# yanglei18/SGV3D

Measured on AMD Instinct MI355X. Metric: camera frames/sec at 864x1536->BEV, higher is better.
Workload: dtype f32

## Files before the change

include/sgv3d_hip.h:

```cpp
#ifndef SGV3D_HIP_H
#define SGV3D_HIP_H

#include <stddef.h>
#include <stdint.h>

#ifdef __cplusplus
extern "C" {
#endif

#define SGV3D_OK 0
#define SGV3D_EINVAL (-1)
#define SGV3D_ELAUNCH (-2)
#define SGV3D_ENOSPACE (-3)

const char *sgv3d_last_error(void);
int sgv3d_abi_version(void);


int sgv3d_voxel_pooling_forward(int batch_size, int num_points, int num_channels,
                                int num_voxel_x, int num_voxel_y, int num_voxel_z,
                                const int32_t *geom_xyz, const float *input_features,
                                float *output_features, int32_t *pos_memo, void *stream);
int sgv3d_voxel_pooling_forward_fresh(int batch_size, int num_points, int num_channels,
                                      int num_voxel_x, int num_voxel_y, int num_voxel_z,
                                      const int32_t *geom_xyz, const float *input_features,
                                      float *output_features, int32_t *pos_memo, void *stream);
int sgv3d_voxel_pooling_select_kernel(int which);
int sgv3d_voxel_pooling_kernel_for(int batch_size, int num_points, int num_channels, int num_voxel_x, int num_voxel_y, int fused);
int sgv3d_voxel_pooling_cache_clear(void);
int sgv3d_voxel_pooling_cache_stats(unsigned long long *out4);

int sgv3d_voxel_pooling_forward_atomic(int batch_size, int num_points, int num_channels,
                                       int num_voxel_x, int num_voxel_y, int num_voxel_z,
                                       const int32_t *geom_xyz, const float *input_features,
                                       float *output_features, int32_t *pos_memo, void *stream);

size_t sgv3d_voxel_plan_bytes(int batch_size, int num_points, int num_voxel_x, int num_voxel_y);

int sgv3d_voxel_plan_build(int batch_size, int num_points,
                           int num_voxel_x, int num_voxel_y, int num_voxel_z,
                           const int32_t *geom_xyz, int32_t *pos_memo,
                           void *plan, size_t plan_bytes, int sort_segments, void *stream);

int sgv3d_voxel_plan_init(int batch_size, int num_points, int num_voxel_x, int num_voxel_y,
                          void *plan, size_t plan_bytes, void *stream);
int sgv3d_voxel_plan_build_cached(int batch_size, int num_points,
                                  int num_voxel_x, int num_voxel_y, int num_voxel_z,
                                  const int32_t *geom_xyz, void *plan, size_t plan_bytes,
                                  int sort_segments, void *stream);
size_t sgv3d_voxel_plan_stats_offset(int batch_size, int num_points, int num_voxel_x, int num_voxel_y);

size_t sgv3d_voxel_pooling_workspace_bytes(int batch_size, int num_points, int num_channels);
int sgv3d_voxel_pooling_forward_planned(int batch_size, int num_points, int num_channels,
                                        int num_voxel_x, int num_voxel_y,
                                        const void *plan, const float *input_features,
                                        float *output_features, void *workspace, size_t workspace_bytes,
                                        void *stream);
int sgv3d_voxel_pooling_forward_planned_bf16(int batch_size, int num_points, int num_channels,
                                             int num_voxel_x, int num_voxel_y, const void *plan,
                                             const void *input_features_bf16, void *output_features, int out_bf16_ld,
                                             void *workspace, size_t workspace_bytes, void *stream);

int sgv3d_lift_splat_planned(int batch_size, int num_depth, int num_pixels, int num_channels,
                             int num_voxel_x, int num_voxel_y, const void *plan,
                             const float *prob, const float *context,
                             float *output_features, void *workspace, size_t workspace_bytes,
                             void *stream);

int sgv3d_lift_splat_planned_bf16out(int batch_size, int num_depth, int num_pixels, int num_channels, int num_voxel_x,
                                     int num_voxel_y, const void *plan, const float *prob, const void *context, int context_bf16,
                                     void *output_bf16, int out_bf16_ld, void *workspace, size_t workspace_bytes, void *stream);

int sgv3d_voxel_pooling_backward(int batch_size, int num_points, int num_channels,
                                 const int32_t *pos_memo, const float *grad_output,
                                 long long sb, long long sc, long long sy, long long sx,
                                 float *grad_input, void *stream);

size_t sgv3d_lift_splat_backward_workspace_bytes(int batch_size, int num_depth, int num_pixels, int num_channels);
int sgv3d_lift_splat_backward(int batch_size, int num_depth, int num_pixels, int num_channels,
                              int num_voxel_x, int num_voxel_y, int num_voxel_z,
                              const int32_t *geom_xyz,
                              const float *prob,
                              const float *context,
                              const float *grad_output,
                              long long sb, long long sy, long long sx,
                              float *grad_prob,
                              float *grad_context,
                              void *workspace, size_t workspace_bytes, void *stream);


int sgv3d_calib_prep(int num_cams, const float *sensor2ego, const float *sensor2virtual,
                     const float *intrin, const float *ida, float *prep, void *stream);

int sgv3d_geometry_voxel_index(int num_cams, int cams_per_batch, int num_depth, int feat_h, int feat_w,
                               const float *frustum, const float *prep, const float *ref_h,
                               const float *bda, const float *voxel_coord ,
                               const float *voxel_size , int32_t *geom_xyz, float *geom_f,
                               void *stream);

int sgv3d_calib_changed(int n, const void *const *tensors , const int32_t *nbytes ,
                        void *copy, int force, int32_t *changed, void *stream);
int sgv3d_calib_prep_gated(int num_cams, const float *sensor2ego, const float *sensor2virtual, const float *intrin,
                           const float *ida, float *prep, const int32_t *run, void *stream);
// ... 3 lines not shown
                                     float *geom_f, const int32_t *run, void *stream);


int sgv3d_lift(int batch_size, int num_pixels, int num_depth, int num_channels,
               const float *height_context, float *prob, float *lifted, void *stream);
int sgv3d_lift_bf16(int batch_size, int num_pixels, int num_depth, int num_channels, const float *height_context,
                    float *prob, void *lifted_bf16, void *stream);


typedef struct sgv3d_conv_desc {
    int batch, in_h, in_w, cin;
    int out_h, out_w, cout;
    int kh, kw, stride, pad, dil;
    int x_ld, x_coff;
    int y_ld, y_coff;
    int res_ld;
    int relu;
    int mode;
    int deconv_ks;
    int k_pad, cout_pad;
    int tile;
    int x_nchw;
    int k_order;
    int split_k;
} sgv3d_conv_desc;

#define SGV3D_CONV_NORMAL 0
#define SGV3D_CONV_DECONV 1
#define SGV3D_CONV_NCHW_OUT 2
#define SGV3D_CONV_GROUP_PLANES 3

#define SGV3D_TILE_128x128 1
#define SGV3D_TILE_128x64 2
#define SGV3D_TILE_64x128 3
#define SGV3D_TILE_64x64 4
#define SGV3D_TILE_32x128 9
#define SGV3D_TILE_48x64 10
#define SGV3D_TILE_X3 64
#define SGV3D_TILE_MFIRST 16
#define SGV3D_TILE_OCC5 32
#define SGV3D_WINOGRAD_RESIDENT 6
#define SGV3D_WINOGRAD_HALF 8

int sgv3d_conv_winograd4_pack_weight(const float *w_src , int cout, int cin, int k_pad, int cout_pad,
                                     float *u_packed , void *stream);
int sgv3d_conv_winograd4_pack_weight_x3(const float *w_src, int cout, int cin, int cin_pad, int cout_pad, void *u3_packed,
                                        void *stream);

int sgv3d_conv_pack_weight_x3(const float *w_src, int cout, int cin, int kh, int kw, int cin_pad, int cout_pad, void *u3_packed,
                              void *stream);
int sgv3d_conv2d_x3_forward(const sgv3d_conv_desc *desc, const float *x, const void *u3_packed, const float *scale,
                            const float *bias, const float *residual, float *y, void *workspace, size_t workspace_bytes,
                            void *stream);
int sgv3d_conv2d_x3_shortcut_forward(const sgv3d_conv_desc *desc_a, const float *xa, const void *u3a, const float *scale_a,
                                     const float *bias_a, const sgv3d_conv_desc *desc_b, const float *xb, const void *u3b,
                                     const float *scale_b, const float *bias_b, float *y, void *stream);
int sgv3d_stem_pool_x3_forward(int batch, int h, int w, const float *x_nchw, const void *w_x3, size_t w_bytes, const float *scale,
                               const float *shift, float *y_nhwc, int y_ld, int variant, void *stream);
int sgv3d_wino4_lattice_axis(int n, int dil, int tile, int k0, int count, int *tiles, int *stacked, int *pixels);
size_t sgv3d_conv2d_winograd4_workspace_bytes(const sgv3d_conv_desc *desc );
int sgv3d_conv2d_winograd4_forward(const sgv3d_conv_desc *desc , const float *x, const float *u_packed,
                                   const float *scale, const float *bias, const float *residual, float *y,
                                   void *workspace, size_t workspace_bytes, void *stream);

size_t sgv3d_conv2d_winograd4_multi_workspace_bytes(int n, const sgv3d_conv_desc *descs );
int sgv3d_conv2d_winograd4_forward_multi(int n, const sgv3d_conv_desc *descs , const float *x, const void *const *u_packed,
                                         const float *const *scale, const float *const *bias, float *const *y, void *workspace,
                                         size_t workspace_bytes, void *stream);

void sgv3d_conv_pack_geometry(int k, int n, int *k_pad, int *n_pad);

int sgv3d_conv_pack_weight(const float *w_src, int cout, int cin, int kh, int kw, int cin_pad,
                           int transposed, int k_order, float *w_packed, int k_pad, int cout_pad,
                           void *stream);

size_t sgv3d_conv2d_workspace_bytes(const sgv3d_conv_desc *desc );
int sgv3d_conv2d_forward(const sgv3d_conv_desc *desc , const float *x, const float *w_packed,
                         const float *scale, const float *bias, const float *residual,
                         const float *gate, float *y, void *workspace, size_t workspace_bytes,
                         void *stream);

int sgv3d_conv2d_forward_bf16(const sgv3d_conv_desc *desc , const float *x, const float *w_packed,
                              const float *scale, const float *bias, const float *residual,
                              const float *gate, float *y, void *workspace, size_t workspace_bytes,
                              void *stream);

int sgv3d_conv_weight_to_bf16(const float *w_packed, int k_pad, int cout_pad, void *w_packed_bf16, void *stream);
int sgv3d_conv2d_forward_bf16io(const sgv3d_conv_desc *desc , const void *x, const void *w_packed,
                                const float *scale, const float *bias, const void *residual, const float *gate,
                                void *y, void *workspace, size_t workspace_bytes, void *stream, int io_flags);

int sgv3d_conv2d_forward_f32x3(const sgv3d_conv_desc *desc , const float *x, const float *w_packed,
                               const float *scale, const float *bias, const float *residual,
                               const float *gate, float *y, void *workspace, size_t workspace_bytes,
                               void *stream);

size_t sgv3d_conv_winograd_weight_floats(int cout, int cin_pad);
int sgv3d_conv_winograd_pack_weight(const float *w_src, int cout, int cin, int cin_pad, float *w_packed,
                                    void *stream);
int sgv3d_conv2d_winograd_forward(const sgv3d_conv_desc *desc , const float *x, const float *w_wino,
                                  const float *scale, const float *bias, const float *residual,
                                  const float *gate, float *y, void *workspace, size_t workspace_bytes,
                                  void *stream);


int sgv3d_maxpool3x3s2(int batch, int in_h, int in_w, int channels, const float *x, float *y,
// ... 630 lines not shown
```

sgv3d_amd/_lib.py:

```python
import ctypes
import os

_HERE = os.path.dirname(os.path.abspath(__file__))
LIB_PATH = os.path.join(_HERE, "csrc", "libsgv3d_hip.so")

c_int, c_void_p, c_size_t, c_ll = ctypes.c_int, ctypes.c_void_p, ctypes.c_size_t, ctypes.c_longlong


class ConvDesc(ctypes.Structure):
    _fields_ = [(n, c_int) for n in (
        "batch", "in_h", "in_w", "cin", "out_h", "out_w", "cout", "kh", "kw", "stride", "pad", "dil",
        "x_ld", "x_coff", "y_ld", "y_coff", "res_ld", "relu", "mode", "deconv_ks", "k_pad", "cout_pad",
        "tile", "x_nchw", "k_order", "split_k")]


class VitAttnDesc(ctypes.Structure):
    _fields_ = [(n, c_int) for n in ("batch", "height", "width", "heads", "head_dim", "win_h", "win_w")]


class SamAttnDesc(ctypes.Structure):
    _fields_ = [(n, c_int) for n in ("batch", "nq", "nk", "heads", "head_dim", "q_ld", "k_ld", "v_ld", "o_ld")] + [("scale", ctypes.c_float)]


CONV_NORMAL, CONV_DECONV, CONV_NCHW_OUT, CONV_GROUP_PLANES = 0, 1, 2, 3
TILE_AUTO, TILE_128x128, TILE_128x64, TILE_64x128, TILE_64x64 = 0, 1, 2, 3, 4

_PROTOS = {
    "sgv3d_last_error": (ctypes.c_char_p, []),
    "sgv3d_abi_version": (c_int, []),
    "sgv3d_voxel_pooling_select_kernel": (c_int, [c_int]),
    "sgv3d_voxel_pooling_kernel_for": (c_int, [c_int] * 6),
    "sgv3d_voxel_pooling_forward": (c_int, [c_int] * 6 + [c_void_p] * 5),
    "sgv3d_voxel_pooling_forward_fresh": (c_int, [c_int] * 6 + [c_void_p] * 5),
    "sgv3d_voxel_pooling_forward_atomic": (c_int, [c_int] * 6 + [c_void_p] * 5),
    "sgv3d_voxel_pooling_cache_clear": (c_int, []),
    "sgv3d_voxel_pooling_cache_stats": (c_int, [ctypes.POINTER(ctypes.c_ulonglong)]),
    "sgv3d_voxel_plan_bytes": (c_size_t, [c_int] * 4),
    "sgv3d_voxel_plan_build": (c_int, [c_int] * 5 + [c_void_p, c_void_p, c_void_p, c_size_t, c_int, c_void_p]),
    "sgv3d_voxel_plan_init": (c_int, [c_int] * 4 + [c_void_p, c_size_t, c_void_p]),
    "sgv3d_voxel_plan_build_cached": (c_int, [c_int] * 5 + [c_void_p, c_void_p, c_size_t, c_int, c_void_p]),
    "sgv3d_voxel_plan_stats_offset": (c_size_t, [c_int] * 4),
    "sgv3d_voxel_pooling_workspace_bytes": (c_size_t, [c_int] * 3),
    "sgv3d_voxel_pooling_forward_planned": (c_int, [c_int] * 5 + [c_void_p] * 4 + [c_size_t, c_void_p]),
    "sgv3d_voxel_pooling_forward_planned_bf16": (c_int, [c_int] * 5 + [c_void_p] * 3 + [c_int, c_void_p, c_size_t, c_void_p]),
    "sgv3d_lift_splat_planned_bf16out": (c_int, [c_int] * 6 + [c_void_p] * 3 + [c_int, c_void_p, c_int, c_void_p, c_size_t, c_void_p]),
    "sgv3d_lift_splat_planned": (c_int, [c_int] * 6 + [c_void_p] * 5 + [c_size_t, c_void_p]),
    "sgv3d_voxel_pooling_backward": (c_int, [c_int] * 3 + [c_void_p, c_void_p, c_ll, c_ll, c_ll, c_ll, c_void_p, c_void_p]),
    "sgv3d_lift_splat_backward_workspace_bytes": (c_size_t, [c_int] * 4),
    "sgv3d_lift_splat_backward": (c_int, [c_int] * 7 + [c_void_p] * 4 + [c_ll] * 3 + [c_void_p] * 3 + [c_size_t, c_void_p]),
    "sgv3d_calib_prep": (c_int, [c_int] + [c_void_p] * 6),
    "sgv3d_calib_prep_gated": (c_int, [c_int] + [c_void_p] * 7),
    "sgv3d_calib_changed": (c_int, [c_int, ctypes.POINTER(c_void_p), ctypes.POINTER(c_int), c_void_p, c_int, c_void_p, c_void_p]),
    "sgv3d_geometry_voxel_index_gated": (c_int, [c_int] * 5 + [c_void_p] * 4 + [ctypes.POINTER(ctypes.c_float)] * 2 + [c_void_p] * 4),
    "sgv3d_dense_gated": (c_int, [c_int] * 3 + [c_void_p] * 4 + [c_int, c_void_p, c_void_p, c_void_p]),
    "sgv3d_geometry_voxel_index": (c_int, [c_int] * 5 + [c_void_p] * 4 + [ctypes.POINTER(ctypes.c_float)] * 2 + [c_void_p] * 3),
    "sgv3d_lift": (c_int, [c_int] * 4 + [c_void_p] * 4),
    "sgv3d_lift_bf16": (c_int, [c_int] * 4 + [c_void_p] * 4),
    "sgv3d_conv_pack_geometry": (None, [c_int, c_int, ctypes.POINTER(c_int), ctypes.POINTER(c_int)]),
    "sgv3d_conv_pack_weight": (c_int, [c_void_p] + [c_int] * 7 + [c_void_p, c_int, c_int, c_void_p]),
    "sgv3d_conv2d_workspace_bytes": (c_size_t, [ctypes.POINTER(ConvDesc)]),
    "sgv3d_conv2d_forward": (c_int, [ctypes.POINTER(ConvDesc)] + [c_void_p] * 8 + [c_size_t, c_void_p]),
    "sgv3d_conv2d_forward_bf16": (c_int, [ctypes.POINTER(ConvDesc)] + [c_void_p] * 8 + [c_size_t, c_void_p]),
    "sgv3d_conv2d_forward_bf16io": (c_int, [ctypes.POINTER(ConvDesc)] + [c_void_p] * 8 + [c_size_t, c_void_p, c_int]),
    "sgv3d_conv_weight_to_bf16": (c_int, [c_void_p, c_int, c_int, c_void_p, c_void_p]),
    "sgv3d_conv2d_forward_f32x3": (c_int, [ctypes.POINTER(ConvDesc)] + [c_void_p] * 8 + [c_size_t, c_void_p]),
    "sgv3d_centerhead_branches_workspace_bytes": (c_size_t, [c_int] * 4),
    "sgv3d_centerhead_branches_forward": (c_int, [c_int] * 6 + [c_void_p, c_int] + [c_void_p] * 3 + [c_int] + [c_void_p] * 5
                                          + [c_size_t, c_void_p]),
    "sgv3d_centerhead_bf16_weight_bytes": (c_size_t, [c_int]),
    "sgv3d_centerhead_bf16_pack_weight": (c_int, [c_void_p, c_int, c_int, c_void_p, c_void_p]),
    "sgv3d_centerhead_bf16_weight2_bytes": (c_size_t, [c_int]),
    "sgv3d_centerhead_bf16_pack_weight2": (c_int, [c_void_p, c_void_p, c_int, c_void_p, c_void_p]),
    "sgv3d_centerhead_f4_weight_floats": (c_size_t, [c_int]),
    "sgv3d_centerhead_f4_pack_weight": (c_int, [c_void_p, c_int, c_void_p, c_void_p]),
    "sgv3d_centerhead_branches_forward_f4": (c_int, [c_int] * 6 + [c_void_p, c_int] + [c_void_p] * 3 + [c_int] + [c_void_p] * 5
                                             + [c_size_t, c_void_p]),
    "sgv3d_conv3x3_f4res_weight_floats": (c_size_t, [c_int, c_int]),
    "sgv3d_conv3x3_f4res_pack_weight": (c_int, [c_void_p, c_int, c_int, c_int, c_void_p, c_void_p]),
    "sgv3d_conv3x3_f4res_forward": (c_int, [ctypes.POINTER(ConvDesc)] + [c_void_p] * 7),
    "sgv3d_centerhead_branches_forward_bf16": (c_int, [c_int] * 6 + [c_void_p, c_int] + [c_void_p] * 3 + [c_int] + [c_void_p] * 5),
    "sgv3d_centerhead_branches_forward_bf16x": (c_int, [c_int] * 6 + [c_void_p, c_int] + [c_void_p] * 3 + [c_int] + [c_void_p] * 5),
    "sgv3d_centerhead_bf16_select_plain": (None, [c_int]),
    "sgv3d_centerhead_bf16_debug_stamps": (None, [c_void_p]),
    "sgv3d_scale_channels_bf16": (c_int, [c_int] * 3 + [c_void_p] * 4),
    "sgv3d_global_avgpool_bf16": (c_int, [c_int] * 4 + [c_void_p] * 3 + [c_size_t, c_void_p]),
    "sgv3d_broadcast_channels_bf16": (c_int, [c_int] * 5 + [c_void_p] * 3),
    "sgv3d_upsample_bilinear2x_bf16": (c_int, [c_int] * 4 + [c_void_p] * 3),
    "sgv3d_add_mul_sigmoid_bf16": (c_int, [c_ll] + [c_void_p] * 5),
    "sgv3d_deform_im2col3x3_bf16": (c_int, [c_int] * 5 + [c_void_p] * 2 + [c_int, c_void_p, c_void_p]),
    "sgv3d_conv3x3_patch_bf16_weight_bytes": (c_size_t, [c_int, c_int]),
    "sgv3d_conv3x3_patch_bf16_debug_stamps": (None, [c_void_p]),
    "sgv3d_conv3x3_patch_bf16_pack_weight": (c_int, [c_void_p, c_int, c_int, c_void_p, c_void_p]),
    "sgv3d_conv3x3_patch_bf16_forward": (c_int, [c_int] * 11 + [c_void_p] * 6 + [c_int, c_int, c_void_p, c_size_t, c_void_p]),
    "sgv3d_conv_dw_bf16_weight_bytes": (c_size_t, [c_int] * 4),
    "sgv3d_conv_dw_bf16_pack_weight": (c_int, [c_void_p] + [c_int] * 5 + [c_void_p, c_void_p]),
    "sgv3d_conv_dw_bf16_forward": (c_int, [ctypes.POINTER(ConvDesc)] + [c_void_p] * 7),
    "sgv3d_conv_dw_bf16_workspace_bytes": (c_size_t, [ctypes.POINTER(ConvDesc)]),
    "sgv3d_conv_dw_bf16_forward_splitk": (c_int, [ctypes.POINTER(ConvDesc)] + [c_void_p] * 7 + [c_size_t, c_void_p]),
    "sgv3d_conv_dw_bf16_pair_forward": (c_int, [ctypes.POINTER(ConvDesc)] + [c_void_p] * 4 + [c_int] + [c_void_p] * 4 + [c_int, c_void_p, c_int, c_int, c_int, c_void_p]),
    "sgv3d_conv_winograd_weight_floats": (c_size_t, [c_int, c_int]),
    "sgv3d_conv_winograd_pack_weight": (c_int, [c_void_p, c_int, c_int, c_int, c_void_p, c_void_p]),
    "sgv3d_conv2d_winograd_forward": (c_int, [ctypes.POINTER(ConvDesc)] + [c_void_p] * 8 + [c_size_t, c_void_p]),
    "sgv3d_conv_winograd4_pack_weight": (c_int, [c_void_p, c_int, c_int, c_int, c_int, c_void_p, c_void_p]),
    "sgv3d_conv_winograd4_pack_weight_x3": (c_int, [c_void_p, c_int, c_int, c_int, c_int, c_void_p, c_void_p]),
    "sgv3d_conv_pack_weight_x3": (c_int, [c_void_p, c_int, c_int, c_int, c_int, c_int, c_int, c_void_p, c_void_p]),
    "sgv3d_conv2d_x3_forward": (c_int, [c_void_p] * 8 + [c_size_t, c_void_p]),
    "sgv3d_conv2d_x3_shortcut_forward": (c_int, [c_void_p] * 12),
    "sgv3d_stem_pool_x3_forward": (c_int, [c_int] * 3 + [c_void_p, c_void_p, c_size_t] + [c_void_p] * 3 + [c_int, c_int, c_void_p]),
    "sgv3d_wino4_lattice_axis": (c_int, [c_int] * 5 + [c_void_p] * 3),
    "sgv3d_conv2d_winograd4_workspace_bytes": (c_size_t, [ctypes.POINTER(ConvDesc)]),
    "sgv3d_conv2d_winograd4_forward": (c_int, [ctypes.POINTER(ConvDesc)] + [c_void_p] * 7 + [c_size_t, c_void_p]),
    "sgv3d_conv2d_winograd4_multi_workspace_bytes": (c_size_t, [c_int, c_void_p]),
    "sgv3d_conv2d_winograd4_forward_multi": (c_int, [c_int] + [c_void_p] * 7 + [c_size_t, c_void_p]),
    "sgv3d_maxpool3x3s2": (c_int, [c_int] * 4 + [c_void_p] * 3),
    "sgv3d_maxpool3x3s2_bf16": (c_int, [c_int] * 4 + [c_void_p] * 3),
    "sgv3d_nchw_to_nhwc": (c_int, [c_int] * 5 + [c_void_p] * 3),
    "sgv3d_nhwc_to_nchw": (c_int, [c_int] * 6 + [c_void_p] * 3),
    "sgv3d_global_avgpool_workspace_bytes": (c_size_t, [c_int] * 2),
    "sgv3d_global_avgpool": (c_int, [c_int] * 4 + [c_void_p] * 3 + [c_size_t, c_void_p]),
    "sgv3d_dense": (c_int, [c_int] * 3 + [c_void_p] * 4 + [c_int, c_void_p, c_void_p]),
    "sgv3d_broadcast_channels": (c_int, [c_int] * 5 + [c_void_p] * 3),
    "sgv3d_scale_channels": (c_int, [c_int] * 3 + [c_void_p] * 4),
    "sgv3d_copy_channels": (c_int, [c_int] * 5 + [c_void_p] * 3),
    "sgv3d_upsample_bilinear2x": (c_int, [c_int] * 4 + [c_void_p] * 3),
    "sgv3d_add_mul_sigmoid": (c_int, [c_ll] + [c_void_p] * 5),
    "sgv3d_bsm_compose": (c_int, [c_int] * 6 + [c_void_p, c_int, ctypes.c_float, c_void_p, c_void_p]),
    "sgv3d_deform_im2col3x3": (c_int, [c_int] * 5 + [c_void_p, c_void_p, c_int, c_void_p, c_void_p]),
    "sgv3d_deform_conv3x3_forward": (c_int, [c_int] * 6 + [c_void_p, c_void_p, c_int, c_void_p, c_int, c_int, c_void_p, c_int, c_int,
                                                          c_void_p]),
    "sgv3d_deform_conv3x3_bf16_weight_bytes": (c_size_t, [c_int] * 3),
    "sgv3d_deform_conv3x3_bf16_pack_weight": (c_int, [c_void_p, c_int, c_int, c_int, c_void_p, c_void_p]),
    "sgv3d_deform_conv3x3_forward_bf16": (c_int, [c_int] * 6 + [c_void_p, c_int, c_void_p, c_int, c_void_p, c_void_p, c_int, c_int, c_int,
                                                               c_void_p]),
    "sgv3d_head_final_conv": (c_int, [c_int] * 6 + [c_void_p] * 6),
    "sgv3d_centerpoint_decode_workspace_bytes": (c_size_t, [c_int] * 3),
    "sgv3d_centerpoint_decode": (c_int, [c_int] * 5 + [c_void_p] * 6 + [c_ll] + [ctypes.c_float] * 6 +
                                 [ctypes.POINTER(ctypes.c_float), c_int, ctypes.c_float, c_int, c_void_p, c_size_t] +
                                 [c_void_p] * 6),
    "sgv3d_centerpoint_decode_tasks_workspace_bytes": (c_size_t, [c_int] * 4),
    "sgv3d_centerpoint_decode_tasks": (c_int, [c_int, c_int, ctypes.POINTER(ctypes.c_int32), c_int, c_int, c_int] +
                                       [ctypes.POINTER(c_void_p)] * 6 + [c_ll] + [ctypes.c_float] * 6 +
                                       [ctypes.POINTER(ctypes.c_float), c_int, ctypes.POINTER(ctypes.c_float), c_int, c_void_p,
                                        c_size_t] + [c_void_p] * 6),
    "sgv3d_centerpoint_merge_tasks": (c_int, [c_int] * 3 + [c_void_p] * 4 + [ctypes.POINTER(ctypes.c_int32)] + [c_void_p] * 5),
    "sgv3d_rotated_bev_iou_host": (c_int, [c_int] + [ctypes.POINTER(ctypes.c_float)] * 3),
    "sgv3d_rotate_nms_workspace_bytes": (c_size_t, [c_int] * 3),
    "sgv3d_rotate_nms": (c_int, [c_int] * 3 + [c_void_p] * 3 + [ctypes.c_float, ctypes.POINTER(ctypes.c_float), c_int, c_int,
                                                                ctypes.POINTER(ctypes.c_float), c_void_p, c_size_t, c_void_p, c_void_p]),
    "sgv3d_centerpoint_decode_tasks_rotate_workspace_bytes": (c_size_t, [c_int] * 4),
    "sgv3d_centerpoint_decode_tasks_rotate": (c_int, [c_int, c_int, ctypes.POINTER(ctypes.c_int32), c_int, c_int, c_int] +
                                              [ctypes.POINTER(c_void_p)] * 6 + [c_ll] + [ctypes.c_float] * 6 +
                                              [ctypes.POINTER(ctypes.c_float), c_int, ctypes.c_float, ctypes.POINTER(ctypes.c_float),
                                               c_int, c_int, ctypes.POINTER(ctypes.c_float), c_void_p, c_size_t] + [c_void_p] * 6),
    "sgv3d_centerhead_targets": (c_int, [c_int, c_int, c_void_p, c_void_p, c_int, ctypes.POINTER(ctypes.c_int32)] +
                                 [c_int] * 3 + [ctypes.c_float] * 5 + [ctypes.c_double, c_int, c_int] + [c_void_p] * 5),
    "sgv3d_conv2d_backward_weight_workspace_bytes": (c_size_t, [ctypes.POINTER(ConvDesc), c_int]),
    "sgv3d_conv2d_backward_weight": (c_int, [ctypes.POINTER(ConvDesc)] + [c_void_p] * 3 + [c_int, c_void_p, c_size_t, c_void_p]),
    "sgv3d_conv2d_backward_weight_bf16_workspace_bytes": (c_size_t, [ctypes.POINTER(ConvDesc), c_int]),
    "sgv3d_conv2d_backward_weight_bf16": (c_int, [ctypes.POINTER(ConvDesc)] + [c_void_p] * 3 + [c_int, c_void_p, c_size_t, c_void_p]),
# ... 196 lines not shown
```

sgv3d_amd/csrc/conv_pw_x3.hip:

```cpp
#include "conv_common.hpp"
#include "f32x3.hpp"

using namespace sgv3d;

namespace {

struct PwX3Args {
    const float *x, *scale, *bias, *res;
    const void *w;
    float *y;
    int M, K, N;
    int x_ld, x_coff, y_ld, y_coff, res_ld, relu;
    int cout_pad, tiles_m, tiles_n, mfirst;
    unsigned x_bytes, w_bytes;
    int in_h, in_w, out_h, out_w, kh, kw, stride, pad, dil;
    int cin4;
    int split_k;
    float *ws;
    const float *x2, *scale2, *bias2;
    const void *w2;
    int K2, x2_ld, x2_coff;
    unsigned x2_bytes, w2_bytes;
};

template <int MA, int WN, int MODE>
__global__ __launch_bounds__(64 * WN, 2) void conv_pw_x3_kernel(const PwX3Args a) {
    constexpr bool TAPS = MODE == 1, TM = MODE == 2, DUAL = MODE == 3, DECONV = MODE == 4;
    constexpr int NT = 64 * WN, BM = 16 * MA, BN = 32 * WN;
    constexpr int PLANE = x3_plane_bytes(BM), BUF = x3_buf_bytes(BM);
    __shared__ __attribute__((aligned(16))) unsigned char smem[2 * BUF];

    const int logical = xcd_tile(blockIdx.x, a.tiles_m * a.tiles_n);
    int tn, tm;
    if (a.mfirst) {
        tm = (int)((unsigned)logical / (unsigned)a.tiles_n);
        tn = logical - tm * a.tiles_n;
    } else {
        tn = (int)((unsigned)logical / (unsigned)a.tiles_m);
        tm = logical - tn * a.tiles_m;
    }
    const int m0 = tm * BM, n0 = tn * BN;
    const int kb = a.K >> 5;

    const int tid = threadIdx.x;
    __amdgpu_buffer_rsrc_t x_rsrc = __builtin_amdgcn_make_buffer_rsrc(const_cast<float *>(a.x), 0, (int)a.x_bytes, 0x00020000);
    __amdgpu_buffer_rsrc_t w_rsrc = __builtin_amdgcn_make_buffer_rsrc(const_cast<void *>(a.w), 0, (int)a.w_bytes, 0x00020000);

    constexpr int RPA = NT / 8, PA = (BM + RPA - 1) / RPA;
    static_assert(RPA % 16 == 0, "a pass is a multiple of 16 rows");
    const int arow = tid >> 3, ach = tid & 7;
    unsigned xg[PA];
    [[maybe_unused]] unsigned xmask[PA];
    [[maybe_unused]] unsigned long long xmask64[PA];
    bool a_on[PA];
    const int taps = (TAPS || TM) ? a.kh * a.kw : 1;
#pragma unroll
    for (int i = 0; i < PA; ++i) {
        const int r = arow + RPA * i;
        a_on[i] = (arow & ~7) + RPA * i < BM;
        const bool live = a_on[i] && m0 + r < a.M;
        if constexpr (!TAPS && !TM) {
            xg[i] = live ? (unsigned)((((long long)(m0 + r)) * a.x_ld + a.x_coff + ach * 4) * 4) : 0xffffffffu;
        } else if constexpr (TM) {
            const int m = live ? m0 + r : 0;
            const int t = (int)((unsigned)m / (unsigned)a.out_w);
            const int ow = m - t * a.out_w;
            const int n = (int)((unsigned)t / (unsigned)a.out_h);
            const int oh = t - n * a.out_h;
            const int ih0 = oh * a.stride - a.pad, iw0 = ow * a.stride - a.pad;
            xg[i] = (unsigned)((((long long)(n * a.in_h + ih0) * a.in_w + iw0) * a.x_ld + a.x_coff) * 4);
            unsigned long long mk = 0;
            int tt = 0;
            for (int th = 0; th < a.kh; ++th) {
                const bool row_in = live && (unsigned)(ih0 + th * a.dil) < (unsigned)a.in_h;
                for (int tw = 0; tw < a.kw; ++tw, ++tt) mk |= (row_in && (unsigned)(iw0 + tw * a.dil) < (unsigned)a.in_w) ? (1ull << tt) : 0ull;
            }
            xmask64[i] = mk;
        } else {
            const int m = live ? m0 + r : 0;
            const int t = (int)((unsigned)m / (unsigned)a.out_w);
            const int ow = m - t * a.out_w;
            const int n = (int)((unsigned)t / (unsigned)a.out_h);
            const int oh = t - n * a.out_h;
            const int ih0 = oh * a.stride - a.pad, iw0 = ow * a.stride - a.pad;
            xg[i] = (unsigned)((((long long)(n * a.in_h + ih0) * a.in_w + iw0) * a.x_ld + a.x_coff + ach * 4) * 4);
            unsigned mk = 0;
            int tt = 0;
            for (int th = 0; th < a.kh; ++th) {
                const bool row_in = live && (unsigned)(ih0 + th * a.dil) < (unsigned)a.in_h;
                for (int tw = 0; tw < a.kw; ++tw, ++tt) mk |= (row_in && (unsigned)(iw0 + tw * a.dil) < (unsigned)a.in_w) ? (1u << tt) : 0u;
            }
            xmask[i] = mk;
        }
    }
    [[maybe_unused]] int ld_tap = 0, ld_kh = 0, ld_kw = 0, ld_c0 = 0;
    [[maybe_unused]] const int cq = a.cin4;
    [[maybe_unused]] int tm_tap = 0, tm_kh = 0, tm_kw = 0, tm_c4 = 0;
    const unsigned xl = (unsigned)(arow * 64 + ((((ach >> 1) ^ x3_swizzle(arow)) << 4) | ((ach & 1) << 3)));

    const int wave = tid >> 6, lane = tid & 63;
    const int l16 = lane & 15, g = lane >> 4;
    unsigned wgo[2];
#pragma unroll
    for (int nb = 0; nb < 2; ++nb) wgo[nb] = u3_lane_offset((n0 >> 4) + 2 * wave + nb, kb, lane, a.cout_pad);
    const unsigned x_frag = X3_FRAG_OFFSET(l16, g);

    f32x4 acc[MA][2];
#pragma unroll
    for (int ma = 0; ma < MA; ++ma)
#pragma unroll
        for (int nb = 0; nb < 2; ++nb) acc[ma][nb] = f32x4{0.f, 0.f, 0.f, 0.f};

    f32x4 rx[PA];
    bf16x8 fw[2][2][3];
    int kt0 = 0, nkt = kb;
    if (a.split_k > 1) {
        kt0 = (int)((unsigned)kb * blockIdx.y / (unsigned)a.split_k);
        nkt = (int)((unsigned)kb * (blockIdx.y + 1) / (unsigned)a.split_k) - kt0;
        if constexpr (TAPS) {
            const int chunk = kt0 / taps;
            ld_tap = kt0 - chunk * taps;
            ld_c0 = chunk * 32;
            ld_kh = ld_tap / a.kw;
            ld_kw = ld_tap - ld_kh * a.kw;
        }
    }
    if constexpr (TM) {
        const int q = kt0 * 8 + ach;
        tm_tap = q / cq;
        tm_c4 = q - tm_tap * cq;
        tm_kh = tm_tap / a.kw;
        tm_kw = tm_tap - tm_kh * a.kw;
    }

#define PWX3_REQUEST(KT)                                                                                  \
    do {                                                                                                  \
        if constexpr (!TAPS && !TM) {                                                                     \
            _Pragma("unroll") for (int i = 0; i < PA; ++i)                                                \
                rx[i] = __builtin_bit_cast(f32x4, __builtin_amdgcn_raw_buffer_load_b128(x_rsrc, xg[i], (kt0 + (KT)) * 128, 0)); \
        } else if constexpr (TM) {                                                                        \
            const unsigned koff_ = (unsigned)((((tm_kh * a.in_w + tm_kw) * a.dil) * a.x_ld + tm_c4 * 4) * 4); \
            const unsigned long long bit_ = tm_tap < taps ? 1ull << tm_tap : 0ull;      \
            _Pragma("unroll") for (int i = 0; i < PA; ++i)                                                \
                rx[i] = __builtin_bit_cast(f32x4, __builtin_amdgcn_raw_buffer_load_b128(                   \
                    x_rsrc, (xmask64[i] & bit_) ? xg[i] + koff_ : 0xffffffffu, 0, 0));                    \
            tm_c4 += 8;                                                                                   \
            while (tm_c4 >= cq) {                                                                         \
                tm_c4 -= cq;                                                                              \
                ++tm_tap;                                                                                 \
                if (++tm_kw == a.kw) { tm_kw = 0; ++tm_kh; }                                              \
            }                                                                                             \
        } else {                                                                                          \
            const unsigned koff_ = (unsigned)((((ld_kh * a.in_w + ld_kw) * a.dil) * a.x_ld + ld_c0) * 4);  \
            const unsigned bit_ = 1u << ld_tap;                                                           \
            _Pragma("unroll") for (int i = 0; i < PA; ++i)                                                \
                rx[i] = __builtin_bit_cast(f32x4, __builtin_amdgcn_raw_buffer_load_b128(                   \
                    x_rsrc, (xmask[i] & bit_) ? xg[i] + koff_ : 0xffffffffu, 0, 0));                      \
            ++ld_tap;                                                                                     \
            if (++ld_kw == a.kw) {                                                                        \
                ld_kw = 0;                                                                                \
                if (++ld_kh == a.kh) { ld_kh = 0; ld_tap = 0; ld_c0 += 32; }                              \
            }                                                                                             \
        }                                                                                                 \
    } while (0)
#define PWX3_STORE(B)                                                                                     \
    do {                                                                                                  \
        _Pragma("unroll") for (int i = 0; i < PA; ++i)                                                    \
            if (a_on[i]) {                                                                                \
                bf16x4 hi, mid, lo;                                                                       \
                split3(rx[i], hi, mid, lo);                                                               \
                unsigned char *d = smem + (B) * BUF + xl + i * RPA * 64;                                  \
                *reinterpret_cast<bf16x4 *>(d) = hi;                                                      \
                *reinterpret_cast<bf16x4 *>(d + PLANE) = mid;                                             \
                *reinterpret_cast<bf16x4 *>(d + 2 * PLANE) = lo;                                          \
            }                                                                                             \
    } while (0)
#define PWX3_KLOOP() X3_KLOOP(MA, smem, w_rsrc, wgo, kt0, nkt, x_frag, fw, acc, PWX3_REQUEST, PWX3_STORE)

    PWX3_KLOOP();
    [[maybe_unused]] f32x4 tkeep[MA][2];
    if constexpr (DUAL) {
#pragma unroll
        for (int nb = 0; nb < 2; ++nb) {
            const int col = n0 + 32 * wave + 16 * nb + 4 * g;
            const bool on = col < a.N;
            const f32x4 sc = (on && a.scale) ? *reinterpret_cast<const f32x4 *>(a.scale + col) : f32x4{1.f, 1.f, 1.f, 1.f};
            const f32x4 sh = (on && a.bias) ? *reinterpret_cast<const f32x4 *>(a.bias + col) : f32x4{0.f, 0.f, 0.f, 0.f};
#pragma unroll
            for (int ma = 0; ma < MA; ++ma) {
                tkeep[ma][nb] = acc[ma][nb] * sc + sh;
                acc[ma][nb] = f32x4{0.f, 0.f, 0.f, 0.f};
            }
        }
        x_rsrc = __builtin_amdgcn_make_buffer_rsrc(const_cast<float *>(a.x2), 0, (int)a.x2_bytes, 0x00020000);
        w_rsrc = __builtin_amdgcn_make_buffer_rsrc(const_cast<void *>(a.w2), 0, (int)a.w2_bytes, 0x00020000);
        nkt = a.K2 >> 5;
#pragma unroll
        for (int i = 0; i < PA; ++i) {
            const int r = arow + RPA * i;
            const bool live = a_on[i] && m0 + r < a.M;
            const int m = live ? m0 + r : 0;
            const int t = (int)((unsigned)m / (unsigned)a.out_w);
            const int ow = m - t * a.out_w;
            const int n = (int)((unsigned)t / (unsigned)a.out_h);
            const int oh = t - n * a.out_h;
            xg[i] = live ? (unsigned)((((long long)(n * a.in_h + oh * a.stride) * a.in_w + ow * a.stride) * a.x2_ld + a.x2_coff + ach * 4) * 4)
                         : 0xffffffffu;
        }
#pragma unroll
        for (int nb = 0; nb < 2; ++nb) wgo[nb] = u3_lane_offset((n0 >> 4) + 2 * wave + nb, nkt, lane, a.cout_pad);
        __syncthreads();
        PWX3_KLOOP();
    }
#undef PWX3_KLOOP
#undef PWX3_REQUEST
#undef PWX3_STORE

    if (a.split_k > 1) {
        float *wsb = a.ws + (size_t)blockIdx.y * a.M * a.N;
#pragma unroll
        for (int nb = 0; nb < 2; ++nb) {
            const int col = n0 + 32 * wave + 16 * nb + 4 * g;
            if (col >= a.N) continue;
#pragma unroll
            for (int ma = 0; ma < MA; ++ma) {
                const int row = m0 + 16 * ma + l16;
                if (row < a.M) *reinterpret_cast<f32x4 *>(wsb + (size_t)row * a.N + col) = acc[ma][nb];
            }
        }
        return;
    }
    const float floor_ = a.relu ? 0.f : -__builtin_inff();
// ... 32 lines not shown
                const int row = m0 + 16 * ma + l16;
                if (row >= a.M) continue;
                const int img = (int)((unsigned)row / (unsigned)hw), pix = row - img * hw;
                const int ih = (int)((unsigned)pix / (unsigned)a.in_w), iw = pix - ih * a.in_w;
                f32x4 v = acc[ma][nb] * sc + sh;
                v = f32x4{fmaxf(v[0], floor_), fmaxf(v[1], floor_), fmaxf(v[2], floor_), fmaxf(v[3], floor_)};
                *reinterpret_cast<f32x4 *>(a.y + ((size_t)(img * a.out_h + ih * ks + dy) * a.out_w + (iw * ks + dx)) * a.y_ld + a.y_coff + co) = v;
            }
        }
        return;
    }
#pragma unroll
    for (int nb = 0; nb < 2; ++nb) {
        const int col = n0 + 32 * wave + 16 * nb + 4 * g;
        if (col >= a.N) continue;
        const f32x4 sc = a.scale ? *reinterpret_cast<const f32x4 *>(a.scale + col) : f32x4{1.f, 1.f, 1.f, 1.f};
        const f32x4 sh = a.bias ? *reinterpret_cast<const f32x4 *>(a.bias + col) : f32x4{0.f, 0.f, 0.f, 0.f};
#pragma unroll
        for (int ma = 0; ma < MA; ++ma) {
            const int row = m0 + 16 * ma + l16;
            if (row >= a.M) continue;
            f32x4 v = acc[ma][nb] * sc + sh;
            if (a.res) v += *reinterpret_cast<const f32x4 *>(a.res + (size_t)row * a.res_ld + col);
            v = f32x4{fmaxf(v[0], floor_), fmaxf(v[1], floor_), fmaxf(v[2], floor_), fmaxf(v[3], floor_)};
            *reinterpret_cast<f32x4 *>(a.y + (size_t)row * a.y_ld + a.y_coff + col) = v;
        }
    }
}

__global__ __launch_bounds__(256) void pack_weight_x3_kernel(const float *__restrict__ w, int cout, int cin, int cin_pad, int cout_pad,
                                                             int taps, int k_order, __bf16 *__restrict__ u) {
    const long long kp = k_order ? (long long)taps * cin_pad : ((long long)taps * cin_pad + 31) / 32 * 32;
    const long long i = (long long)blockIdx.x * 256 + threadIdx.x;
    if (i >= (long long)cout_pad * kp) return;
    const int co = (int)(i / kp), k = (int)(i - (long long)co * kp);
    int tap, ci;
    if (k_order) {
        const int chunk = k / (32 * taps), rem = k - chunk * 32 * taps;
        tap = rem >> 5;
        ci = chunk * 32 + (rem & 31);
    } else {
        tap = k / cin_pad;
        ci = k - tap * cin_pad;
    }
    const float v = (co < cout && ci < cin && tap < taps) ? w[((size_t)co * cin + ci) * taps + tap] : 0.f;
    __bf16 hi, mid, lo;
    split3_rounded(v, hi, mid, lo);
    u3_store(u3_at(u, co, k, kp), hi, mid, lo);
}

template <int MA, int WN>
int launch_pw(const PwX3Args &a, int mode, hipStream_t st) {
    const dim3 grid(a.tiles_m * a.tiles_n, a.split_k > 1 ? a.split_k : 1);
    if (mode == 4) hipLaunchKernelGGL((conv_pw_x3_kernel<MA, WN, 4>), grid, dim3(64 * WN), 0, st, a);
    else if (mode == 3) hipLaunchKernelGGL((conv_pw_x3_kernel<MA, WN, 3>), grid, dim3(64 * WN), 0, st, a);
    else if (mode == 2) hipLaunchKernelGGL((conv_pw_x3_kernel<MA, WN, 2>), grid, dim3(64 * WN), 0, st, a);
    else if (mode == 1) hipLaunchKernelGGL((conv_pw_x3_kernel<MA, WN, 1>), grid, dim3(64 * WN), 0, st, a);
    else hipLaunchKernelGGL((conv_pw_x3_kernel<MA, WN, 0>), grid, dim3(64 * WN), 0, st, a);
    return check_launch("conv_pw_x3_kernel");
}

}

extern "C" int sgv3d_conv_pack_weight_x3(const float *w_src, int cout, int cin, int kh, int kw, int cin_pad, int cout_pad, void *u3_packed,
                                         void *stream) {
    const int k_order = cin_pad % 32 == 0 ? 1 : 0;
    SGV3D_REQUIRE(w_src && u3_packed && cout > 0 && cin > 0 && kh > 0 && kw > 0 && kh * kw <= (k_order ? 32 : 64) && cin_pad >= cin &&
                      cin_pad % 4 == 0 && cout_pad >= cout && cout_pad % 32 == 0,
                  "conv_pack_weight_x3: bad arguments (cout=%d cin=%d k=%dx%d cin_pad=%d cout_pad=%d)", cout, cin, kh, kw, cin_pad, cout_pad);
    const long long kp = k_order ? (long long)cin_pad * kh * kw : ((long long)cin_pad * kh * kw + 31) / 32 * 32;
    const long long total = (long long)cout_pad * kp;
    hipLaunchKernelGGL(pack_weight_x3_kernel, dim3(cdiv(total, 256)), dim3(256), 0, as_stream(stream), w_src, cout, cin, cin_pad, cout_pad,
                       kh * kw, k_order, static_cast<__bf16 *>(u3_packed));
    return check_launch("pack_weight_x3_kernel");
}

extern "C" int sgv3d_conv2d_x3_forward(const sgv3d_conv_desc *d, const float *x, const void *u3_packed, const float *scale,
                                       const float *bias, const float *residual, float *y, void *workspace, size_t workspace_bytes,
                                       void *stream) {
    SGV3D_REQUIRE(d && x && u3_packed && y, "conv2d_x3_forward: null pointer");
    const bool tapmajor = d->cin % 32 != 0;
    const bool deconv = d->mode == SGV3D_CONV_DECONV;
    if (deconv) {
        SGV3D_REQUIRE(d->kh == 1 && d->kw == 1 && d->stride == 1 && d->pad == 0 && d->deconv_ks >= 1 && d->deconv_ks <= 64 &&
                          residual == nullptr,
                      "conv2d_x3_forward: DECONV runs as a 1x1 GEMM with deconv_ks = kernel = stride (<= 64), no residual");
        SGV3D_REQUIRE(d->in_h > 0 && d->in_w > 0 && d->out_h == d->in_h * d->deconv_ks && d->out_w == d->in_w * d->deconv_ks,
                      "conv2d_x3_forward: DECONV output must be input * deconv_ks");
        SGV3D_REQUIRE(d->cin > 0 && d->cin % 32 == 0 && d->cout > 0 && d->cout % 4 == 0 &&
                          (long long)d->cout * d->deconv_ks * d->deconv_ks <= 0x1000000LL,
                      "conv2d_x3_forward: DECONV needs cin %% 32 == 0, cout %% 4 == 0 (cin=%d cout=%d)", d->cin, d->cout);
        SGV3D_REQUIRE((long long)d->batch * d->out_h * d->out_w < 0x7fffffffLL, "conv2d_x3_forward: DECONV output has 2^31 pixels or more");
    }
    SGV3D_REQUIRE((deconv || d->mode == SGV3D_CONV_NORMAL) && d->kh > 0 && d->kw > 0 && d->kh * d->kw <= (tapmajor ? 64 : 32) && d->stride > 0 &&
                      d->dil > 0 && d->pad >= 0,
                  "conv2d_x3_forward: NHWC output, at most 32 taps (64 with tap-major weights)");
    SGV3D_REQUIRE(d->batch > 0 && d->in_h > 0 && d->in_w > 0 && d->cin > 0 && d->cout > 0 && d->cin % 4 == 0 && d->cout % 4 == 0,
                  "conv2d_x3_forward: cin %% 4 == 0, cout %% 4 == 0 (cin=%d cout=%d)", d->cin, d->cout);
    SGV3D_REQUIRE(deconv || (d->out_h == (d->in_h + 2 * d->pad - d->dil * (d->kh - 1) - 1) / d->stride + 1 &&
                                 d->out_w == (d->in_w + 2 * d->pad - d->dil * (d->kw - 1) - 1) / d->stride + 1),
                  "conv2d_x3_forward: output size does not match the geometry");
    SGV3D_REQUIRE((d->x_ld & 3) == 0 && (d->x_coff & 3) == 0 && (d->y_ld & 3) == 0 && (d->y_coff & 3) == 0 && (residual == nullptr || (d->res_ld & 3) == 0),
                  "conv2d_x3_forward: leading dimensions and channel offsets must be multiples of 4");
    SGV3D_REQUIRE(d->x_ld >= d->x_coff + d->cin && d->y_ld >= d->y_coff + d->cout && (residual == nullptr || d->res_ld >= d->cout),
                  "conv2d_x3_forward: leading dimension too small");
    const int gemm_n = deconv ? d->cout * d->deconv_ks * d->deconv_ks : d->cout;
    SGV3D_REQUIRE(d->cout_pad >= gemm_n && d->cout_pad % 32 == 0, "conv2d_x3_forward: desc.cout_pad = rows of the x3 weights (a multiple of 32)");
    SGV3D_REQUIRE(((reinterpret_cast<uintptr_t>(x) | reinterpret_cast<uintptr_t>(y) | reinterpret_cast<uintptr_t>(residual) |
                    reinterpret_cast<uintptr_t>(scale) | reinterpret_cast<uintptr_t>(bias) | reinterpret_cast<uintptr_t>(u3_packed)) & 15) == 0,
                  "conv2d_x3_forward: pointers must be 16-B aligned");
    const long long M = deconv ? (long long)d->batch * d->in_h * d->in_w : (long long)d->batch * d->out_h * d->out_w;
    const long long K = tapmajor ? ((long long)d->kh * d->kw * d->cin + 31) / 32 * 32 : (long long)d->kh * d->kw * d->cin;
    const long long xb = (long long)d->batch * d->in_h * d->in_w * d->x_ld * 4, wb = (long long)d->cout_pad * K * 6;
    SGV3D_REQUIRE(M < 0x7fffffffLL && xb < 0xf0000000LL && wb < 0xf0000000LL, "conv2d_x3_forward: operands larger than 3.75 GiB");
    const int variant = d->tile & 15;
    SGV3D_REQUIRE((d->tile & SGV3D_TILE_X3) && (variant & 3) < 3 && (variant & 12) != 12,
                  "conv2d_x3_forward: desc.tile = SGV3D_TILE_X3 | variant, variant in {0,1,2, 4,5,6, 8,9,10}");
    const int taps = deconv ? 4 : tapmajor ? 2 : (d->kh == 1 && d->kw == 1 && d->stride == 1 && d->pad == 0) ? 0 : 1;
    PwX3Args a;
    a.x = x; a.w = u3_packed; a.scale = scale; a.bias = bias; a.res = residual; a.y = y;
    a.M = (int)M; a.K = (int)K; a.N = gemm_n;
    a.x_ld = d->x_ld; a.x_coff = d->x_coff; a.y_ld = d->y_ld; a.y_coff = d->y_coff; a.res_ld = d->res_ld; a.relu = d->relu;
    a.cout_pad = d->cout_pad;
    a.mfirst = (d->tile & SGV3D_TILE_MFIRST) ? 1 : 0;
    a.x_bytes = (unsigned)xb; a.w_bytes = (unsigned)wb;
    a.in_h = d->in_h; a.in_w = d->in_w; a.out_h = d->out_h; a.out_w = d->out_w;
    a.kh = d->kh; a.kw = d->kw; a.stride = d->stride; a.pad = d->pad; a.dil = d->dil;
    a.cin4 = d->cin / 4;
    if (deconv) { a.kh = d->deconv_ks; a.cin4 = d->cout; }
    const int bm = 32 << (variant & 3), bn = (variant & 8) ? 256 : (variant & 4) ? 64 : 128;
    a.tiles_m = (int)cdiv(M, bm);
    a.tiles_n = cdiv(gemm_n, bn);
    hipStream_t st = as_stream(stream);
    a.split_k = d->split_k > 1 ? d->split_k : 1;
    a.ws = nullptr;
    if (a.split_k > 1) {
        SGV3D_REQUIRE(a.split_k <= K / 32, "conv2d_x3_forward: split_k %d exceeds the %lld k-steps", a.split_k, K / 32);
        const size_t need = (size_t)a.split_k * (size_t)M * gemm_n * sizeof(float);
        if (!workspace || workspace_bytes < need)
            return fail(SGV3D_ENOSPACE, "conv2d_x3_forward: split-K workspace has %zu bytes, needs %zu", workspace_bytes, need);
        SGV3D_REQUIRE((reinterpret_cast<uintptr_t>(workspace) & 15) == 0, "conv2d_x3_forward: workspace must be 16-B aligned");
        a.ws = static_cast<float *>(workspace);
    }
    int rc;
    switch (variant) {
        case 0: rc = launch_pw<2, 4>(a, taps, st); break;
        case 1: rc = launch_pw<4, 4>(a, taps, st); break;
        case 2: rc = launch_pw<8, 4>(a, taps, st); break;
        case 4: rc = launch_pw<2, 2>(a, taps, st); break;
        case 5: rc = launch_pw<4, 2>(a, taps, st); break;
        case 6: rc = launch_pw<8, 2>(a, taps, st); break;
        case 8: rc = launch_pw<2, 8>(a, taps, st); break;
        case 9: rc = launch_pw<4, 8>(a, taps, st); break;
        default: rc = launch_pw<8, 8>(a, taps, st); break;
    }
    if (rc != SGV3D_OK || a.split_k <= 1) return rc;
    ConvArgs r{};
    r.M = a.M; r.N = a.N; r.ws = a.ws; r.split_k = a.split_k;
    r.scale = scale; r.bias = bias; r.res = residual; r.res_ld = d->res_ld; r.relu = d->relu;
    r.y = y; r.y_ld = d->y_ld; r.y_coff = d->y_coff; r.mode = d->mode; r.ks = d->deconv_ks; r.cout = d->cout;
    r.m_h = deconv ? d->in_h : d->out_h; r.m_w = deconv ? d->in_w : d->out_w; r.out_h = d->out_h; r.out_w = d->out_w;
    return launch_splitk_reduce(r, st);
}

extern "C" int sgv3d_conv2d_x3_shortcut_forward(const sgv3d_conv_desc *da, const float *xa, const void *u3a, const float *scale_a,
                                                const float *bias_a, const sgv3d_conv_desc *db, const float *xb, const void *u3b,
                                                const float *scale_b, const float *bias_b, float *y, void *stream) {
    SGV3D_REQUIRE(da && db && xa && xb && u3a && u3b && y, "conv2d_x3_shortcut_forward: null pointer");
    SGV3D_REQUIRE(da->mode == SGV3D_CONV_NORMAL && db->mode == SGV3D_CONV_NORMAL && da->split_k <= 1 && db->split_k <= 1,
                  "conv2d_x3_shortcut_forward: NHWC output, no split-K");
    SGV3D_REQUIRE(da->kh == 1 && da->kw == 1 && da->stride == 1 && da->pad == 0 && db->kh == 1 && db->kw == 1 && db->pad == 0 &&
                      (db->stride == 1 || db->stride == 2),
                  "conv2d_x3_shortcut_forward: source A is 1x1 / stride 1, source B 1x1 / stride 1 or 2, neither padded");
    SGV3D_REQUIRE(da->batch > 0 && da->in_h > 0 && da->in_w > 0 && db->in_h > 0 && db->in_w > 0 && da->cin > 0 && db->cin > 0 &&
                      da->cout > 0 && da->cin % 32 == 0 && db->cin % 32 == 0 && da->cout % 4 == 0,
                  "conv2d_x3_shortcut_forward: cin %% 32 == 0 on both sources, cout %% 4 == 0 (cin=%d / %d cout=%d)", da->cin, db->cin,
                  da->cout);
    SGV3D_REQUIRE(da->cout == db->cout && da->cout_pad == db->cout_pad, "conv2d_x3_shortcut_forward: the sources' cout differ (%d / %d)",
                  da->cout, db->cout);
    SGV3D_REQUIRE(da->out_h == da->in_h && da->out_w == da->in_w && db->out_h == (db->in_h - 1) / db->stride + 1 &&
                      db->out_w == (db->in_w - 1) / db->stride + 1,
                  "conv2d_x3_shortcut_forward: output size does not match the geometry");
    SGV3D_REQUIRE(da->batch == db->batch && da->out_h == db->out_h && da->out_w == db->out_w,
                  "conv2d_x3_shortcut_forward: the sources' output geometries differ (%dx%dx%d / %dx%dx%d)", da->batch, da->out_h,
                  da->out_w, db->batch, db->out_h, db->out_w);
    SGV3D_REQUIRE(((da->x_ld | da->x_coff | da->y_ld | da->y_coff | db->x_ld | db->x_coff) & 3) == 0,
                  "conv2d_x3_shortcut_forward: leading dimensions and channel offsets must be multiples of 4");
    SGV3D_REQUIRE(da->x_ld >= da->x_coff + da->cin && db->x_ld >= db->x_coff + db->cin && da->y_ld >= da->y_coff + da->cout &&
                      da->x_coff >= 0 && db->x_coff >= 0 && da->y_coff >= 0,
                  "conv2d_x3_shortcut_forward: leading dimension too small");
    SGV3D_REQUIRE(da->cout_pad >= da->cout && da->cout_pad % 32 == 0,
                  "conv2d_x3_shortcut_forward: desc.cout_pad = rows of the x3 weights (a multiple of 32)");
    SGV3D_REQUIRE(((reinterpret_cast<uintptr_t>(xa) | reinterpret_cast<uintptr_t>(xb) | reinterpret_cast<uintptr_t>(y) |
                    reinterpret_cast<uintptr_t>(scale_a) | reinterpret_cast<uintptr_t>(bias_a) | reinterpret_cast<uintptr_t>(scale_b) |
                    reinterpret_cast<uintptr_t>(bias_b) | reinterpret_cast<uintptr_t>(u3a) | reinterpret_cast<uintptr_t>(u3b)) & 15) == 0,
                  "conv2d_x3_shortcut_forward: pointers must be 16-B aligned");
    const long long M = (long long)da->batch * da->out_h * da->out_w;
    const long long xab = M * da->x_ld * 4, xbb = (long long)db->batch * db->in_h * db->in_w * db->x_ld * 4;
    const long long wab = (long long)da->cout_pad * da->cin * 6, wbb = (long long)db->cout_pad * db->cin * 6;
    SGV3D_REQUIRE(M < 0x7fffffffLL && xab < 0xf0000000LL && xbb < 0xf0000000LL && wab < 0xf0000000LL && wbb < 0xf0000000LL,
                  "conv2d_x3_shortcut_forward: operands larger than 3.75 GiB");
    const int variant = da->tile & 15;
    SGV3D_REQUIRE((da->tile & SGV3D_TILE_X3) && (variant & 3) < 3 && (variant & 12) != 12,
                  "conv2d_x3_shortcut_forward: desc_a.tile = SGV3D_TILE_X3 | variant, variant in {0,1,2, 4,5,6, 8,9,10}");
    PwX3Args a{};
    a.x = xa; a.w = u3a; a.scale = scale_a; a.bias = bias_a; a.res = nullptr; a.y = y;
    a.M = (int)M; a.K = da->cin; a.N = da->cout;
    a.x_ld = da->x_ld; a.x_coff = da->x_coff; a.y_ld = da->y_ld; a.y_coff = da->y_coff; a.res_ld = 0; a.relu = da->relu;
    a.cout_pad = da->cout_pad;
    a.mfirst = (da->tile & SGV3D_TILE_MFIRST) ? 1 : 0;
    a.x_bytes = (unsigned)xab; a.w_bytes = (unsigned)wab;
    a.in_h = db->in_h; a.in_w = db->in_w; a.out_h = db->out_h; a.out_w = db->out_w;
    a.kh = 1; a.kw = 1; a.stride = db->stride; a.pad = 0; a.dil = 1;
    a.cin4 = da->cin / 4;
    a.x2 = xb; a.w2 = u3b; a.scale2 = scale_b; a.bias2 = bias_b;
// ... 21 lines not shown
```

sgv3d_amd/csrc/voxel_pooling.hip:

```cpp
#include <atomic>
#include "common.hpp"

#include <limits.h>
#include <stdlib.h>

#include <mutex>
#include <vector>

using namespace sgv3d;

namespace {

constexpr int kBlock = 256;

__device__ __forceinline__ int voxel_of_point(const int32_t *__restrict__ geom, long long pt, int b,
                                              int X, int Y, int Z, int &x, int &y) {
    x = geom[pt * 3 + 0];
    y = geom[pt * 3 + 1];
    const int z = geom[pt * 3 + 2];
    if (x < 0 || x >= X || y < 0 || y >= Y || z < 0 || z >= Z) return -1;
    return (b * Y + y) * X + x;
}

constexpr int kAtomicPts = 64;

__global__ __launch_bounds__(kBlock) void vp_atomic_kernel(
    long long total_pts, int N, int C, int X, int Y, int Z, const int32_t *__restrict__ geom,
    const float *__restrict__ feats, float *__restrict__ out, int32_t *__restrict__ pos_memo) {
    __shared__ int vid_s[kAtomicPts];
    const int tid = threadIdx.x;
    const long long p0 = (long long)blockIdx.x * kAtomicPts;
    if (tid < kAtomicPts) {
        const long long pt = p0 + tid;
        int v = -1;
        if (pt < total_pts) {
            const int b = (int)(pt / N);
            int x, y;
            v = voxel_of_point(geom, pt, b, X, Y, Z, x, y);
            if (v >= 0 && pos_memo) {
                pos_memo[pt * 3 + 0] = b;
                pos_memo[pt * 3 + 1] = y;
                pos_memo[pt * 3 + 2] = x;
            }
        }
        vid_s[tid] = v;
    }
    __syncthreads();
    const int nelem = kAtomicPts * C;
    const float *f = feats + (size_t)p0 * C;
    for (int e = tid; e < nelem; e += kBlock) {
        const int pl = e / C;
        const int c = e - pl * C;
        const int v = vid_s[pl];
        if (v >= 0) {
            __hip_atomic_fetch_add(out + (size_t)v * C + c, f[e], __ATOMIC_RELAXED,
                                   __HIP_MEMORY_SCOPE_AGENT);
        }
    }
}

constexpr int kScanPerThread = 8;
constexpr int kScanElems = kBlock * kScanPerThread;

struct PlanLayout {
    long long V;
    long long total;
    int nblk;
    int ncw;
    size_t off_seg, off_cur, off_order, off_slotvox, off_blk, off_hdr, off_geom, off_long, off_perm, off_bins, bytes;
    int long_cap;
};

constexpr int kVoxClasses = 55;
__host__ __device__ inline int vp_class(int n) {
    if (n <= 0) return 0;
    if (n <= 32) return n;
    if (n <= 320) return 33 + (n - 33) / 32;
    int c = 42, hi = 400;
    while (c < kVoxClasses - 1 && n > hi) {
        hi += hi >> 2;
        ++c;
    }
    return c;
}

constexpr int kLongRun = 128;

struct PlanHeader {
    int dirty;
    int diff;
    int ticket;
    int params[7];
    int builds;
    int bar;
    int err;
};
constexpr int kPlanMagic = 0x53475633;

PlanLayout plan_layout(int B, int N, int X, int Y) {
    PlanLayout L;
    L.V = (long long)B * Y * X;
    L.total = (long long)B * N;
    L.nblk = cdiv(L.V, kScanElems);
    auto al = [](size_t x) { return (x + 255) & ~(size_t)255; };
    L.off_seg = 0;
    L.off_cur = al(L.off_seg + sizeof(int) * (size_t)(L.V + 1));
    L.off_order = al(L.off_cur + sizeof(int) * (size_t)(L.V + 1));
    L.off_slotvox = al(L.off_order + sizeof(int) * (size_t)L.total);
    L.off_blk = al(L.off_slotvox + sizeof(int) * (size_t)(L.total + 1));
    L.off_hdr = al(L.off_blk + sizeof(int) * (size_t)(L.nblk + 2));
    L.off_geom = al(L.off_hdr + sizeof(PlanHeader));
    L.off_long = al(L.off_geom + sizeof(int) * 3 * (size_t)L.total);
    L.long_cap = (int)(L.total / kLongRun) + 1;
    L.off_perm = al(L.off_long + sizeof(int) * (size_t)(L.long_cap + 1));
    L.off_bins = al(L.off_perm + sizeof(int) * 4 * (size_t)L.V);
    L.ncw = cdiv(L.V, kBlock);
    L.bytes = al(L.off_bins + sizeof(int) * ((size_t)kVoxClasses * L.ncw + 2 * kVoxClasses + 2));
    return L;
}

__device__ __forceinline__ void wave_runs(int v, int lane, int &head_lane, int &run_len, bool &is_head) {
    const int vp = __shfl_up(v, 1, 64);
    is_head = (lane == 0) || (vp != v);
    const unsigned long long heads = __ballot(is_head);
    const unsigned long long upto = lane == 63 ? ~0ull : ((1ull << (lane + 1)) - 1);
    head_lane = 63 - __clzll((long long)(heads & upto));
    const unsigned long long after = head_lane == 63 ? 0ull : heads & ~((1ull << (head_lane + 1)) - 1);
    const int next = after ? __ffsll((long long)after) - 1 : 64;
    run_len = next - head_lane;
}

#define VP_SKIP_IF_CLEAN(dirty) \
    if ((dirty) != nullptr && *reinterpret_cast<const volatile int *>(dirty) == 0) return

__global__ __launch_bounds__(kBlock) void vp_plan_init_kernel(PlanHeader *__restrict__ hdr) {
    if (threadIdx.x == 0) {
        hdr->dirty = 1; hdr->diff = 0; hdr->ticket = 0; hdr->builds = 0; hdr->bar = 0; hdr->err = 0;
        for (int i = 0; i < 7; ++i) hdr->params[i] = 0;
    }
}

__global__ __launch_bounds__(kBlock) void vp_geom_compare_kernel(long long n_ints, const int32_t *__restrict__ geom,
                                                                 const int32_t *__restrict__ copy,
                                                                 PlanHeader *__restrict__ hdr, int p0, int p1, int p2,
                                                                 int p3, int p4, int p5, int p6) {
    __shared__ int any_s;
    if (threadIdx.x == 0) any_s = 0;
    __syncthreads();
    const long long n4 = n_ints >> 2;
    const long long stride = (long long)gridDim.x * kBlock;
    bool diff = false;
    const int4 *g4 = reinterpret_cast<const int4 *>(geom);
    const int4 *c4 = reinterpret_cast<const int4 *>(copy);
    for (long long i = (long long)blockIdx.x * kBlock + threadIdx.x; i < n4; i += stride) {
        const int4 a = g4[i], b = c4[i];
        diff |= (a.x != b.x) | (a.y != b.y) | (a.z != b.z) | (a.w != b.w);
    }
    if (blockIdx.x == 0 && threadIdx.x < (n_ints & 3)) diff |= geom[n4 * 4 + threadIdx.x] != copy[n4 * 4 + threadIdx.x];
    if (diff) any_s = 1;
    __syncthreads();
    if (threadIdx.x == 0) {
        if (any_s) atomicOr(&hdr->diff, 1);
        __threadfence();
        const int t = atomicAdd(&hdr->ticket, 1);
        if (t == (int)gridDim.x - 1) {
            __threadfence();
            const int d = atomicOr(&hdr->diff, 0);
            const int *q = hdr->params;
            const bool same = q[0] == p0 && q[1] == p1 && q[2] == p2 && q[3] == p3 && q[4] == p4 && q[5] == p5 && q[6] == p6;
            hdr->dirty = (d != 0 || !same) ? 1 : 0;
// ... 121 lines not shown
        const int v = (i < nblk) ? blk_sum[i] : 0;
        int tot;
        const int ex = block_exclusive_scan(v, wave_tot, tot);
        if (i < nblk) blk_sum[i] = carry + ex;
        carry += tot;
    }
    if (threadIdx.x == 0) blk_sum[nblk] = carry;
}

__global__ __launch_bounds__(kBlock) void vp_scan_top_kernel(int nblk, int *__restrict__ blk_sum,
                                                             const int *__restrict__ dirty, int *__restrict__ long_list) {
    VP_SKIP_IF_CLEAN(dirty);
    vp_scan_top_body(nblk, blk_sum, dirty, long_list, (int)blockIdx.x, (int)gridDim.x);
}

__device__ __forceinline__ void vp_scan_add_body(long long V, int nblk,
                                                             const int *__restrict__ blk_sum,
                                                             int *__restrict__ seg_start,
                                                             int *__restrict__ cursor, const int *__restrict__ dirty, const int VBID, const int VGRID) {
    const long long i = (long long)VBID * kBlock + threadIdx.x;
    if (i < V) {
        const int s = seg_start[i] + blk_sum[i / kScanElems];
        seg_start[i] = s;
        cursor[i] = s;
    } else if (i == V) {
        seg_start[V] = blk_sum[nblk];
    }
}

__global__ __launch_bounds__(kBlock) void vp_scan_add_kernel(long long V, int nblk,
                                                             const int *__restrict__ blk_sum,
                                                             int *__restrict__ seg_start,
                                                             int *__restrict__ cursor, const int *__restrict__ dirty) {
    VP_SKIP_IF_CLEAN(dirty);
    vp_scan_add_body(V, nblk, blk_sum, seg_start, cursor, dirty, (int)blockIdx.x, (int)gridDim.x);
}

__device__ __forceinline__ void vp_long_list_body(long long V, const int *__restrict__ seg_start,
                                                              int *__restrict__ long_list, int cap,
                                                              const int *__restrict__ dirty, const int VBID, const int VGRID) {
    const long long v = (long long)VBID * kBlock + threadIdx.x;
    if (v >= V) return;
    if (seg_start[v + 1] - seg_start[v] > kLongRun) {
        const int i = atomicAdd(long_list, 1);
        if (i < cap) long_list[1 + i] = (int)v;
    }
}

__global__ __launch_bounds__(kBlock) void vp_long_list_kernel(long long V, const int *__restrict__ seg_start,
                                                              int *__restrict__ long_list, int cap,
                                                              const int *__restrict__ dirty) {
    VP_SKIP_IF_CLEAN(dirty);
    vp_long_list_body(V, seg_start, long_list, cap, dirty, (int)blockIdx.x, (int)gridDim.x);
}

__device__ __forceinline__ void vp_fill_body(long long total_pts, int N, int X, int Y, int Z,
                                                         const int32_t *__restrict__ geom,
                                                         int *__restrict__ cursor,
                                                         int *__restrict__ order,
                                                         int *__restrict__ slot_voxel, const int *__restrict__ dirty,
                                                         const int *__restrict__ seg_start, const int VBID, const int VGRID) {
    const long long pt = (long long)VBID * kBlock + threadIdx.x;
    const int lane = threadIdx.x & 63;
    int v = -1;
    if (pt < total_pts) {
        const int b = (int)(pt / N);
        int x, y;
        v = voxel_of_point(geom, pt, b, X, Y, Z, x, y);
    }
    int head_lane, run_len;
    bool is_head;
    wave_runs(v, lane, head_lane, run_len, is_head);
    int base = 0;
    if (is_head && v >= 0) base = atomicAdd(cursor + v, run_len);
    base = __shfl(base, head_lane, 64);
    if (v >= 0) {
        const int slot = base + (lane - head_lane);
        order[slot] = (int)pt;
        slot_voxel[slot] = (seg_start[v + 1] - seg_start[v] > kLongRun) ? ~v : v;
    }
}

__global__ __launch_bounds__(kBlock) void vp_fill_kernel(long long total_pts, int N, int X, int Y, int Z,
                                                         const int32_t *__restrict__ geom,
                                                         int *__restrict__ cursor,
                                                         int *__restrict__ order,
                                                         int *__restrict__ slot_voxel, const int *__restrict__ dirty,
                                                         const int *__restrict__ seg_start) {
    VP_SKIP_IF_CLEAN(dirty);
    vp_fill_body(total_pts, N, X, Y, Z, geom, cursor, order, slot_voxel, dirty, seg_start, (int)blockIdx.x, (int)gridDim.x);
}

__device__ __forceinline__ void vp_cls_count_body(long long V, const int *__restrict__ seg_start, int ncw,
                                                              int *__restrict__ tbl, const int *__restrict__ dirty, const int VBID, const int VGRID) {
    __shared__ int h[kVoxClasses];
    if (threadIdx.x < kVoxClasses) h[threadIdx.x] = 0;
    __syncthreads();
    const long long v = (long long)VBID * kBlock + threadIdx.x;
    const int c = v < V ? vp_class(seg_start[v + 1] - seg_start[v]) : -1;
#pragma unroll
    for (int k = 0; k < kVoxClasses; ++k) {
        const unsigned long long m = __ballot(c == k);
        if ((threadIdx.x & 63) == 0 && m != 0ull) atomicAdd(&h[k], __popcll(m));
    }
    __syncthreads();
    if (threadIdx.x < kVoxClasses) tbl[threadIdx.x * ncw + VBID] = h[threadIdx.x];
// ... 1136 lines not shown
                    bool cached, hipStream_t st, const char *what, bool compare_done = false) {
    if (int rc = check_common(batch_size, num_points, 1, num_voxel_x, num_voxel_y, num_voxel_z)) return rc;
    SGV3D_REQUIRE(geom_xyz && plan, "%s: null pointer", what);
    SGV3D_REQUIRE((reinterpret_cast<uintptr_t>(plan) & 15) == 0, "%s: plan must be 16-B aligned", what);
    SGV3D_REQUIRE(!cached || compare_done || (reinterpret_cast<uintptr_t>(geom_xyz) & 15) == 0, "%s: geom_xyz must be 16-B aligned", what);
    const PlanLayout L = plan_layout(batch_size, num_points, num_voxel_x, num_voxel_y);
    if (plan_bytes < L.bytes) return fail(SGV3D_ENOSPACE, "%s: plan has %zu bytes, needs %zu", what, plan_bytes, L.bytes);
    char *base = static_cast<char *>(plan);
    int *seg = reinterpret_cast<int *>(base + L.off_seg);
    int *cur = reinterpret_cast<int *>(base + L.off_cur);
    int *order = reinterpret_cast<int *>(base + L.off_order);
    int *blk = reinterpret_cast<int *>(base + L.off_blk);
    PlanHeader *hdr = reinterpret_cast<PlanHeader *>(base + L.off_hdr);
    int32_t *gcopy = reinterpret_cast<int32_t *>(base + L.off_geom);
    const int *dirty = cached ? &hdr->dirty : nullptr;
    const int p[7] = {kPlanMagic, batch_size, num_points, num_voxel_x, num_voxel_y, num_voxel_z, sort_segments ? 1 : 0};
    if (cached && !compare_done) {
        const long long n_ints = L.total * 3;
        const int cgrid = (int)(cdiv(n_ints / 4 + 1, kBlock) < 256 ? cdiv(n_ints / 4 + 1, kBlock) : 256);
        hipLaunchKernelGGL(vp_geom_compare_kernel, dim3(cgrid), dim3(kBlock), 0, st, n_ints, geom_xyz, gcopy, hdr, p[0],
                           p[1], p[2], p[3], p[4], p[5], p[6]);
    }
    hipLaunchKernelGGL(vp_zero_kernel, dim3(cdiv(L.V + 1, kBlock)), dim3(kBlock), 0, st, L.V + 1, cur, dirty);
    const int pgrid = cdiv(L.total, kBlock);
    hipLaunchKernelGGL(vp_count_kernel, dim3(pgrid), dim3(kBlock), 0, st, L.total, num_points, num_voxel_x,
                       num_voxel_y, num_voxel_z, geom_xyz, pos_memo, cur, dirty, cached ? gcopy : nullptr);
    hipLaunchKernelGGL(vp_scan_local_kernel, dim3(L.nblk), dim3(kBlock), 0, st, L.V, cur, seg, blk, dirty);
    int *long_list = reinterpret_cast<int *>(base + L.off_long);
    hipLaunchKernelGGL(vp_scan_top_kernel, dim3(1), dim3(kBlock), 0, st, L.nblk, blk, dirty, long_list);
    hipLaunchKernelGGL(vp_scan_add_kernel, dim3(cdiv(L.V + 1, kBlock)), dim3(kBlock), 0, st, L.V, L.nblk, blk,
                       seg, cur, dirty);
    hipLaunchKernelGGL(vp_long_list_kernel, dim3(cdiv(L.V, kBlock)), dim3(kBlock), 0, st, L.V, seg, long_list, L.long_cap, dirty);
    {
        int *tbl = reinterpret_cast<int *>(base + L.off_bins);
        int *cls = tbl + (size_t)kVoxClasses * L.ncw;
        int *perm = reinterpret_cast<int *>(base + L.off_perm);
        hipLaunchKernelGGL(vp_cls_count_kernel, dim3(L.ncw), dim3(kBlock), 0, st, L.V, seg, L.ncw, tbl, dirty);
        int *tot = cls + kVoxClasses;
        hipLaunchKernelGGL(vp_cls_scan_kernel, dim3(kVoxClasses), dim3(kBlock), 0, st, L.ncw, tbl, tot, dirty);
        hipLaunchKernelGGL(vp_cls_scatter_kernel, dim3(L.ncw), dim3(kBlock), 0, st, L.V, seg, L.ncw, tbl, tot, cls, perm, dirty);
    }
    hipLaunchKernelGGL(vp_fill_kernel, dim3(pgrid), dim3(kBlock), 0, st, L.total, num_points, num_voxel_x,
                       num_voxel_y, num_voxel_z, geom_xyz, cur, order, reinterpret_cast<int *>(base + L.off_slotvox), dirty, seg);
    if (sort_segments) {
        const int g_wave = (int)(L.V / 4 < 4096 ? (L.V + 3) / 4 : 4096);
        hipLaunchKernelGGL((vp_sort_wave_kernel<1>), dim3(g_wave), dim3(kBlock), 0, st, L.V, seg, order, 1, dirty);
        hipLaunchKernelGGL((vp_sort_wave_kernel<4>), dim3(g_wave), dim3(kBlock), 0, st, L.V, seg, order, 64, dirty);
        hipLaunchKernelGGL((vp_sort_wave_kernel<16>), dim3(g_wave), dim3(kBlock), 0, st, L.V, seg, order, 256, dirty);
        hipLaunchKernelGGL((vp_sort_wave_kernel<32>), dim3(g_wave), dim3(kBlock), 0, st, L.V, seg, order, 1024, dirty);
        const int g_large = (int)((L.V + 255) / 256 < 1024 ? (L.V + 255) / 256 : 1024);
        hipLaunchKernelGGL((vp_sort_segments_kernel<256, 8192>), dim3(g_large), dim3(256), 0, st, L.V, seg, order,
                           2048, 0x7fffffff, dirty);
    }
    if (cached)
        hipLaunchKernelGGL(vp_plan_commit_kernel, dim3(1), dim3(64), 0, st, hdr, p[0], p[1], p[2], p[3], p[4], p[5], p[6]);
    return check_launch(what);
}

}

extern "C" int sgv3d_voxel_plan_build(int batch_size, int num_points, int num_voxel_x, int num_voxel_y,
                                      int num_voxel_z, const int32_t *geom_xyz, int32_t *pos_memo,
                                      void *plan, size_t plan_bytes, int sort_segments, void *stream) {
    return plan_build_impl(batch_size, num_points, num_voxel_x, num_voxel_y, num_voxel_z, geom_xyz, pos_memo, plan,
                           plan_bytes, sort_segments, false, as_stream(stream), "voxel_plan_build");
}

extern "C" int sgv3d_voxel_plan_init(int batch_size, int num_points, int num_voxel_x, int num_voxel_y, void *plan,
                                     size_t plan_bytes, void *stream) {
    SGV3D_REQUIRE(plan && batch_size > 0 && num_points > 0 && num_voxel_x > 0 && num_voxel_y > 0, "voxel_plan_init: bad argument");
    const PlanLayout L = plan_layout(batch_size, num_points, num_voxel_x, num_voxel_y);
    if (plan_bytes < L.bytes) return fail(SGV3D_ENOSPACE, "voxel_plan_init: plan has %zu bytes, needs %zu", plan_bytes, L.bytes);
    hipLaunchKernelGGL(vp_plan_init_kernel, dim3(1), dim3(kBlock), 0, as_stream(stream),
                       reinterpret_cast<PlanHeader *>(static_cast<char *>(plan) + L.off_hdr));
    return check_launch("voxel_plan_init");
}

extern "C" int sgv3d_voxel_plan_build_cached(int batch_size, int num_points, int num_voxel_x, int num_voxel_y,
                                             int num_voxel_z, const int32_t *geom_xyz, void *plan, size_t plan_bytes,
                                             int sort_segments, void *stream) {
    return plan_build_impl(batch_size, num_points, num_voxel_x, num_voxel_y, num_voxel_z, geom_xyz, nullptr, plan,
                           plan_bytes, sort_segments, true, as_stream(stream), "voxel_plan_build_cached");
}

namespace {

template <bool VEC>
__global__ __launch_bounds__(kBlock) void vp_level1_prologue_kernel(long long total_pts, int N, int X, int Y, int Z,
                                                                    const int32_t *__restrict__ geom,
                                                                    const int32_t *__restrict__ copy,
                                                                    int32_t *__restrict__ pos_memo, PlanHeader *__restrict__ hdr,
                                                                    int *__restrict__ host_flag) {
    bool diff = false;
    const long long t = (long long)blockIdx.x * kBlock + threadIdx.x;
    if constexpr (VEC) {
        const long long pt0 = t * 4;
        if (pt0 + 3 < total_pts) {
            const int4 *g4 = reinterpret_cast<const int4 *>(geom) + t * 3;
            const int4 *c4 = reinterpret_cast<const int4 *>(copy) + t * 3;
            const int4 g0 = g4[0], g1 = g4[1], g2 = g4[2];
            const int4 c0 = c4[0], c1 = c4[1], c2 = c4[2];
            diff = (g0.x != c0.x) | (g0.y != c0.y) | (g0.z != c0.z) | (g0.w != c0.w) | (g1.x != c1.x) | (g1.y != c1.y) |
                   (g1.z != c1.z) | (g1.w != c1.w) | (g2.x != c2.x) | (g2.y != c2.y) | (g2.z != c2.z) | (g2.w != c2.w);
            if (pos_memo != nullptr) {
                const int px[4] = {g0.x, g0.w, g1.z, g2.y}, py[4] = {g0.y, g1.x, g1.w, g2.z}, pz[4] = {g0.z, g1.y, g2.x, g2.w};
                bool keep[4];
// ... 258 lines not shown
                                           const int32_t *geom_xyz, const float *input_features,
                                           float *output_features, int32_t *pos_memo, void *stream) {
    return level1_forward<false>(batch_size, num_points, num_channels, num_voxel_x, num_voxel_y, num_voxel_z, geom_xyz,
                                 input_features, output_features, pos_memo, stream);
}

extern "C" int sgv3d_voxel_pooling_forward_fresh(int batch_size, int num_points, int num_channels,
                                                 int num_voxel_x, int num_voxel_y, int num_voxel_z,
                                                 const int32_t *geom_xyz, const float *input_features,
                                                 float *output_features, int32_t *pos_memo, void *stream) {
    return level1_forward<true>(batch_size, num_points, num_channels, num_voxel_x, num_voxel_y, num_voxel_z, geom_xyz,
                                input_features, output_features, pos_memo, stream);
}

extern "C" int sgv3d_voxel_pooling_kernel_for(int batch_size, int num_points, int num_channels, int num_voxel_x, int num_voxel_y,
                                              int fused) {
    if (batch_size <= 0 || num_points <= 0 || num_voxel_x <= 0 || num_voxel_y <= 0) return 0;
    if ((long long)batch_size * num_points >= 0x7fffffffLL || (long long)batch_size * num_voxel_x * num_voxel_y >= 0x7fffffffLL) return 0;
    (void)fused;
    const PlanLayout L = plan_layout(batch_size, num_points, num_voxel_x, num_voxel_y);
    return vp_pick_gather(L, num_channels, L.total, 4, 4, 0).kernel == VpGather::kVoxelOwner ? 2 : 0;
}

extern "C" int sgv3d_voxel_pooling_select_kernel(int which) {
    SGV3D_REQUIRE(which >= 0 && which <= 2, "voxel_pooling_select_kernel: 0 or 2 (the rule), 1 (vp_gather3_kernel in place of the voxel-owner kernel)");
    g_vp_kernel.store(which, std::memory_order_relaxed);
    return SGV3D_OK;
}

extern "C" int sgv3d_voxel_pooling_cache_clear(void) {
    std::lock_guard<std::mutex> lock(g_l1_mutex);
    (void)hipDeviceSynchronize();
    std::vector<Level1Entry> kept;
    for (auto &e : g_l1) {
        if (e.pinned) kept.push_back(e);
        else level1_free(e);
    }
    g_l1.swap(kept);
    return SGV3D_OK;
}

extern "C" int sgv3d_voxel_pooling_cache_stats(unsigned long long *out4) {
    SGV3D_REQUIRE(out4 != nullptr, "voxel_pooling_cache_stats: null pointer");
    std::lock_guard<std::mutex> lock(g_l1_mutex);
    for (int i = 0; i < 4; ++i) out4[i] = g_l1_stats[i];
    return SGV3D_OK;
}

extern "C" size_t sgv3d_voxel_plan_stats_offset(int batch_size, int num_points, int num_voxel_x, int num_voxel_y) {
    if (batch_size <= 0 || num_points <= 0 || num_voxel_x <= 0 || num_voxel_y <= 0) return 0;
    return plan_layout(batch_size, num_points, num_voxel_x, num_voxel_y).off_hdr;
}

extern "C" size_t sgv3d_voxel_pooling_workspace_bytes(int batch_size, int num_points, int num_channels) {
    if (batch_size <= 0 || num_points <= 0 || num_channels <= 0) return 0;
    return 16;
}

extern "C" int sgv3d_voxel_pooling_forward_planned(int batch_size, int num_points, int num_channels,
                                                   int num_voxel_x, int num_voxel_y, const void *plan,
                                                   const float *input_features, float *output_features,
                                                   void *workspace, size_t workspace_bytes, void *stream) {
    if (int rc = check_common(batch_size, num_points, num_channels, num_voxel_x, num_voxel_y, 1)) return rc;
    SGV3D_REQUIRE(plan && input_features && output_features, "voxel_pooling_forward_planned: null pointer");
    SGV3D_REQUIRE((reinterpret_cast<uintptr_t>(input_features) & 15) == 0 &&
                      (reinterpret_cast<uintptr_t>(output_features) & 15) == 0,
                  "voxel_pooling_forward_planned: feature buffers must be 16-B aligned");
    return launch_gather<false>(batch_size, num_points, num_channels, num_voxel_x, num_voxel_y, plan,
                                input_features, nullptr, nullptr, 1, output_features, workspace, workspace_bytes,
                                as_stream(stream));
}

extern "C" int sgv3d_voxel_pooling_forward_planned_bf16(int batch_size, int num_points, int num_channels, int num_voxel_x,
                                                        int num_voxel_y, const void *plan, const void *input_features_bf16,
                                                        void *output_features, int out_bf16_ld, void *workspace,
                                                        size_t workspace_bytes, void *stream) {
    if (int rc = check_common(batch_size, num_points, num_channels, num_voxel_x, num_voxel_y, 1)) return rc;
    SGV3D_REQUIRE(plan && input_features_bf16 && output_features, "voxel_pooling_forward_planned_bf16: null pointer");
    SGV3D_REQUIRE((reinterpret_cast<uintptr_t>(input_features_bf16) & 7) == 0 && (reinterpret_cast<uintptr_t>(output_features) & 15) == 0,
                  "voxel_pooling_forward_planned_bf16: features must be 8-B, output 16-B aligned");
    SGV3D_REQUIRE(out_bf16_ld == 0 || (out_bf16_ld >= num_channels && out_bf16_ld % 4 == 0 && out_bf16_ld - num_channels <= 4 * (num_channels / 4)),
                  "voxel_pooling_forward_planned_bf16: out_bf16_ld must be 0 (f32 output) or a multiple of 4 in [C, 2C]");
    if (out_bf16_ld)
        return launch_gather<false, true, true>(batch_size, num_points, num_channels, num_voxel_x, num_voxel_y, plan,
                                                static_cast<const float *>(input_features_bf16), nullptr, nullptr, 1,
                                                static_cast<float *>(output_features), workspace, workspace_bytes, as_stream(stream),
                                                out_bf16_ld);
    return launch_gather<false, true>(batch_size, num_points, num_channels, num_voxel_x, num_voxel_y, plan,
                                      static_cast<const float *>(input_features_bf16), nullptr, nullptr, 1,
                                      static_cast<float *>(output_features), workspace, workspace_bytes, as_stream(stream));
}

extern "C" int sgv3d_lift_splat_planned(int batch_size, int num_depth, int num_pixels, int num_channels,
                                        int num_voxel_x, int num_voxel_y, const void *plan, const float *prob,
                                        const float *context, float *output_features, void *workspace,
                                        size_t workspace_bytes, void *stream) {
    SGV3D_REQUIRE(num_depth > 0 && num_pixels > 0, "lift_splat_planned: non-positive size");
    const long long N = (long long)num_depth * num_pixels;
    SGV3D_REQUIRE(N < 0x7fffffffLL, "lift_splat_planned: D*P too large");
    if (int rc = check_common(batch_size, (int)N, num_channels, num_voxel_x, num_voxel_y, 1)) return rc;
    SGV3D_REQUIRE(plan && prob && context && output_features, "lift_splat_planned: null pointer");
    SGV3D_REQUIRE((reinterpret_cast<uintptr_t>(context) & 15) == 0 &&
                      (reinterpret_cast<uintptr_t>(output_features) & 15) == 0,
                  "lift_splat_planned: context/output must be 16-B aligned");
    return launch_gather<true>(batch_size, (int)N, num_channels, num_voxel_x, num_voxel_y, plan, nullptr, prob,
                               context, num_pixels, output_features, workspace, workspace_bytes, as_stream(stream));
// ... 36 lines not shown
```

sgv3d_amd/hip_ops.py:

```python
import ctypes
from collections import namedtuple
from functools import partialmethod

import torch

from . import _lib, conv_tiles, pack_cache
from ._lib import ConvDesc, CONV_NORMAL, CONV_DECONV, CONV_NCHW_OUT, CONV_GROUP_PLANES
from .conv_tiles import (TILE_WINO, TILE_WINO_RES, TILE_PATCH, TILE_WINO_HALF, TILE_WINO4, TILE_WINO4_WIDE, TILE_WINO4_NARROW,
                         TILE_WINO4_OCC, TILE_WINO4_G48, TILE_F4RES)


def _st(t):
    return _lib.stream_handle(t.device)


PROFILE = None
AUTOTUNE = not __import__("os").environ.get("SGV3D_NO_AUTOTUNE")
DETERMINISTIC = __import__("os").environ.get("SGV3D_DETERMINISTIC", "0") not in ("", "0")


def deterministic():
    return DETERMINISTIC or torch.are_deterministic_algorithms_enabled()
PROFILE_DETAIL = False
import os as _os
# ... 81 lines not shown

def tune_may_measure():
    return AUTOTUNE and not deterministic() and not torch.cuda.is_current_stream_capturing()


def tune_record(sig, entry):
    TUNE_DB[sig] = entry
    _COMMITTED_SIGS.discard(sig)


def tune_best_of(sig, device, baseline, candidates):
    baseline()
    t0 = time_callable(baseline, device)
    best, t1 = None, None
    for key, fn in candidates:
        fn()
        dt = time_callable(fn, device)
        if TUNE_VERBOSE:
            print(f"[tune] {sig}: {key}: {dt * 1e3 / TUNE_ROUNDS:.1f} us (baseline {t0 * 1e3 / TUNE_ROUNDS:.1f} us)", flush=True)
        if t1 is None or dt < t1:
            best, t1 = key, dt
    return t0, best, t1


load_default_tune_dbs()
load_tune_db()
TILES = conv_tiles.TILES
TILE_NAMES = {t: T.label for t, T in TILES.items()}
MFIRST = _os.environ.get("SGV3D_MFIRST", "1") != "0"
WINO4_X3_TILES = conv_tiles.family("wino4_x3")
X3_TILE_ROWS = {t: TILES[t].bm for t in WINO4_X3_TILES}
X3_TILE_COLS = {t: TILES[t].bn for t in WINO4_X3_TILES}
WINO4_TILES = conv_tiles.family("wino4", "wino4_x3")


def wino4_axis_tiles(n, dil):
    dil = max(1, int(dil))
    return min(dil * -(-(-(-n // dil)) // 4), -(-(n + dil - 1) // 4))


def wino4_tiles(batch, oh, ow, dil):
    return batch * wino4_axis_tiles(oh, dil) * wino4_axis_tiles(ow, dil)


def _wino4_tiles_per_phase(batch, oh, ow, dil):
    dil = max(1, int(dil))
    return batch * dil * dil * -(-(-(-oh // dil)) // 4) * -(-(-(-ow // dil)) // 4)


WINO4_G48 = _os.environ.get("SGV3D_WINO4_G48", "1") != "0"
WINO4_X3 = _os.environ.get("SGV3D_WINO4_X3", "1") != "0"
PW_X3 = _os.environ.get("SGV3D_PW_X3", "1") != "0"
PW_X3_TILES = conv_tiles.family("pw_x3")
PW_X3_DIMS = {t: (TILES[t].bm, TILES[t].bn) for t in PW_X3_TILES}


def _pw_x3_tiles(gemm_m, gemm_n, nkt=None, mfirst=True, skip=()):
    out = ()
    for t in PW_X3_TILES:
        bm, bn = PW_X3_DIMS[t]
        wgs = -(-gemm_m // bm) * -(-gemm_n // bn)
        if (bm, bn) in skip or (bn == 256 and gemm_n < 256) or (TILES[t].mfirst and not (mfirst and MFIRST and gemm_n > bn)):
            continue
        if (wgs >= 96 or (SPLIT_K and nkt is not None and nkt >= 16)) and (bn >= 128 or gemm_n <= 64 or wgs < 1024):
            out += (t,)
    return out


def _split_factors(policy, nk, wgs):
    if not SPLIT_K:
        return ()
    pol = conv_tiles.SPLIT_POLICY[policy]
    return tuple(s for s in conv_tiles.SPLITS if nk // s >= pol["min_k"] and wgs < pol["max_wgs"] and wgs * s <= pol["max_total"])


F4RES = _os.environ.get("SGV3D_F4RES", "1") != "0"
OCC5_TILES = conv_tiles.select("igemm", occ5=True) + conv_tiles.select("igemm", occ5=True, mfirst=True)
OCC5 = _os.environ.get("SGV3D_OCC5", "1") != "0"
WINO4 = _os.environ.get("SGV3D_WINO4", "1") != "0"
WINO4_MIN_CHANNELS = 128
WINO_HALF = _os.environ.get("SGV3D_WINO_HALF", "1") != "0"
PATCH_BF16 = _os.environ.get("SGV3D_PATCH_BF16", "1") != "0"
DW_TILES = conv_tiles.family("dw_bf16")
DW_DEEP_TILES = conv_tiles.select("dw_bf16", deep=True)
DW_DEEP = _os.environ.get("SGV3D_DW_DEEP", "1") != "0"
DW_NARROW = _os.environ.get("SGV3D_DW_NARROW", "1") != "0"
DW_DEEP_MAX_WGS = int(_os.environ.get("SGV3D_DW_DEEP_MAX_WGS", "768"))
DW_BF16 = _os.environ.get("SGV3D_DW_BF16", "1") != "0"
DW_SPLIT_K = _os.environ.get("SGV3D_DW_SPLITK", "1") != "0"


class prof:
    __slots__ = ("name", "flops", "nbytes", "extra", "e0")

    def __init__(self, name, flops=0.0, nbytes=0.0, extra=None):
        self.name, self.flops, self.nbytes, self.extra, self.e0 = name, flops, nbytes, extra, None

    def __enter__(self):
        if PROFILE is not None:
            self.e0 = torch.cuda.Event(enable_timing=True)
            self.e0.record()
        return self

    def __exit__(self, *exc):
        if self.e0 is not None:
            e1 = torch.cuda.Event(enable_timing=True)
# ... 259 lines not shown

    def wino4_ok(self, d=None, gate=None):
        is3x3 = (not self.transposed and self.kh == 3 and self.kw == 3 and self.stride == 1 and self.pad == self.dil)
        wide = min(self.cin, self.cout) >= WINO4_MIN_CHANNELS or (self.cin >= 64 and self.cout >= 1024)
        ok = (WINO4 and WINOGRAD and is3x3 and not MFMA_BF16 and self.cin % 32 == 0 and self.cout % 4 == 0 and wide and gate is None)
        if ok and d is not None:
            ok = ((d.mode == CONV_NORMAL and d.y_ld % 4 == 0 and d.y_coff % 4 == 0) or
                  (d.mode == CONV_GROUP_PLANES and d.deconv_ks % 4 == 0)) and d.x_ld % 4 == 0 and d.x_coff % 4 == 0 and d.res_ld % 4 == 0
        return ok

    def f4res_ok(self, d=None, gate=None, io=0):
        ok = (F4RES and WINO4 and WINOGRAD and not MFMA_BF16 and not MFMA_F32X3 and not self.transposed and self.kh == 3
              and self.kw == 3 and self.stride == 1 and self.pad == 1 and self.dil == 1 and gate is None and io == 0
              and self.cin % 64 == 0 and self.cout % 64 == 0 and (self.cin == 64 or self.cout == 64))
        if ok and d is not None:
            ok = (d.mode == CONV_NORMAL and d.x_ld % 4 == 0 and d.x_coff % 4 == 0 and d.y_ld % 4 == 0 and d.y_coff % 4 == 0
                  and d.res_ld % 4 == 0)
        return ok

    def pw_x3_ok(self, d=None, gate=None, io=0):
        taps = self.kh * self.kw
        shape_ok = ((self.k_order == 1 and self.cin % 32 == 0 and self.cin >= 64 and taps <= 32) or
                    (self.k_order == 0 and self.cin % 4 == 0 and taps <= 64 and taps * self.cin >= 128))
        ok = (PW_X3 and not MFMA_BF16 and not MFMA_F32X3 and not self.transposed and gate is None and io == 0 and shape_ok
              and self.cout % 4 == 0)
        if ok and d is not None:
            ok = (d.mode == CONV_NORMAL and d.x_ld % 4 == 0 and d.x_coff % 4 == 0 and d.y_ld % 4 == 0 and d.y_coff % 4 == 0
                  and d.res_ld % 4 == 0)
        return ok

    def _dw_eligible(self, d, gate=None, io=0):
        return (MFMA_BF16 and not MFMA_F32X3 and DW_BF16 and io == 3 and d.mode in (CONV_NORMAL, CONV_DECONV)
                and gate is None and self.cin % 32 == 0 and self.cout % 8 == 0 and d.x_ld % 8 == 0 and d.x_coff % 8 == 0
                and d.y_ld % 8 == 0 and d.y_coff % 8 == 0 and d.res_ld % 8 == 0)

    def out_hw(self, h, w):
        if self.transposed:
            return h * self.ks, w * self.ks
        oh = (h + 2 * self.pad - self.dil * (self.kh - 1) - 1) // self.stride + 1
        ow = (w + 2 * self.pad - self.dil * (self.kw - 1) - 1) // self.stride + 1
        return oh, ow

    def __call__(self, x, out=None, *, shift=None, **kw):
        if shift is None:
            return self._call(x, out, **kw)
        assert shift.dtype == torch.float32 and shift.numel() == self.cout and shift.is_contiguous() and shift.device == x.device
        saved, self.shift = self.shift, shift
        try:
            return self._call(x, out, **kw)
        finally:
            self.shift = saved

    def _call(self, x, out=None, *, x_coff=0, y_coff=0, residual=None, gate=None, nchw_out=False, tile=None,
              group_planes=0, split_k=None, out_dtype=None):
        B, H, W, x_ld = (int(s) for s in x.shape)
        assert x.is_contiguous() and x.dtype in (torch.float32, torch.bfloat16)
        if out is not None:
            out_dtype = out.dtype
        out_dtype = out_dtype or torch.float32
        io = (1 if x.dtype == torch.bfloat16 else 0) | (2 if out_dtype == torch.bfloat16 else 0)
        if io:
            if not MFMA_BF16 or MFMA_F32X3:
                raise _lib.SGV3DError("bf16 tensors are only handled in bf16 mode (hip_ops.MFMA_BF16)")
            if io & 2:
                assert not (nchw_out or group_planes or gate is not None), "bf16 output: NORMAL / transposed-conv layouts only"
                assert residual is None or residual.dtype == torch.bfloat16
            else:
                assert residual is None or residual.dtype == torch.float32
        oh, ow = self.out_hw(H, W)
        if group_planes:
            assert self.cout % group_planes == 0 and not self.transposed and residual is None
            if out is None:
                out = torch.empty(self.cout // group_planes, B, oh, ow, group_planes, dtype=torch.float32, device=x.device)
            assert out.is_contiguous() and out.numel() == B * oh * ow * self.cout
        elif out is None:
            shape = (B, self.cout, oh, ow) if nchw_out else (B, oh, ow, self.cout)
            out = torch.empty(shape, dtype=out_dtype, device=x.device)
        else:
            want = (B, None, oh, ow) if nchw_out else (B, oh, ow, None)
            got = tuple(int(v) for v in out.shape)
            if len(got) != 4 or any(w is not None and w != g for w, g in zip(want, got)) or not out.is_contiguous():
                raise _lib.SGV3DError(f"conv output buffer {got} does not match {want}")
        y_ld = int(out.shape[1] if nchw_out else out.shape[-1])
        if group_planes:
            y_ld, y_coff = self.cout, 0
        d = ConvDesc()
        d.batch, d.in_h, d.in_w, d.cin = B, H, W, self.cin
        d.out_h, d.out_w, d.cout = oh, ow, self.cout
        d.kh, d.kw, d.stride, d.pad, d.dil = self.kh, self.kw, self.stride, self.pad, self.dil
        d.x_ld, d.x_coff, d.y_ld, d.y_coff = x_ld, int(x_coff), y_ld, int(y_coff)
        d.res_ld = int(residual.shape[-1]) if residual is not None else 0
        d.relu = 1 if self.relu else 0
        d.mode = CONV_DECONV if self.transposed else (CONV_NCHW_OUT if nchw_out else CONV_NORMAL)
        d.deconv_ks = self.ks
        if group_planes:
            d.mode, d.deconv_ks = CONV_GROUP_PLANES, int(group_planes)
        d.k_pad, d.cout_pad = self.k_pad, self.cout_pad
        d.x_nchw = 0
        d.k_order = self.k_order
        lib = _lib.load()
        gemm_m = B * (H * W if self.transposed else oh * ow)
        gemm_n = self.cout * (self.ks * self.ks if self.transposed else 1)
        nkt = self.k_pad // 32
        t = int(self.tile if tile is None else tile)
        sk = int(split_k) if split_k else 0
        if t == 0 or sk == 0:
            key = (B, H, W, t, sk, MFMA_BF16, MFMA_F32X3, d.mode, residual is not None, gate is not None, io)
            choice = self._tile_cache.get(key)
            if choice is None:
                sig = (f"{self.cout}x{self.cin}k{self.kh}x{self.kw}s{self.stride}p{self.pad}d{self.dil}"
                       f"ks{self.ks}|{B}x{H}x{W}|m{d.mode}r{int(residual is not None)}g{int(gate is not None)}|{t}.{sk}"
                       + ("|bf16" if MFMA_BF16 else "|f32x3" if MFMA_F32X3 is True else "|x3auto" if MFMA_F32X3 else "")
                       + (f"|io{io}" if io else "") + f"|ts{TUNE_STREAMS}")
                choice = self._db_choice(sig, d, x, gate, gemm_m, gemm_n, nkt, t, sk, io)
                if choice is not None:
                    self._tile_cache[key] = choice
                    TUNE_STATS["from_db"] += 1
                elif tune_may_measure():
                    TUNE_STATS["measured"] += 1
                    choice = self._autotune(lib, d, x, residual, gate, out, gemm_m, gemm_n, nkt, t, sk, io)
                    self._tile_cache[key] = choice
                    tune_record(sig, choice)
                else:
                    choice = self._rule(t, sk, d, gemm_m, gemm_n, gate)
            t, sk = choice
        d.tile, d.split_k = t, sk
        name, flops, nbytes, extra = self._profile_record(TILES[t], sk, x, out, residual, gemm_m, io)
        with torch.cuda.device(x.device), prof(name, flops, nbytes, extra):
            rc = self._launch(lib, d, x, residual, gate, out, io)
        _lib.check(rc, "sgv3d_conv2d_forward")
        return out

    def _profile_record(self, T, sk, x, out, residual, gemm_m, io):
        B, H, W, _ = (int(s) for s in x.shape)
        ks2 = self.ks * self.ks if self.transposed else 1
        real_n = self.cout_real * ks2
        flops = 2.0 * gemm_m * real_n * (self.cin_real * self.kh * self.kw)
        plain = T.family == "igemm"
        x3 = plain and (T.x3 or (MFMA_F32X3 is True and not (T.mfirst or T.occ5)))
        name = (("conv_igemm_bf16_" if MFMA_BF16 else "conv_igemm_f32x3_" if x3 else "conv_igemm_") if plain else "conv_") + T.label
        pw1 = self.kh == 1 and self.kw == 1 and self.stride == 1 and self.pad == 0
        if plain and self.k_order == 0:
            name += "_tapmajor"
        elif plain and not MFMA_BF16 and not x3:
            if pw1 and not self.transposed and (T.occ5 or self.cin >= 128) and (T.occ5 or T.bm == 64):
                name += "_pw"
            if T.occ5:
                name += "_occ5"
        nbytes = (float(x.element_size()) * B * H * W * self.cin_real
                  + (2.0 if MFMA_BF16 else 4.0) * self.cout_real * self.cin_real * self.kh * self.kw * ks2
                  + float(out.element_size()) * gemm_m * real_n
                  + (float(residual.element_size()) * gemm_m * real_n if residual is not None else 0.0))
        if PROFILE_DETAIL:
            name += (f"|{B}x{H}x{W}x{self.cin}->{self.cout} k{self.kh if not self.transposed else -self.ks} "
                     f"s{self.stride} d{self.dil} splitk{sk}" + (" mfirst" if plain and T.mfirst else "") + (" occ5" if T.occ5 else ""))
        if io:
            name = name.replace("conv_igemm_bf16_", "conv_igemm_bf16io_")
        extra = None
        if PROFILE is not None and not MFMA_BF16 and not x3 and T.symbol:
            b = lambda v: "true" if v else "false"
            symbol = T.symbol.format(chunk=b(self.k_order != 0), pw=b(name.endswith(("_pw", "_pw_occ5"))),
                                     kmode=2 if self.k_order == 0 else 0 if pw1 else 1)
            if T.flops == "wino4":
                oh, ow = self.out_hw(H, W)
                tiles = _wino4_tiles_per_phase(B, oh, ow, self.dil)
                mfma = 2.0 * 36 * (-(-tiles // T.bm) * T.bm) * self.cin * self.cout
            elif T.flops == "direct_k32":
                mfma = 2.0 * gemm_m * self.cout * _up32(self.cin * self.kh * self.kw)
            else:
                mfma = 2.0 * gemm_m * self.cout * self.cin * self.kh * self.kw * ks2
            extra = {"symbol": symbol, "mfma_flops": mfma}
            if T.x3:
                extra["bf16_mfma_flops"] = 6 * mfma
        return name, flops, nbytes, extra

    def _rule(self, t, sk, d, gemm_m, gemm_n, gate=None):
        if t == 0 and self.wino_ok and WINOGRAD and not MFMA_BF16 and d.out_h * d.out_w * d.batch >= 1024:
            wgs = d.batch * -(-d.out_h // 16) * -(-d.out_w // 16) * -(-gemm_n // 64)
            split = 1
            if not sk and SPLIT_K:
                for cand in (2, 3, 4, 6, 8):
                    if wgs * cand <= 512 and self.cin // 8 // cand >= 4:
                        split = cand
            return TILE_WINO, sk or split
        if t == 0 and self._patch_eligible(d, gate) and d.out_h * d.out_w * d.batch >= 4096:
            wgs = d.batch * -(-d.out_h // 16) * -(-d.out_w // 32) * -(-gemm_n // 64)
            split = 1
            if not sk and SPLIT_K:
                for cand in (2, 3, 4, 6, 8):
                    if wgs * cand <= 512 and self.cin // 32 // cand >= 2:
                        split = cand
            return TILE_PATCH, sk or split
        return (t or heuristic_tile(gemm_m, gemm_n)), (sk or 1)

    def _patch_eligible(self, d, gate=None):
        return (MFMA_BF16 and not MFMA_F32X3 and PATCH_BF16 and self.patch_ok and d.mode == CONV_NORMAL and gate is None
                and d.x_ld % 8 == 0 and d.x_coff % 8 == 0 and d.y_ld % 8 == 0 and d.y_coff % 8 == 0
                and (d.res_ld % 8 == 0))

    def _launch(self, lib, d, x, residual, gate, out, io=0):
        T = TILES[d.tile]
        ws, nws = None, 0
        if d.split_k > 1 and T.family != "dw_bf16":
            nws = lib.sgv3d_conv2d_workspace_bytes(ctypes.byref(d))
            ws = torch.empty(nws, dtype=torch.uint8, device=x.device)
        tail = (_lib.ptr(self.scale), _lib.ptr(self.shift), _lib.ptr(residual))
        return getattr(self, "_launch_" + T.entry)(lib, T, d, x, tail, gate, out, io, ws, nws)

    @staticmethod
    def _abi(d, T, k_pad=None, cout_pad=None):
        a = ConvDesc.from_buffer_copy(d)
        if T.abi is not None:
            a.tile = T.abi
        if k_pad is not None:
            a.k_pad, a.cout_pad = k_pad, cout_pad
        return ctypes.byref(a)

    def _launch_conv2d(self, lib, T, d, x, tail, gate, out, io, ws, nws):
        x3 = T.x3 or (MFMA_F32X3 is True)
        if T.occ5 and (MFMA_BF16 or x3 or io or self.k_order != 1):
            raise _lib.SGV3DError("the five-per-CU 64x64 tile is f32 only and needs channel-chunk-major weights (cin % 32 == 0)")
        if io:
            return lib.sgv3d_conv2d_forward_bf16io(self._abi(d, T), x.data_ptr(), self._bf16_weights().data_ptr(), *tail, _lib.ptr(gate),
                                                   out.data_ptr(), _lib.ptr(ws), nws, _st(x), int(io))
        fwd = (lib.sgv3d_conv2d_forward_bf16 if MFMA_BF16 else
               lib.sgv3d_conv2d_forward_f32x3 if x3 else lib.sgv3d_conv2d_forward)
        return fwd(self._abi(d, T), x.data_ptr(), self.w.data_ptr(), *tail, _lib.ptr(gate), out.data_ptr(), _lib.ptr(ws), nws, _st(x))

    def _launch_winograd(self, lib, T, d, x, tail, gate, out, io, ws, nws):
        if not self.wino_ok:
            raise _lib.SGV3DError("this layer has no Winograd weights (needs 3x3 / stride 1 / pad 1 / cin % 8 == 0)")
        return lib.sgv3d_conv2d_winograd_forward(self._abi(d, T), x.data_ptr(), self.w_wino.data_ptr(), *tail, _lib.ptr(gate),
                                                 out.data_ptr(), _lib.ptr(ws), nws, _st(x))

    def _launch_winograd4(self, lib, T, d, x, tail, gate, out, io, ws, nws):
        if not self.wino4_ok(d, gate) or d.split_k > 1:
            raise _lib.SGV3DError("F(4x4) Winograd covers f32 3x3 / stride 1 / pad 1 layers with cin % 32 == 0, cout % 4 == 0, "
                                  "NHWC output, no gate, no split-K")
        u = self._form(T.form)
        a = self._abi(d, T, self.cin, self.wino4_x3_cout_pad) if T.x3 else self._abi(d, T, *self.wino4_geom)
        nws4 = lib.sgv3d_conv2d_winograd4_workspace_bytes(a)
        ws4 = torch.empty(nws4, dtype=torch.uint8, device=x.device)
        return lib.sgv3d_conv2d_winograd4_forward(a, x.data_ptr(), u.data_ptr(), *tail, out.data_ptr(), ws4.data_ptr(), nws4, _st(x))

    def _launch_f4res(self, lib, T, d, x, tail, gate, out, io, ws, nws):
        if not self.f4res_ok(d, gate, io) or d.split_k > 1 or x.dtype != torch.float32:
            raise _lib.SGV3DError("the resident F(4x4) kernel covers f32 3x3 / stride 1 / pad 1 layers with 64 input channels "
                                  "(cout % 64 == 0) or 64 output channels (cin % 64 == 0), NHWC output, no gate, no split-K")
        return lib.sgv3d_conv3x3_f4res_forward(self._abi(d, T), x.data_ptr(), self._form(T.form).data_ptr(), *tail, out.data_ptr(), _st(x))

    def _launch_x3(self, lib, T, d, x, tail, gate, out, io, ws, nws):
        if not self.pw_x3_ok(d, gate, io) or x.dtype != torch.float32:
            raise _lib.SGV3DError("the implicit-GEMM f32x3 kernel covers f32 layers with at most 32 taps, cin % 32 == 0 (>= 64), cout % 4 == 0, "
                                  "NHWC output, no gate")
        u = self._form(T.form)
        return lib.sgv3d_conv2d_x3_forward(self._abi(d, T, d.k_pad, self.pw_x3_cout_pad), x.data_ptr(), u.data_ptr(), *tail, out.data_ptr(),
                                           _lib.ptr(ws), nws, _st(x))

    def _launch_patch_bf16(self, lib, T, d, x, tail, gate, out, io, ws, nws):
        if not self._patch_eligible(d, gate):
            raise _lib.SGV3DError("the bf16 patch kernel covers 3x3 / stride 1 / pad 1 layers with cin % 32 == 0 in bf16 mode")
        return lib.sgv3d_conv3x3_patch_bf16_forward(d.batch, d.in_h, d.in_w, self.cin, self.cout, d.x_ld, d.x_coff, d.y_ld,
                                                    d.y_coff, d.res_ld, d.relu, x.data_ptr(), self._patch_weights().data_ptr(),
                                                    *tail, out.data_ptr(), int(io), int(d.split_k), _lib.ptr(ws), nws, _st(x))

    def _launch_dw_bf16(self, lib, T, d, x, tail, gate, out, io, ws, nws):
        if not self._dw_eligible(d, gate, io) or (d.split_k > 1 and d.mode != CONV_NORMAL):
            raise _lib.SGV3DError("the bf16 direct-weight kernel covers layers with cin % 32 == 0, cout % 8 == 0 and bf16 tensors in "
                                  "and out (NHWC), no gate; split-K in NORMAL mode only")
        if d.split_k > 1:
            nws = lib.sgv3d_conv_dw_bf16_workspace_bytes(ctypes.byref(d))
            ws = torch.empty(nws, dtype=torch.uint8, device=x.device)
            return lib.sgv3d_conv_dw_bf16_forward_splitk(self._abi(d, T), x.data_ptr(), self._dw_weights().data_ptr(), *tail,
                                                         out.data_ptr(), ws.data_ptr(), nws, _st(x))
        return lib.sgv3d_conv_dw_bf16_forward(self._abi(d, T), x.data_ptr(), self._dw_weights().data_ptr(), *tail, out.data_ptr(), _st(x))

    def _time_under_load(self, lib, d, x, residual, gate, out, rounds=None, io=0):
        global _TUNE_SIDE_STREAMS
        cur = torch.cuda.current_stream(x.device)
        if len(_TUNE_SIDE_STREAMS) < TUNE_STREAMS:
            _TUNE_SIDE_STREAMS = [torch.cuda.Stream(device=x.device) for _ in range(TUNE_STREAMS)]
        best = None
        rounds = rounds or TUNE_ROUNDS
        for _ in range(TUNE_REPEATS):
            e0 = torch.cuda.Event(enable_timing=True)
            e1 = torch.cuda.Event(enable_timing=True)
            e0.record(cur)
            for s in _TUNE_SIDE_STREAMS[:TUNE_STREAMS]:
                s.wait_event(e0)
                with torch.cuda.stream(s):
                    for _r in range(rounds):
                        self._launch(lib, d, x, residual, gate, out, io)
                cur.wait_stream(s)
            e1.record(cur)
            e1.synchronize()
            dt = e0.elapsed_time(e1)
            best = dt if best is None else min(best, dt)
        return best

    def _candidates(self, d, gate, gemm_m, gemm_n, nkt, fixed_tile, fixed_split, io=0):
        sel = conv_tiles.select
        mfirst = lambda t: MFIRST and d.mode in (CONV_NORMAL, CONV_NCHW_OUT) and gemm_n > TILES[t].bn
        tiles = sel("igemm") + tuple(t for t in sel("igemm", mfirst=True) if mfirst(t))
        if OCC5 and self.k_order == 1 and not MFMA_BF16 and not MFMA_F32X3 and io == 0:
            tiles += sel("igemm", occ5=True) + tuple(t for t in sel("igemm", occ5=True, mfirst=True) if mfirst(t))
        if MFMA_F32X3 == "auto" and not MFMA_BF16:
            tiles += sel("igemm", x3=True)
        if self.wino_ok and WINOGRAD and not MFMA_BF16:
            tiles += (TILE_WINO,)
            if WINO_HALF:
                tiles += (TILE_WINO_HALF,)
            if self.cin <= 96 and self.cout >= 128:
                tiles += (TILE_WINO_RES,)

        if self.wino4_ok(d, gate):
            tiles += ((TILE_WINO4, TILE_WINO4_WIDE) + ((TILE_WINO4_NARROW,) if self.cin >= 128 else ()) + ((TILE_WINO4_OCC,) if OCC5 else ())
                      + ((TILE_WINO4_G48,) if WINO4_G48 and self.k_order == 1 else ()))
            if WINO4_X3 and not MFMA_F32X3:
                tiles += self._x3_tiles(d)
        if self.f4res_ok(d, gate, io):
            tiles += (TILE_F4RES,)
        if self.pw_x3_ok(d, gate, io):
            tiles += _pw_x3_tiles(gemm_m, gemm_n, nkt)
        if self._patch_eligible(d, gate):
            tiles += (TILE_PATCH,)
        if self._dw_eligible(d, gate, io):
            dw = lambda bm, bn, deep=False: (conv_tiles.by_shape("dw_bf16", bm, bn, deep),)
            deep = self.kh * self.kw * self.cin >= 512
            tiles += (dw(64, 256) + (dw(128, 256) if deep else ()) if gemm_n > 128 else
                      dw(128, 128) + (dw(256, 128) if deep else ()) if gemm_n > 64 else dw(128, 128) + dw(256, 64))
            if DW_DEEP and self.kh * self.kw * self.cin >= 256:
                if gemm_n > 128 and -(-gemm_m // 64) * -(-gemm_n // 256) <= DW_DEEP_MAX_WGS:
                    tiles += dw(64, 256, True)
                    if DW_NARROW and -(-gemm_m // 64) * -(-gemm_n // 256) <= 384:
                        tiles += dw(64, 128) + dw(64, 128, True)
                elif 64 < gemm_n <= 128 and -(-gemm_m // 128) * -(-gemm_n // 128) <= DW_DEEP_MAX_WGS:
                    tiles += dw(128, 128, True)
        if fixed_tile:
            tiles = (fixed_tile,)
        cands = []
        for t in tiles:
            T = TILES[t]
            wgs = -(-gemm_m // T.bm) * -(-gemm_n // T.bn)
            nk = nkt
            if T.spatial:
                th, tw, kc = T.spatial
                nk = self.cin // kc
                wgs = d.batch * -(-d.out_h // th) * -(-d.out_w // tw) * -(-gemm_n // T.bn)
            if T.family == "dw_bf16":
                nk = -(-(self.kh * self.kw * (self.cin // 32)) // 2)
            if T.split is None or (T.family == "dw_bf16" and (d.mode != CONV_NORMAL or not DW_SPLIT_K)):
                splits = (1,)
            elif fixed_split:
                splits = (fixed_split,)
            else:
                splits = (1,) + _split_factors(T.split, nk, wgs)
            cands.append((t, splits))
        return cands

    def _x3_tiles(self, d):
        tiles = _wino4_tiles_per_phase(d.batch, d.out_h, d.out_w, d.dil)
        waste = {r: (-(-tiles // r) * r - tiles) / tiles for r in sorted(set(X3_TILE_ROWS.values()))}
        best = min(waste.values())
        ms = [r for r in waste if waste[r] <= max(best, 0.10) and (r <= 64 or tiles >= r)]
        idle = lambda c: -(-self.cout // c) * c - self.cout
        cols = [128] + ([160] if idle(160) < idle(128) else [])
        return tuple(conv_tiles.by_shape("wino4_x3", r, c) for c in cols for r in ms)

    def _db_choice(self, sig, d, x, gate, gemm_m, gemm_n, nkt, fixed_tile, fixed_split, io=0):
        choice = tune_lookup(sig, x.device)
        if choice is None:
            return None
        t, sk = int(choice[0]), int(choice[1])
        for ct, splits in self._candidates(d, gate, gemm_m, gemm_n, nkt, fixed_tile, fixed_split, io):
            if ct == t and sk in splits:
                return (t, sk)
        del TUNE_DB[sig]
        _COMMITTED_SIGS.discard(sig)
        return None

    def _autotune(self, lib, d, x, residual, gate, out, gemm_m, gemm_n, nkt, fixed_tile, fixed_split, io=0):
        cands = self._candidates(d, gate, gemm_m, gemm_n, nkt, fixed_tile, fixed_split, io)
        best, best_t = (cands[0][0], fixed_split or 1), None
        with torch.cuda.device(x.device):
            for t, splits in cands:
                for sk in splits:
                    d.tile, d.split_k = t, sk
                    _lib.check(self._launch(lib, d, x, residual, gate, out, io), "sgv3d_conv2d_forward")
                    if TUNE_STREAMS > 1:
                        dt = self._time_under_load(lib, d, x, residual, gate, out, io=io)
                    else:
                        nrep = max(4, TUNE_ROUNDS * TUNE_REPEATS // 2)
                        evs = [torch.cuda.Event(enable_timing=True) for _ in range(nrep + 1)]
                        evs[0].record()
                        for r in range(nrep):
                            self._launch(lib, d, x, residual, gate, out, io)
                            evs[r + 1].record()
                        evs[-1].synchronize()
                        dt = min(evs[r].elapsed_time(evs[r + 1]) for r in range(nrep))
                    if TUNE_VERBOSE:
                        print(f"[tune] {self.cout}x{self.cin}k{self.kh} {d.batch}x{d.in_h}x{d.in_w}: tile {t} split {sk}: {dt * 1e3:.1f} us", flush=True)
                    if best_t is None or dt < best_t:
                        best, best_t = (t, sk), dt
        return best


PAIR_BF16 = _os.environ.get("SGV3D_PAIR_BF16", "1") != "0"


PARALLEL_BRANCHES = _os.environ.get("SGV3D_PARALLEL_BRANCHES", "0") == "1"
_BRANCH_POOL = {}
_BRANCH_TOP = {}


_OWNED_STREAMS = {}


def distinct_stream(device, avoid=()):
    dev = torch.device(device)
    key = dev.index if dev.index is not None else torch.cuda.current_device()
    taken = _OWNED_STREAMS.setdefault(key, set())
    banned = {st.cuda_stream for st in avoid if st is not None} | {torch.cuda.current_stream(dev).cuda_stream} | taken
    for _ in range(64):
        st = torch.cuda.Stream(device=dev)
        if st.cuda_stream not in banned:
            if len(taken) < 24:
                taken.add(st.cuda_stream)
            return st
    return torch.cuda.Stream(device=dev)


def release_stream(st):
    for taken in _OWNED_STREAMS.values():
        taken.discard(st.cuda_stream)


def run_parallel(device, thunks):
    thunks = list(thunks)
    if len(thunks) <= 1 or not PARALLEL_BRANCHES or not torch.cuda.is_current_stream_capturing():
        return [t() for t in thunks]
    dev = torch.device(device)
    key = dev.index if dev.index is not None else torch.cuda.current_device()
    pool = _BRANCH_POOL.setdefault(key, [])
    top = _BRANCH_TOP.get(key, 0)
    if top > 0:
        return [t() for t in thunks]
    need = top + len(thunks) - 1
    while len(pool) < need:
        pool.append(distinct_stream(dev, pool))
    mine = pool[top:need]
    _BRANCH_TOP[key] = need
    cur = torch.cuda.current_stream(dev)
    results = [None] * len(thunks)
    try:
        for st, (i, t) in zip(mine, list(enumerate(thunks))[1:]):
            st.wait_stream(cur)
            with torch.cuda.stream(st):
                results[i] = t()
        results[0] = thunks[0]()
    finally:
        for st in mine:
            cur.wait_stream(st)
        _BRANCH_TOP[key] = top
    return results


_GRAPH_SPLIT_HOOK = None


def graph_split_point(tag):
    if _GRAPH_SPLIT_HOOK is not None:
        _GRAPH_SPLIT_HOOK(tag)


def switch_state():
    g = globals()
    return tuple(g.get(k) for k in ("AUTOTUNE", "SPLIT_K", "WINOGRAD", "FUSED_HEAD", "HEAD_PATH", "MFMA_BF16", "BF16_ACTIVATIONS",
                                    "MFMA_F32X3", "MFIRST", "WINO4", "WINO_HALF", "PATCH_BF16", "DW_BF16", "DW_DEEP", "DW_NARROW",
                                    "DW_SPLIT_K", "DW_DEEP_MAX_WGS", "PAIR_BF16", "TUNE_STREAMS", "PARALLEL_BRANCHES", "F4RES", "OCC5", "WINO4_G48", "DCN_FUSED", "WINO4_X3", "WINO4_MULTI", "PW_X3",
                                    "DCN_FUSED_BF16", "DCN_FUSED_TRAIN", "TRAIN_BF16_STORAGE", "SHORTCUT_X3", "DECONV_X3", "VIT_BF16", "STEM_FUSED"))


def conv_pair_eligible(a, b, x, residual=None):
    return (MFMA_BF16 and not MFMA_F32X3 and DW_BF16 and PAIR_BF16 and x.dtype == torch.bfloat16 and not a.transposed and not b.transposed
            and a.cout == 256 and a.cin % 32 == 0 and int(x.shape[-1]) % 8 == 0 and b.cin == 256 and b.kh == 1 and b.kw == 1
            and b.stride == 1 and b.pad == 0 and b.cout % 256 == 0 and (residual is None or residual.dtype == torch.bfloat16))


def conv_pair_bf16(a, b, x, residual=None, out=None):
    B, H, W, x_ld = (int(v) for v in x.shape)
    oh, ow = a.out_hw(H, W)
    if out is None:
        out = torch.empty(B, oh, ow, b.cout, dtype=torch.bfloat16, device=x.device)
    d = ConvDesc()
    d.batch, d.in_h, d.in_w, d.cin = B, H, W, a.cin
    d.out_h, d.out_w, d.cout = oh, ow, a.cout
    d.kh, d.kw, d.stride, d.pad, d.dil = a.kh, a.kw, a.stride, a.pad, a.dil
    d.x_ld, d.x_coff, d.y_ld, d.y_coff = x_ld, 0, a.cout, 0
    d.relu, d.mode, d.split_k = (1 if a.relu else 0), CONV_NORMAL, 1
    flops = 2.0 * B * oh * ow * (a.cout_real * a.cin_real * a.kh * a.kw + b.cout_real * b.cin_real)
    name = "conv_dw_bf16_pair"
    if PROFILE_DETAIL:
        name += f"|{B}x{H}x{W}x{a.cin}->{a.cout} k{a.kh} s{a.stride} d{a.dil} ->{b.cout} k1"
    with torch.cuda.device(x.device), prof(name, flops):
        rc = _lib.load().sgv3d_conv_dw_bf16_pair_forward(
            ctypes.byref(d), x.data_ptr(), a._dw_weights().data_ptr(), _lib.ptr(a.scale), _lib.ptr(a.shift), b.cout,
            b._dw_weights().data_ptr(), _lib.ptr(b.scale), _lib.ptr(b.shift), _lib.ptr(residual),
            int(residual.shape[-1]) if residual is not None else 0, out.data_ptr(), int(out.shape[-1]), 0, 1 if b.relu else 0, _st(x))
    _lib.check(rc, "sgv3d_conv_dw_bf16_pair_forward")
    return out


def conv_pair_choice(a, b, x, residual=None):
    if not conv_pair_eligible(a, b, x, residual):
        return False
    B, H, W, _ = (int(v) for v in x.shape)
    sig = (f"pair|{a.cout}x{a.cin}k{a.kh}x{a.kw}s{a.stride}p{a.pad}d{a.dil}->{b.cout}|{B}x{H}x{W}|r{int(residual is not None)}|bf16|ts{TUNE_STREAMS}")
    hit = tune_lookup(sig, x.device)
    if hit is not None:
        return bool(hit[0])
    if not tune_may_measure():
        return True
    act = torch.bfloat16
    two = lambda: b(a(x, out_dtype=act), residual=residual, out_dtype=act)
    one = lambda: conv_pair_bf16(a, b, x, residual)
    two(); one()
    t2 = time_callable(two, x.device)
    t1 = time_callable(one, x.device)
    tune_record(sig, [1 if t1 < t2 else 0, 0])
    return t1 < t2


SHORTCUT_X3 = _os.environ.get("SGV3D_SHORTCUT_X3", "1") != "0"
# ... 780 lines not shown
```

sgv3d_amd/layers/backbones/bsm_lss_fpn.py:

```python
import copy

import torch
from torch import nn

from ... import hip_ops
from ...calibration import CalibrationCache
from ..blocks import BasicBlock, HipModule, build_backbone, build_neck, conv_bn
from .lss_fpn import ASPP, CACHE_CAMERA_GATES, FUSE_LIFT_SPLAT, HeightNet, LSSFPN, Mlp, SELayer, _require_hip_inference

__all__ = ['BSMLSSFPN']


class SABlock(HipModule):

    def __init__(self, in_channels, out_channels):
        super().__init__()
        self.attention = nn.Sequential(nn.Conv2d(in_channels, out_channels, 3, padding=1, bias=False), nn.Sigmoid())
        self.conv = nn.Conv2d(in_channels, out_channels, 3, padding=1, bias=False)

    def hip_compile(self, device):
        return dict(att=conv_bn(self.attention[0], None, False, device), conv=conv_bn(self.conv, None, False, device))

    def hip_forward_residual(self, x, y, residual):
        s = self.hip_state(x.device)
# ... 123 lines not shown
            layers = s[f'gate{i}']
            h = v
            if tmp is None:
                for w, b, act in layers:
                    h = hip_ops.dense(h, w, None, b, act)
            else:
                bufs = tmp.get(i)
                if bufs is None or bufs[0].shape[0] != v.shape[0]:
                    bufs = tmp[i] = [torch.zeros(v.shape[0], int(w.shape[0]), dtype=torch.float32, device=v.device) for w, _, _ in layers[:-1]]
                last = out[i] if out is not None else torch.zeros(v.shape[0], int(layers[-1][0].shape[0]), dtype=torch.float32, device=v.device)
                for (w, b, act), dst in zip(layers, bufs + [last]):
                    h = hip_ops.dense(h, w, None, b, act, out=dst, run=run)
            res.append(h)
        return res

    def hip_forward(self, feats, mats_dict, out_ld, gates=None):
        s = self.hip_state(feats[0].device)
        if gates is None:
            gates = self.camera_gates(mats_dict, feats[0].device)
        gate = lambda i: gates[i]
        dt = hip_ops.activation_dtype(*[c.cout for c in (s['reduce0'], s['reduce1'], s['ctx0'], s['ctx1a'])])
        dev = feats[0].device

        def scale0_branch():
            r = s['reduce0'](feats[0], out_dtype=dt)
            return self.aspp.hip_forward(hip_ops.scale_channels(r, gate(0)))

        def scale1_branch():
            r = s['reduce1'](feats[1], out_dtype=dt)
            return hip_ops.scale_channels(r, gate(1))
        scale0, scale1 = hip_ops.run_parallel(dev, (scale0_branch, scale1_branch))
        B, H, W, _ = scale1.shape
        out = torch.empty(B, H, W, out_ld, dtype=torch.float32, device=scale1.device)

        def depth_task():
            depth_feat = self.depth_fpn.hip_forward(scale0, scale1)
            self.depth_head1.hip_head(self.depth_head1.hip_decoder(depth_feat), out, y_coff=0)

        def semantic_task():
            semantic_feat = self.semantic_head0.hip_decoder(scale0)
            sem0 = self.semantic_head0.hip_head(semantic_feat)
            semantic_feat = self.semantic_fpn.hip_forward(semantic_feat, scale1)
            return self.semantic_head1.hip_head(self.semantic_head1.hip_decoder(semantic_feat)), sem0

        def context_task():
            context_feat = s['ctx0'](scale0, out_dtype=dt)
            context_feat = self.context_fpn.hip_forward(context_feat, scale1)
            s['ctx1b'](s['ctx1a'](context_feat, out_dtype=dt), out, y_coff=self.depth_channels)
        _, (semantic1, semantic0), _ = hip_ops.run_parallel(dev, (depth_task, semantic_task, context_task))
        return out, semantic1, semantic0


class BSMLSSFPN(LSSFPN):
    def __init__(self, x_bound, y_bound, z_bound, d_bound, final_dim, output_channels, downsample_factor,
                 img_backbone_conf, img_neck_conf, height_net_conf, is_train_height, is_bsm):
        HipModule.__init__(self)
        import numpy as np
        self.downsample_factor = downsample_factor // 2
        self.d_bound = d_bound
        self.final_dim = final_dim
        self.output_channels = output_channels
        self.is_train_height = is_train_height
        self.register_buffer('voxel_size', torch.Tensor([row[2] for row in [x_bound, y_bound, z_bound]]))
        self.register_buffer('voxel_coord',
                             torch.Tensor([row[0] + row[2] / 2.0 for row in [x_bound, y_bound, z_bound]]))
        nums = [(row[1] - row[0]) / row[2] for row in [x_bound, y_bound, z_bound]]
        for q in nums:
            assert abs(q - round(q)) < 1e-6, f"voxel bound does not divide evenly: {q}"
        self.register_buffer('voxel_num', torch.LongTensor([int(round(q)) for q in nums]))
        self.register_buffer('frustum', self.create_frustum())
        self.height_channels, _, _, _ = self.frustum.shape
        self.img_backbone = build_backbone(img_backbone_conf)
        self.img_backbone.init_weights()
        self.img_neck_16 = build_neck(img_neck_conf)
        self.img_neck_16.init_weights()
        neck8 = copy.deepcopy(dict(img_neck_conf))
        neck8['upsample_strides'] = [0.5, 1, 2, 4]
        self.img_neck_8 = build_neck(neck8)
        self.img_neck_8.init_weights()
        self.height_net = self._configure_height_net(height_net_conf)
        self._voxel_num_host = tuple(int(round(q)) for q in nums)
        self._voxel_coord_host = [float(np.float32(row[0] + row[2] / 2.0)) for row in [x_bound, y_bound, z_bound]]
        self._voxel_size_host = [float(np.float32(row[2])) for row in [x_bound, y_bound, z_bound]]
        self.semantic_channels = height_net_conf['semantic_channels']
        self.background_threshold = 0.45
        self.fuse_lift_splat = FUSE_LIFT_SPLAT
        self.calib_cache = CalibrationCache()

    def _configure_height_net(self, height_net_conf):
        return MSCThead(
            in_channels=height_net_conf['in_channels'],
            mid_channels=height_net_conf['mid_channels'],
            depth_channels=self.height_channels,
            semantic_channels=height_net_conf['semantic_channels'],
            context_channels=self.output_channels,
        )

    @property
    def bev_channels(self):
        return self.output_channels + self.semantic_channels

    def get_cam_feats_nhwc(self, imgs):
        batch_size, num_sweeps, num_cams, num_channels, imH, imW = imgs.shape
        imgs = imgs.reshape(batch_size * num_sweeps * num_cams, num_channels, imH, imW).float().contiguous()
        feats = self.img_backbone.hip_forward_image(imgs, split_tag="img_backbone.stage1")
        return [n.hip_forward(feats, out_dtype=hip_ops.activation_dtype(*n.out_channels)) for n in (self.img_neck_16, self.img_neck_8)]
# ... 32 lines not shown
```

sgv3d_amd/layers/backbones/lss_fpn.py:

```python
import ctypes

import numpy as np
import torch
from torch import nn

from ... import _lib, hip_ops
from ...hip_ops import PackedConv, fold_bn
from ...calibration import CalibrationCache
from ...ops.voxel_pooling import VoxelPlan
from ..blocks import BasicBlock, HipModule, build_backbone, build_neck, conv_bn

import os as _os

CACHE_CAMERA_GATES = _os.environ.get("SGV3D_CACHE_CAMERA_GATES", "1") != "0"
GATED_CALIBRATION = _os.environ.get("SGV3D_GATED_CALIBRATION", "1") != "0"
FOLD_ASPP_POOL = _os.environ.get("SGV3D_FOLD_ASPP_POOL", "1") != "0"
FUSE_LIFT_SPLAT = _os.environ.get("SGV3D_FUSE_LIFT_SPLAT", "1") != "0"

__all__ = ['LSSFPN']


class _ASPPModule(HipModule):

    def __init__(self, inplanes, planes, kernel_size, padding, dilation, BatchNorm):
# ... 219 lines not shown

    def camera_gates(self, mats_dict, device, out=None, tmp=None, run=None):
        s = self.hip_state(device)
        v = self.mlp_input(mats_dict)
        for name in ('context', 'height'):
            key = name + '_fc1_folded'
            if key not in s:
                fc1_w, fc1_b, _ = s[name + '_gate'][0]
                s[key] = ((fc1_w * s['bn_scale'][None, :]).contiguous(),
                          (fc1_b + fc1_w @ s['bn_shift']).contiguous())

        def gate(i, name):
            layers = [(s[name + '_fc1_folded'][0], s[name + '_fc1_folded'][1], hip_ops.ACT_RELU)] + list(s[name + '_gate'][1:])
            if tmp is None:
                h = v
                for w, b, act in layers:
                    h = hip_ops.dense(h, w, None, b, act)
                return h
            bufs = tmp.get(name)
            if bufs is None or bufs[0].shape[0] != v.shape[0]:
                bufs = tmp[name] = [torch.zeros(v.shape[0], int(w.shape[0]), dtype=torch.float32, device=v.device) for w, _, _ in layers[:-1]]
            last = out[i] if out is not None else torch.zeros(v.shape[0], int(layers[-1][0].shape[0]), dtype=torch.float32, device=v.device)
            h = v
            for (w, b, act), dst in zip(layers, bufs + [last]):
                h = hip_ops.dense(h, w, None, b, act, out=dst, run=run)
            return h
        return [gate(0, 'context'), gate(1, 'height')]

    def hip_forward(self, x, mats_dict, gates=None):
        s = self.hip_state(x.device)
        B, H, W, _ = x.shape
        dt = hip_ops.activation_dtype(self.mid_channels, self.mid_channels // 4)
        x_in = x
        if gates is None:
            gates = self.camera_gates(mats_dict, x.device)
        g_ctx, g_h = gates
        x = s['reduce'](x_in, out_dtype=dt)
        out = torch.empty(B, H, W, self.height_channels + self.context_channels, dtype=torch.float32, device=x.device)

        def context_branch():
            ctx_in = hip_ops.scale_channels(x, g_ctx)
            s['context'](ctx_in, out, y_coff=self.height_channels)

        def height_branch():
            h = hip_ops.scale_channels(x, g_h)
            for blk in self.height_conv:
                h = blk.hip_forward(h, dt) if isinstance(blk, BasicBlock) else blk.hip_forward(h)
            s['height'](h, out, y_coff=0)
        hip_ops.run_parallel(x.device, (height_branch, context_branch))
        return out


class LSSFPN(HipModule):
    def __init__(self, x_bound, y_bound, z_bound, d_bound, final_dim, output_channels, downsample_factor,
                 img_backbone_conf, img_neck_conf, height_net_conf, is_train_height, is_bsm=False):
        super().__init__()
        self.downsample_factor = downsample_factor
        self.d_bound = d_bound
        self.final_dim = final_dim
        self.output_channels = output_channels
        self.is_train_height = is_train_height

        self.register_buffer('voxel_size', torch.Tensor([row[2] for row in [x_bound, y_bound, z_bound]]))
        self.register_buffer('voxel_coord',
                             torch.Tensor([row[0] + row[2] / 2.0 for row in [x_bound, y_bound, z_bound]]))
        nums = [(row[1] - row[0]) / row[2] for row in [x_bound, y_bound, z_bound]]
        for q in nums:
            assert abs(q - round(q)) < 1e-6, f"voxel bound does not divide evenly: {q}"
        self.register_buffer('voxel_num', torch.LongTensor([int(round(q)) for q in nums]))
        self.register_buffer('frustum', self.create_frustum())
        self.height_channels, _, _, _ = self.frustum.shape

        self.img_backbone = build_backbone(img_backbone_conf)
        self.img_neck = build_neck(img_neck_conf)
        self.img_neck.init_weights()
        self.img_backbone.init_weights()
        self.height_net = self._configure_height_net(height_net_conf)
        self.assist_layer = nn.Conv2d(512, 256, kernel_size=1, stride=1, padding=0)
        self._voxel_num_host = tuple(int(round(q)) for q in nums)
        self._voxel_coord_host = [float(np.float32(row[0] + row[2] / 2.0)) for row in [x_bound, y_bound, z_bound]]
        self._voxel_size_host = [float(np.float32(row[2])) for row in [x_bound, y_bound, z_bound]]
        self.fuse_lift_splat = FUSE_LIFT_SPLAT
        self.calib_cache = CalibrationCache()

    def _configure_height_net(self, height_net_conf):
        return HeightNet(height_net_conf['in_channels'], height_net_conf['mid_channels'], self.output_channels,
                         self.height_channels)

    def create_frustum(self):
        ogfH, ogfW = self.final_dim
        fH, fW = ogfH // self.downsample_factor, ogfW // self.downsample_factor
        alpha = 1.5
        d_coords = np.arange(self.d_bound[2]) / self.d_bound[2]
        d_coords = np.power(d_coords, alpha)
        d_coords = self.d_bound[0] + d_coords * (self.d_bound[1] - self.d_bound[0])
        d_coords = torch.tensor(d_coords, dtype=torch.float).view(-1, 1, 1).expand(-1, fH, fW)
        D, _, _ = d_coords.shape
        x_coords = torch.linspace(0, ogfW - 1, fW, dtype=torch.float).view(1, 1, fW).expand(D, fH, fW)
        y_coords = torch.linspace(0, ogfH - 1, fH, dtype=torch.float).view(1, fH, 1).expand(D, fH, fW)
        paddings = torch.ones_like(d_coords)
        return torch.stack((x_coords, y_coords, d_coords, paddings), -1)

    def get_geometry_voxel_index(self, sensor2ego_mat, sensor2virtual_mat, intrin_mat, ida_mat,
                                 reference_heights, bda_mat, want_float=False, out=None, run=None):
        lib = _lib.load()
        B, num_cams = int(sensor2ego_mat.shape[0]), int(sensor2ego_mat.shape[1])
# ... 64 lines not shown
        run = self._calibration_changed(cc, srcs, force=not (reuse and cc._tag == tag and cc.plan is not None))
        if not reuse:
            run = None
        geom = self.get_geometry_voxel_index(
            mats_dict['sensor2ego_mats'][:, sweep_index, ...],
            mats_dict['sensor2virtual_mats'][:, sweep_index, ...],
            mats_dict['intrin_mats'][:, sweep_index, ...],
            mats_dict['ida_mats'][:, sweep_index, ...],
            mats_dict['reference_heights'][:, sweep_index, ...],
            mats_dict.get('bda_mat', None), out=cc.geom if reuse else None, run=run)
        flat = geom.view(B, -1, 3)
        if reuse and cc.plan is not None:
            cc.plan.rebuild(flat)
        else:
            cc.plan = VoxelPlan(flat, self._voxel_num_host, cached=True)
        cc.geom = geom
        if int(sweep_index) == 0 and CACHE_CAMERA_GATES:
            n_rows = int(s2e.shape[0]) * int(s2e.shape[2])
            keep = cc.gates is not None and all(g.shape[0] == n_rows and g.device == s2e.device for g in cc.gates)
            if not keep:
                cc.gates, cc.gate_tmp = None, {}
            if cc.gate_tmp is None:
                cc.gate_tmp = {}
            cc.gates = self.height_net.camera_gates(mats_dict, s2e.device, out=cc.gates, tmp=cc.gate_tmp, run=run if keep else None)
        cc.remember(srcs, tag)
        cc.mark_built(s2e.device)
        cache.refreshes += 1
        return geom, cc.plan

    def get_cam_feats_nhwc(self, imgs):
        batch_size, num_sweeps, num_cams, num_channels, imH, imW = imgs.shape
        imgs = imgs.reshape(batch_size * num_sweeps * num_cams, num_channels, imH, imW).float().contiguous()
        feats = self.img_backbone.hip_forward_image(imgs, split_tag="img_backbone.stage1")
        return self.img_neck.hip_forward(feats, out_dtype=hip_ops.activation_dtype(*self.img_neck.out_channels))

    def _forward_single_sweep(self, sweep_index, sweep_imgs, mats_dict, nhwc_out=False):
        batch_size, num_sweeps, num_cams, num_channels, img_height, img_width = sweep_imgs.shape
        source_features = self.get_cam_feats_nhwc(sweep_imgs)
        geom_xyz, plan = self.calibration(mats_dict, sweep_index)
        gates = self.calib_cache.entry(0).gates if CACHE_CAMERA_GATES else None
        height_feature = self.height_net.hip_forward(source_features, mats_dict, gates=gates)
        D, C = self.height_channels, self.output_channels
        fH, fW = int(height_feature.shape[1]), int(height_feature.shape[2])
        if self.fuse_lift_splat and num_cams == 1:
            prob, _ = hip_ops.lift(height_feature, D, C, want_prob=True, want_lifted=False)
            ldo = hip_ops.pad_channels(C) if (nhwc_out and hip_ops.activation_dtype(C) == torch.bfloat16 and getattr(self, '_single_sweep', True)) else 0
            ctx = torch.empty(batch_size, fH * fW, C, dtype=torch.float32, device=height_feature.device)
            hip_ops.copy_channels(height_feature, ctx.view(batch_size, fH, fW, C), coff=D)
            bev = plan.lift_splat(prob, ctx, out_bf16_ld=ldo)
        else:
            _, lifted = hip_ops.lift(height_feature, D, C, lifted_dtype=hip_ops.activation_dtype(C))
            ldo = hip_ops.pad_channels(C) if (nhwc_out and lifted.dtype == torch.bfloat16 and getattr(self, '_single_sweep', True)) else 0
            bev = plan.pool(lifted.view(batch_size, num_cams * D * fH * fW, C), out_bf16_ld=ldo)
        feature_map = bev.permute(0, 3, 1, 2)
        if nhwc_out:
            return feature_map.permute(0, 2, 3, 1)
        return hip_ops.nhwc_to_nchw(feature_map.permute(0, 2, 3, 1))

    def forward(self, sweep_imgs, mats_dict, timestamps=None, nhwc_out=False):
        _require_hip_inference(self, sweep_imgs)
        batch_size, num_sweeps, num_cams, num_channels, img_height, img_width = sweep_imgs.shape
        self._single_sweep = num_sweeps == 1
        key_frame_res = self._forward_single_sweep(0, sweep_imgs[:, 0:1, ...], mats_dict, nhwc_out=nhwc_out)
        if num_sweeps == 1:
            return key_frame_res
        ret_feature_list = [key_frame_res]
        for sweep_index in range(1, num_sweeps):
            ret_feature_list.append(self._forward_single_sweep(
                sweep_index, sweep_imgs[:, sweep_index:sweep_index + 1, ...], mats_dict, nhwc_out=nhwc_out))
        return torch.cat(ret_feature_list, 3 if nhwc_out else 1)

    def hip_compile(self, device):
        return {}


def _require_hip_inference(module, x):
    if not x.is_cuda:
        raise RuntimeError("sgv3d_amd runs on the MI355X only: got a CPU tensor and there is no CPU fallback "
                           "(the CPU restatement lives in oracle/ and is test infrastructure)")
    if module.training:
        raise NotImplementedError("this entry point is the inference forward (call model.eval()); a module in training mode "
                                  "goes through sgv3d_amd/train_forward.py, which BEVHeight.forward dispatches to")
```

sgv3d_amd/layers/heads/bev_height_head.py:

```python
import torch
from torch import nn

from ... import hip_ops
from ...hip_ops import PackedConv, fold_bn
from ..blocks import HipModule, build_backbone, build_neck, conv_bn

__all__ = ['BEVHeightHead']

bev_backbone_conf = dict(
    type='ResNet',
    in_channels=80,
    depth=18,
    num_stages=3,
    strides=(1, 2, 2),
    dilations=(1, 1, 1),
    out_indices=[0, 1, 2],
    norm_eval=False,
    base_channels=160,
)

bev_neck_conf = dict(type='SECONDFPN',
                     in_channels=[160, 320, 640],
                     upsample_strides=[2, 4, 8],
                     out_channels=[64, 64, 128])
# ... 66 lines not shown
            heads = dict(common_heads)
            heads.update(dict(heatmap=(num_cls, num_heatmap_convs)))
            sh = dict(separate_head)
            sh.pop('type', None)
            self.task_heads.append(SeparateHead(in_channels=share_conv_channel, heads=heads, head_conv=64, **sh))
        self.trunk = build_backbone(bev_backbone_conf)
        self.trunk.init_weights()
        self.neck = build_neck(bev_neck_conf)
        self.neck.init_weights()
        del self.trunk.maxpool
        self.gaussian_overlap = gaussian_overlap
        self.min_radius = min_radius
        self.train_cfg = train_cfg
        self.test_cfg = test_cfg
        self.share_conv_channel = share_conv_channel

    def _branches(self):
        out = []
        for t, th in enumerate(self.task_heads):
            for name in th.heads:
                out.append((t, name, getattr(th, name)))
        return out

    def hip_compile(self, device):
        br = self._branches()
        hc = 64
        for _, name, seq in br:
            assert len(seq) == 2 and seq[0].conv.out_channels == hc, "fused head expects (ConvModule, Conv2d) branches"
            assert seq[1].out_channels <= 4
        w1 = torch.cat([seq[0].conv.weight.detach() for _, _, seq in br], 0)
        sc, sh = zip(*[fold_bn(seq[0].bn, seq[0].conv.bias) for _, _, seq in br])
        first = PackedConv(w1, pad=1, scale=torch.cat(sc), shift=torch.cat(sh), relu=True, device=device)
        w2 = torch.cat([seq[1].weight.detach().permute(0, 2, 3, 1) for _, _, seq in br], 0)
        b2 = torch.cat([seq[1].bias.detach() for _, _, seq in br], 0)
        out_begin, slices, off = [0], [], 0
        for i, (t, name, seq) in enumerate(br):
            c = seq[1].out_channels
            slices.append((t, name, off, c))
            off += c
            out_begin.append(off)
        f = lambda t_: t_.to(device).float().contiguous()
        ob_dev = torch.tensor(out_begin, dtype=torch.int32, device=device)
        w1_bf16 = None
        if hip_ops.MFMA_BF16 and hip_ops.FUSED_HEAD and tuple(w1.shape[1:]) == (64, 3, 3):
            w1_bf16 = hip_ops.pack_centerhead_bf16(w1.to(device), w2.to(device), ob_dev)
        u_f4 = None
        if hip_ops.FUSED_HEAD and not hip_ops.MFMA_BF16 and tuple(w1.shape[1:]) == (64, 3, 3) and hc == 64:
            u_f4 = hip_ops.pack_centerhead_f4(w1.to(device).float())
        return dict(w1_bf16=w1_bf16, u_f4=u_f4, shared=conv_bn(self.shared_conv.conv, self.shared_conv.bn, True, device), first=first,
                    w2=f(w2), b2=f(b2), branch_of_out=hip_ops.head_branch_of_out([c for _, _, _, c in slices], device),
                    out_begin=ob_dev,
                    slices=slices, nb=len(br), hc=hc, total=off)

    def hip_forward(self, x):
        s = self.hip_state(x.device)
        trunk_outs = [x]
        dt = self.trunk.act_dtype()
        h = self.trunk.hip_state(x.device)['stem'](x, out_dtype=dt)
        for i, layer_name in enumerate(self.trunk.res_layers):
            for blk in getattr(self.trunk, layer_name):
                h = blk.hip_forward(h, dt)
            if i in self.trunk.out_indices:
                trunk_outs.append(h)
        nd = dt if (dt is not None and hip_ops.MFMA_BF16 and s.get('w1_bf16') is not None) else None
        fpn_output = self.neck.hip_forward(trunk_outs, out_dtype=nd)
        shared = s['shared'](fpn_output, out_dtype=nd if fpn_output.dtype == torch.bfloat16 else None)
        if hip_ops.MFMA_BF16 and s.get('w1_bf16') is not None:
            out = hip_ops.centerhead_branches_bf16(shared, s['w1_bf16'], s['first'].scale, s['first'].shift, s['b2'],
                                                   s['out_begin'], s['nb'])
        elif hip_ops.FUSED_HEAD and not hip_ops.MFMA_BF16 and s['first'].wino_ok and s['first'].cin <= 64 and s['hc'] == 64:
            path = self._branch_path(s, shared)
            if path == 2:
                out = self._fused_f4(s, shared)
            elif path == 0:
                out = hip_ops.centerhead_branches(shared, s['first'], s['w2'], s['b2'], s['out_begin'], s['nb'])
            else:
                out = self._two_kernel_branches(s, shared)
        else:
            out = self._two_kernel_branches(s, shared)
        ret = [dict() for _ in self.task_heads]
        for t, name, off, c in s['slices']:
            ret[t][name] = out[:, off:off + c]
        return tuple([d] for d in ret)

    @staticmethod
    def _two_kernel_branches(s, shared):
        hidden = s['first'](shared, group_planes=s['hc'])
        return hip_ops.head_final_conv(hidden, s['w2'], s['b2'], s['branch_of_out'], s['nb'], s['hc'])

    @staticmethod
    def _fused_f4(s, shared):
        return hip_ops.centerhead_branches_f4(shared, s['u_f4'], s['first'].scale, s['first'].shift, s['w2'], s['b2'],
                                              s['out_begin'], s['nb'])

    def _branch_path(self, s, shared):
        f4_ok = (s.get('u_f4') is not None and shared.dtype == torch.float32 and int(shared.shape[-1]) >= 64
                 and s['first'].cin == 64)
        want = hip_ops.HEAD_PATH
        if want in (0, 1, 2):
            return want if (want != 2 or f4_ok) else 0
        B, H, W, _ = (int(v) for v in shared.shape)
        sig = f"centerhead_branches3|{B}x{H}x{W}x{s['nb']}|ts{hip_ops.TUNE_STREAMS}"
        ok = {0: True, 1: s['first'].wino4_ok(), 2: f4_ok}
        hit = hip_ops.tune_lookup(sig, shared.device)
        if hit is not None and ok.get(int(hit[0]) - 100, False):
            return int(hit[0]) - 100
        if not hip_ops.tune_may_measure():
            return 2 if f4_ok else 0
        cands = {0: lambda: hip_ops.centerhead_branches(shared, s['first'], s['w2'], s['b2'], s['out_begin'], s['nb']),
                 1: lambda: self._two_kernel_branches(s, shared), 2: lambda: self._fused_f4(s, shared)}
        cands = {k: f for k, f in cands.items() if ok[k]}
        for f in cands.values():
            f()
        torch.cuda.synchronize(shared.device)
        times = {k: hip_ops.time_callable(f, shared.device, rounds=2) for k, f in cands.items()}
        choice = min(times, key=times.get)
        hip_ops.tune_record(sig, (100 + choice, 1))
        return choice

    def forward(self, x, nhwc=False):
        if not x.is_cuda:
            raise RuntimeError("sgv3d_amd runs on the MI355X only (no CPU fallback)")
        if self.training:
            raise NotImplementedError("HIP path = inference forward; call model.eval()")
        cin_pad = self.trunk.hip_state(x.device)['cin_pad']
        if not nhwc:
            x = hip_ops.nchw_to_nhwc(x.float().contiguous(), c_pad=max(cin_pad, (int(x.shape[1]) + 3) // 4 * 4))
        elif not x.is_contiguous():
            x = x.contiguous()
        if int(x.shape[-1]) < cin_pad:
            x = torch.nn.functional.pad(x, (0, cin_pad - int(x.shape[-1])))
        return self.hip_forward(x)

    def get_targets(self, gt_bboxes_3d, gt_labels_3d):
        import ctypes
        from ... import _lib
        cfg = self.train_cfg
        lib = _lib.load()
        boxes = [getattr(b, 'tensor', b) for b in gt_bboxes_3d]
        dev = next((b.device for b in boxes if b.is_cuda), None) or next(self.parameters()).device
        assert dev.type == 'cuda', "target assignment runs on the GPU (no CPU fallback)"
        B = len(boxes)
        n_max = max([int(b.shape[0]) for b in boxes] + [1])
        bx = torch.zeros(B, n_max, 9, dtype=torch.float32, device=dev)
        lb = torch.full((B, n_max), -1, dtype=torch.int32, device=dev)
        for i, (b, l) in enumerate(zip(boxes, gt_labels_3d)):
            n = int(b.shape[0])
            if n:
                bx[i, :n] = b.to(dev, torch.float32).reshape(n, -1)[:, :9]
                lb[i, :n] = l.to(dev, torch.int32).reshape(n)
        osf = int(cfg['out_size_factor'])
        W, H = int(cfg['grid_size'][0]) // osf, int(cfg['grid_size'][1]) // osf
        max_objs = int(cfg['max_objs']) * int(cfg['dense_reg'])
        T, total = len(self.num_classes), sum(self.num_classes)
        heat = torch.empty(B, total, H, W, dtype=torch.float32, device=dev)
        anno = torch.empty(T, B, max_objs, 10, dtype=torch.float32, device=dev)
        ind = torch.empty(T, B, max_objs, dtype=torch.int64, device=dev)
        mask = torch.empty(T, B, max_objs, dtype=torch.uint8, device=dev)
        cpt = (ctypes.c_int32 * T)(*self.num_classes)
        with torch.cuda.device(dev), hip_ops.prof("centerhead_targets"):
            rc = lib.sgv3d_centerhead_targets(
                B, n_max, bx.data_ptr(), lb.data_ptr(), T, cpt, max_objs, H, W,
                float(cfg['point_cloud_range'][0]), float(cfg['point_cloud_range'][1]), float(cfg['voxel_size'][0]),
                float(cfg['voxel_size'][1]), float(osf), float(cfg['gaussian_overlap']), int(cfg['min_radius']),
                1 if self.norm_bbox else 0, heat.data_ptr(), anno.data_ptr(), ind.data_ptr(), mask.data_ptr(),
                _lib.stream_handle(dev))
        _lib.check(rc, "sgv3d_centerhead_targets")
        heatmaps, c0 = [], 0
        for nc in self.num_classes:
            heatmaps.append(heat[:, c0:c0 + nc])
            c0 += nc
        return heatmaps, [anno[t] for t in range(T)], [ind[t] for t in range(T)], [mask[t] for t in range(T)]

    def loss(self, targets, preds_dicts, **kwargs):
        return _CenterHeadLoss.run(self, targets, preds_dicts)

    def decode_digest(self):
        def freeze(v):
            if isinstance(v, dict):
                return tuple(sorted((str(k), freeze(x)) for k, x in v.items()))
            if isinstance(v, (list, tuple)):
                return tuple(freeze(x) for x in v)
            if torch.is_tensor(v):
                return tuple(v.flatten().tolist())
            return v if isinstance(v, (int, float, str, bool, type(None))) else repr(v)
# ... 189 lines not shown
```

sgv3d_amd/models/bev_height.py:

```python
import os
import weakref

import torch
from torch import nn

from .. import hip_ops
from .. import host_ext as _host_ext
from ..calibration import tensor_version
from ..layers.backbones.bsm_lss_fpn import BSMLSSFPN
from ..layers.backbones.lss_fpn import LSSFPN
from ..layers.blocks import HipModule
from ..layers.heads.bev_height_head import BEVHeightHead

__all__ = ['BEVHeight']

_REGISTRATIONS = [0]
_TRACKED = set()
_LIVE = weakref.WeakSet()
_HOOKS = []


def _count_registration(module, name, value):
    if id(module) in _TRACKED:
        _REGISTRATIONS[0] += 1
# ... 63 lines not shown
            self._flat_reg = _REGISTRATIONS[0]
        self._flat_age += 1
        fast = _host_ext.stamp()
        if fast is not None:
            n, ver, ptr = fast(walk[1])
            return (self._flat_gen, n, ver, ptr)
        n = ver = ptr = 0
        for d in walk[1]:
            for t in d.values():
                if t is not None:
                    n += 1
                    ver += t._version
                    ptr += t.data_ptr() + (id(t) >> 4)
        return (self._flat_gen, n, ver, ptr)

    _RESTAMP_EVERY = 256

    def _apply(self, fn, *args, **kwargs):
        self._flat_dirty = True
        return super()._apply(fn, *args, **kwargs)

    def load_state_dict(self, *args, **kwargs):
        self._flat_dirty = True
        return super().load_state_dict(*args, **kwargs)

    def refresh(self):
        for m in self.modules():
            if isinstance(m, HipModule):
                m._hip = None
        self._param_stamp = None
        self._graphs = {}

    def train(self, mode=True):
        super().train(mode)
        self._flat_dirty = True
        self.refresh()
        return self

    def forward(self, x, mats_dict, timestamps=None):
        if self.training:
            from ..train_forward import bevheight_train_forward
            return bevheight_train_forward(self, x, mats_dict)
        stamp = self._stamp()
        if stamp != self._param_stamp:
            self.refresh()
            self._param_stamp = stamp
        graphed = self._graphed_forward(x, mats_dict)
        if graphed is not None:
            preds, decoded = graphed(self, x, mats_dict)
            self._decoded = (decoded, [weakref.ref(v) for task in preds for v in task[0].values()], tensor_version(preds[0][0]['heatmap']),
                             self._graph_digest)
            return preds
        self._decoded = None
        bev = self.backbone(x, mats_dict, timestamps, nhwc_out=True)
        return self.head(bev, nhwc=True)

    def _graphed_forward(self, x, mats_dict):
        if (not self.graph_forward or self._graph_suspended or torch.is_grad_enabled() or not x.is_cuda
                or hip_ops.PROFILE is not None or torch.cuda.is_current_stream_capturing()):
            return None
        key = (tuple(x.shape), x.dtype, str(x.device), torch.cuda.current_stream(x.device).cuda_stream,
               tuple((k, tuple(v.shape), v.dtype) for k, v in sorted(mats_dict.items())),
               hip_ops.switch_state(), bool(getattr(self.backbone, 'fuse_lift_splat', False)),
               self.head.decode_digest())
        self._graph_digest = key[-1]
        entry = self._graphs.get(key)
        if entry is None:
            self._graphs[key] = entry = [0, None]
            while len(self._graphs) > self.graph_cache_size:
                self._graphs.pop(next(iter(self._graphs)))
        else:
            self._graphs[key] = self._graphs.pop(key)
        entry[0] += 1
        if entry[0] < 2:
            return None
        if entry[1] is None:
            from ..pipeline import GraphedForward, CAPTURE_ERRORS
            try:
                entry[1] = GraphedForward(self, x, mats_dict)
            except CAPTURE_ERRORS as e:
                import warnings
                torch.cuda.synchronize(x.device)
                entry[1] = False
                warnings.warn(f"BEVHeight.forward: hipGraph capture failed ({type(e).__name__}: {e}); this signature keeps "
                              f"launching eagerly", RuntimeWarning, stacklevel=3)
            if entry[1] and self.graph_forward == "auto":
                entry.append(self._replay_pays(entry[1], x, mats_dict))
                if not entry[2]["replay_chosen"]:
                    entry[1] = False
        return entry[1] or None

    def _replay_pays(self, graphed, x, mats_dict, reps=3):
        import time
        from ..pipeline import eager_forward
        dev = x.device

        def timed(fn):
            fn()
            torch.cuda.synchronize(dev)
            t0 = time.perf_counter()
            for _ in range(reps):
                fn()
                torch.cuda.synchronize(dev)
            return (time.perf_counter() - t0) / reps

        def eager():
            with eager_forward(self):
                bev = self.backbone(x, mats_dict, None, nhwc_out=True)
                self.head.decode_device(self.head(bev, nhwc=True))
        t_graph = timed(lambda: graphed(self, x, mats_dict))
        t_eager = timed(eager)
        return {"replay_ms": t_graph * 1e3, "eager_ms": t_eager * 1e3, "replay_chosen": bool(t_graph < 0.98 * t_eager)}

    def get_targets(self, gt_boxes, gt_labels):
        return self.head.get_targets(gt_boxes, gt_labels)

    def loss(self, targets, preds_dicts):
        return self.head.loss(targets, preds_dicts)

    def get_bboxes(self, preds_dicts, img_metas=None, img=None, rescale=False):
        return self.head.get_bboxes(preds_dicts, img_metas, img, rescale, decoded=self._decoded_for(preds_dicts))

    def _decoded_for(self, preds_dicts):
        spec, self._decoded = self._decoded, None
        if spec is None:
            return None
        decoded, refs, version, digest = spec
        try:
            tensors = [v for task in preds_dicts for v in task[0].values()]
        except (TypeError, AttributeError, IndexError, KeyError):
            return None
        if (len(tensors) != len(refs) or any(r() is not t for r, t in zip(refs, tensors)) or version is None
                or tensor_version(tensors[0]) != version or digest != self.head.decode_digest()):
            return None
        return decoded
```

sgv3d_amd/ops/voxel_pooling/voxel_pooling.py:

```python
import weakref

import torch
from torch.autograd import Function

from ... import _lib, hip_ops

_MODE = "planned"
_PLAN_CACHE = {}
_PLAN_CACHE_MAX = 8
CACHE_PLANS = True


def set_mode(mode):
    global _MODE
    if mode not in ("planned", "atomic"):
        raise ValueError("mode must be 'planned' or 'atomic'")
    _MODE = mode


def get_mode():
    return _MODE


_VOXEL_NUM_CACHE = {}


def _voxel_num_ints(voxel_num):
    if isinstance(voxel_num, torch.Tensor):
        if voxel_num.numel() != 3:
            raise RuntimeError("voxel_num must have 3 elements")
        if voxel_num.is_cuda:
            ent = _VOXEL_NUM_CACHE.get(id(voxel_num))
            if ent is not None and ent[0]() is voxel_num and ent[1] == voxel_num._version:
                return ent[2]
            if len(_VOXEL_NUM_CACHE) > 64:
                _VOXEL_NUM_CACHE.clear()
            hit = tuple(int(v) for v in voxel_num.tolist())
            _VOXEL_NUM_CACHE[id(voxel_num)] = (weakref.ref(voxel_num), voxel_num._version, hit)
            return hit
        return tuple(int(v) for v in voxel_num.tolist())
    x, y, z = voxel_num
    return int(x), int(y), int(z)


def _check_cuda(t, name, dtype):
    if not t.is_cuda:
        raise RuntimeError(f"{name} must be a CUDAtensor ")
    if t.dtype != dtype:
        raise RuntimeError(f"{name}: expected {dtype}, got {t.dtype}")


class VoxelPlan:

    def __init__(self, geom_xyz, voxel_num, pos_memo=None, sort_segments=True, cached=False):
        _check_cuda(geom_xyz, "geom_xyz", torch.int32)
        assert geom_xyz.is_contiguous()
        assert not (cached and pos_memo is not None), "the cached build writes no pos_memo (training builds a fresh plan)"
        self.X, self.Y, self.Z = _voxel_num_ints(voxel_num)
        self.B = int(geom_xyz.shape[0])
        self.N = int(geom_xyz.numel() // (3 * self.B))
        self.cached = bool(cached)
        self.sort_segments = bool(sort_segments)
        lib = _lib.load()
        nbytes = lib.sgv3d_voxel_plan_bytes(self.B, self.N, self.X, self.Y)
        if nbytes == 0:
            raise RuntimeError("voxel plan: bad sizes")
        self.buf = torch.empty(nbytes, dtype=torch.uint8, device=geom_xyz.device)
        self.nbytes = nbytes
        if cached:
            with torch.cuda.device(geom_xyz.device):
                _lib.check(lib.sgv3d_voxel_plan_init(self.B, self.N, self.X, self.Y, self.buf.data_ptr(), nbytes,
                                                     _lib.stream_handle(geom_xyz.device)), "sgv3d_voxel_plan_init")
        self.rebuild(geom_xyz, pos_memo)

    def rebuild(self, geom_xyz, pos_memo=None):
        assert geom_xyz.is_contiguous() and geom_xyz.numel() == self.B * self.N * 3 and geom_xyz.dtype == torch.int32
        lib = _lib.load()
        with torch.cuda.device(geom_xyz.device), hip_ops.prof("voxel_plan_build_cached" if self.cached else "voxel_plan_build"):
            st = _lib.stream_handle(geom_xyz.device)
            if self.cached:
                rc = lib.sgv3d_voxel_plan_build_cached(self.B, self.N, self.X, self.Y, self.Z, geom_xyz.data_ptr(),
                                                       self.buf.data_ptr(), self.nbytes, 1 if self.sort_segments else 0, st)
            else:
                rc = lib.sgv3d_voxel_plan_build(self.B, self.N, self.X, self.Y, self.Z, geom_xyz.data_ptr(),
                                                _lib.ptr(pos_memo), self.buf.data_ptr(), self.nbytes,
                                                1 if self.sort_segments else 0, st)
        _lib.check(rc, "sgv3d_voxel_plan_build")
        return self

    def builds(self):
        assert self.cached
        off = _lib.load().sgv3d_voxel_plan_stats_offset(self.B, self.N, self.X, self.Y)
        return int(self.buf[off:off + 44].view(torch.int32)[10].item())

    def _workspace(self, C):
        nws = _lib.load().sgv3d_voxel_pooling_workspace_bytes(self.B, self.N, int(C))
        return torch.empty(nws, dtype=torch.uint8, device=self.buf.device), nws

    def pool(self, input_features, out=None, out_bf16_ld=0):
        bf16 = input_features.dtype == torch.bfloat16
        _check_cuda(input_features, "input_features", torch.bfloat16 if bf16 else torch.float32)
        assert input_features.is_contiguous() and (bf16 or not out_bf16_ld)
        C = int(input_features.shape[-1])
        assert input_features.numel() == self.B * self.N * C
        if out is None:
            out = torch.empty(self.B, self.Y, self.X, int(out_bf16_ld) or C, dtype=torch.bfloat16 if out_bf16_ld else torch.float32,
                              device=input_features.device)
        ws, nws = self._workspace(C)
        lib = _lib.load()
        with torch.cuda.device(input_features.device), hip_ops.prof("voxel_pooling_planned"):
            if bf16:
                rc = lib.sgv3d_voxel_pooling_forward_planned_bf16(
                    self.B, self.N, C, self.X, self.Y, self.buf.data_ptr(), input_features.data_ptr(), out.data_ptr(),
                    int(out_bf16_ld), ws.data_ptr(), nws, _lib.stream_handle(input_features.device))
            else:
                rc = lib.sgv3d_voxel_pooling_forward_planned(
                    self.B, self.N, C, self.X, self.Y, self.buf.data_ptr(), input_features.data_ptr(),
                    out.data_ptr(), ws.data_ptr(), nws, _lib.stream_handle(input_features.device))
        _lib.check(rc, "sgv3d_voxel_pooling_forward_planned")
        return out

# ... 206 lines not shown
```

Before: 296.9.

## Skip empty BEV tiles in head stem conv using voxel-plan occupancy bitmap

```diff
diff --git a/include/sgv3d_hip.h b/include/sgv3d_hip.h
--- a/include/sgv3d_hip.h
+++ b/include/sgv3d_hip.h
@@ -49,6 +49,7 @@
                                   const int32_t *geom_xyz, void *plan, size_t plan_bytes,
                                   int sort_segments, void *stream);
 size_t sgv3d_voxel_plan_stats_offset(int batch_size, int num_points, int num_voxel_x, int num_voxel_y);
+size_t sgv3d_voxel_plan_occupancy_offset(int batch_size, int num_points, int num_voxel_x, int num_voxel_y);
 
 size_t sgv3d_voxel_pooling_workspace_bytes(int batch_size, int num_points, int num_channels);
 int sgv3d_voxel_pooling_forward_planned(int batch_size, int num_points, int num_channels,
@@ -158,6 +159,9 @@
 int sgv3d_conv2d_x3_forward(const sgv3d_conv_desc *desc, const float *x, const void *u3_packed, const float *scale,
                             const float *bias, const float *residual, float *y, void *workspace, size_t workspace_bytes,
                             void *stream);
+int sgv3d_conv2d_x3_forward_occ(const sgv3d_conv_desc *desc, const float *x, const void *u3_packed, const float *scale,
+                                const float *bias, const float *residual, float *y, const uint32_t *occ, int occ_ld,
+                                void *workspace, size_t workspace_bytes, void *stream);
 int sgv3d_conv2d_x3_shortcut_forward(const sgv3d_conv_desc *desc_a, const float *xa, const void *u3a, const float *scale_a,
                                      const float *bias_a, const sgv3d_conv_desc *desc_b, const float *xb, const void *u3b,
                                      const float *scale_b, const float *bias_b, float *y, void *stream);
diff --git a/sgv3d_amd/_lib.py b/sgv3d_amd/_lib.py
--- a/sgv3d_amd/_lib.py
+++ b/sgv3d_amd/_lib.py
@@ -40,6 +40,7 @@
     "sgv3d_voxel_plan_init": (c_int, [c_int] * 4 + [c_void_p, c_size_t, c_void_p]),
     "sgv3d_voxel_plan_build_cached": (c_int, [c_int] * 5 + [c_void_p, c_void_p, c_size_t, c_int, c_void_p]),
     "sgv3d_voxel_plan_stats_offset": (c_size_t, [c_int] * 4),
+    "sgv3d_voxel_plan_occupancy_offset": (c_size_t, [c_int] * 4),
     "sgv3d_voxel_pooling_workspace_bytes": (c_size_t, [c_int] * 3),
     "sgv3d_voxel_pooling_forward_planned": (c_int, [c_int] * 5 + [c_void_p] * 4 + [c_size_t, c_void_p]),
     "sgv3d_voxel_pooling_forward_planned_bf16": (c_int, [c_int] * 5 + [c_void_p] * 3 + [c_int, c_void_p, c_size_t, c_void_p]),
@@ -105,6 +106,7 @@
     "sgv3d_conv_winograd4_pack_weight_x3": (c_int, [c_void_p, c_int, c_int, c_int, c_int, c_void_p, c_void_p]),
     "sgv3d_conv_pack_weight_x3": (c_int, [c_void_p, c_int, c_int, c_int, c_int, c_int, c_int, c_void_p, c_void_p]),
     "sgv3d_conv2d_x3_forward": (c_int, [c_void_p] * 8 + [c_size_t, c_void_p]),
+    "sgv3d_conv2d_x3_forward_occ": (c_int, [c_void_p] * 8 + [c_int, c_void_p, c_size_t, c_void_p]),
     "sgv3d_conv2d_x3_shortcut_forward": (c_int, [c_void_p] * 12),
     "sgv3d_stem_pool_x3_forward": (c_int, [c_int] * 3 + [c_void_p, c_void_p, c_size_t] + [c_void_p] * 3 + [c_int, c_int, c_void_p]),
     "sgv3d_wino4_lattice_axis": (c_int, [c_int] * 5 + [c_void_p] * 3),
diff --git a/sgv3d_amd/csrc/conv_pw_x3.hip b/sgv3d_amd/csrc/conv_pw_x3.hip
--- a/sgv3d_amd/csrc/conv_pw_x3.hip
+++ b/sgv3d_amd/csrc/conv_pw_x3.hip
@@ -21,11 +21,13 @@
     const void *w2;
     int K2, x2_ld, x2_coff;
     unsigned x2_bytes, w2_bytes;
+    const unsigned *occ;
+    int occ_ld;
 };
 
 template <int MA, int WN, int MODE>
 __global__ __launch_bounds__(64 * WN, 2) void conv_pw_x3_kernel(const PwX3Args a) {
-    constexpr bool TAPS = MODE == 1, TM = MODE == 2, DUAL = MODE == 3, DECONV = MODE == 4;
+    constexpr bool TAPS = MODE == 1, OCC = MODE == 5, TM = MODE == 2 || OCC, DUAL = MODE == 3, DECONV = MODE == 4;
     constexpr int NT = 64 * WN, BM = 16 * MA, BN = 32 * WN;
     constexpr int PLANE = x3_plane_bytes(BM), BUF = x3_buf_bytes(BM);
     __shared__ __attribute__((aligned(16))) unsigned char smem[2 * BUF];
@@ -73,7 +75,24 @@
             int tt = 0;
             for (int th = 0; th < a.kh; ++th) {
                 const bool row_in = live && (unsigned)(ih0 + th * a.dil) < (unsigned)a.in_h;
-                for (int tw = 0; tw < a.kw; ++tw, ++tt) mk |= (row_in && (unsigned)(iw0 + tw * a.dil) < (unsigned)a.in_w) ? (1ull << tt) : 0ull;
+                if constexpr (OCC) {
+                    unsigned long long ob = 0;
+                    int ob0 = 0;
+                    if (row_in) {
+                        const unsigned *orow = a.occ + (size_t)(n * a.in_h + ih0 + th * a.dil) * a.occ_ld;
+                        int w0 = (iw0 > 0 ? iw0 : 0) >> 5;
+                        w0 = w0 < a.occ_ld ? w0 : a.occ_ld - 1;
+                        ob0 = w0 * 32;
+                        ob = orow[w0];
+                        if (w0 + 1 < a.occ_ld) ob |= (unsigned long long)orow[w0 + 1] << 32;
+                    }
+                    for (int tw = 0; tw < a.kw; ++tw, ++tt) {
+                        const int iw = iw0 + tw * a.dil;
+                        mk |= (row_in && (unsigned)iw < (unsigned)a.in_w && ((ob >> ((iw - ob0) & 63)) & 1ull)) ? (1ull << tt) : 0ull;
+                    }
+                } else {
+                    for (int tw = 0; tw < a.kw; ++tw, ++tt) mk |= (row_in && (unsigned)(iw0 + tw * a.dil) < (unsigned)a.in_w) ? (1ull << tt) : 0ull;
+                }
             }
             xmask64[i] = mk;
         } else {
@@ -92,6 +111,18 @@
             }
             xmask[i] = mk;
         }
+    }
+    [[maybe_unused]] bool occ_skip = false;
+    if constexpr (OCC) {
+        __shared__ int occ_any;
+        unsigned long long mine = 0;
+#pragma unroll
+        for (int i = 0; i < PA; ++i) mine |= xmask64[i];
+        if (tid == 0) occ_any = 0;
+        __syncthreads();
+        if (__ballot(mine != 0) != 0 && (tid & 63) == 0) occ_any = 1;
+        __syncthreads();
+        occ_skip = occ_any == 0;
     }
     [[maybe_unused]] int ld_tap = 0, ld_kh = 0, ld_kw = 0, ld_c0 = 0;
     [[maybe_unused]] const int cq = a.cin4;
@@ -177,7 +208,11 @@
     } while (0)
 #define PWX3_KLOOP() X3_KLOOP(MA, smem, w_rsrc, wgo, kt0, nkt, x_frag, fw, acc, PWX3_REQUEST, PWX3_STORE)
 
-    PWX3_KLOOP();
+    if constexpr (OCC) {
+        if (!occ_skip) { PWX3_KLOOP(); }
+    } else {
+        PWX3_KLOOP();
+    }
     [[maybe_unused]] f32x4 tkeep[MA][2];
     if constexpr (DUAL) {
 #pragma unroll
@@ -316,7 +351,8 @@
 template <int MA, int WN>
 int launch_pw(const PwX3Args &a, int mode, hipStream_t st) {
     const dim3 grid(a.tiles_m * a.tiles_n, a.split_k > 1 ? a.split_k : 1);
-    if (mode == 4) hipLaunchKernelGGL((conv_pw_x3_kernel<MA, WN, 4>), grid, dim3(64 * WN), 0, st, a);
+    if (mode == 5) hipLaunchKernelGGL((conv_pw_x3_kernel<MA, WN, 5>), grid, dim3(64 * WN), 0, st, a);
+    else if (mode == 4) hipLaunchKernelGGL((conv_pw_x3_kernel<MA, WN, 4>), grid, dim3(64 * WN), 0, st, a);
     else if (mode == 3) hipLaunchKernelGGL((conv_pw_x3_kernel<MA, WN, 3>), grid, dim3(64 * WN), 0, st, a);
     else if (mode == 2) hipLaunchKernelGGL((conv_pw_x3_kernel<MA, WN, 2>), grid, dim3(64 * WN), 0, st, a);
     else if (mode == 1) hipLaunchKernelGGL((conv_pw_x3_kernel<MA, WN, 1>), grid, dim3(64 * WN), 0, st, a);
@@ -339,12 +375,24 @@
     return check_launch("pack_weight_x3_kernel");
 }
 
-extern "C" int sgv3d_conv2d_x3_forward(const sgv3d_conv_desc *d, const float *x, const void *u3_packed, const float *scale,
-                                       const float *bias, const float *residual, float *y, void *workspace, size_t workspace_bytes,
-                                       void *stream) {
+namespace {
+
+int x3_forward_impl(const sgv3d_conv_desc *d, const float *x, const void *u3_packed, const float *scale, const float *bias,
+                    const float *residual, float *y, bool masked, const unsigned *occ, int occ_ld, void *workspace,
+                    size_t workspace_bytes, void *stream) {
     SGV3D_REQUIRE(d && x && u3_packed && y, "conv2d_x3_forward: null pointer");
     const bool tapmajor = d->cin % 32 != 0;
     const bool deconv = d->mode == SGV3D_CONV_DECONV;
+    if (masked) {
+        SGV3D_REQUIRE(occ != nullptr, "conv2d_x3_forward_occ: null occupancy bitmap");
+        SGV3D_REQUIRE(tapmajor && !deconv && d->mode == SGV3D_CONV_NORMAL,
+                      "conv2d_x3_forward_occ: tap-major layers only (cin %% 32 != 0, NHWC output; cin=%d mode=%d)", d->cin, d->mode);
+        SGV3D_REQUIRE(d->in_w > 0 && (long long)occ_ld * 32 >= d->in_w, "conv2d_x3_forward_occ: bitmap row of %d words is too short for in_w=%d",
+                      occ_ld, d->in_w);
+        SGV3D_REQUIRE(d->kw > 0 && d->dil > 0 && (long long)(d->kw - 1) * d->dil < 32,
+                      "conv2d_x3_forward_occ: a row's taps must span fewer than 33 input columns (kw=%d dil=%d)", d->kw, d->dil);
+        SGV3D_REQUIRE((reinterpret_cast<uintptr_t>(occ) & 3) == 0, "conv2d_x3_forward_occ: the bitmap must be 4-B aligned");
+    }
     if (deconv) {
         SGV3D_REQUIRE(d->kh == 1 && d->kw == 1 && d->stride == 1 && d->pad == 0 && d->deconv_ks >= 1 && d->deconv_ks <= 64 &&
                           residual == nullptr,
@@ -380,8 +428,9 @@
     const int variant = d->tile & 15;
     SGV3D_REQUIRE((d->tile & SGV3D_TILE_X3) && (variant & 3) < 3 && (variant & 12) != 12,
                   "conv2d_x3_forward: desc.tile = SGV3D_TILE_X3 | variant, variant in {0,1,2, 4,5,6, 8,9,10}");
-    const int taps = deconv ? 4 : tapmajor ? 2 : (d->kh == 1 && d->kw == 1 && d->stride == 1 && d->pad == 0) ? 0 : 1;
+    const int taps = masked ? 5 : deconv ? 4 : tapmajor ? 2 : (d->kh == 1 && d->kw == 1 && d->stride == 1 && d->pad == 0) ? 0 : 1;
     PwX3Args a;
+    a.occ = masked ? occ : nullptr; a.occ_ld = masked ? occ_ld : 0;
     a.x = x; a.w = u3_packed; a.scale = scale; a.bias = bias; a.res = residual; a.y = y;
     a.M = (int)M; a.K = (int)K; a.N = gemm_n;
     a.x_ld = d->x_ld; a.x_coff = d->x_coff; a.y_ld = d->y_ld; a.y_coff = d->y_coff; a.res_ld = d->res_ld; a.relu = d->relu;
@@ -425,6 +474,20 @@
     r.y = y; r.y_ld = d->y_ld; r.y_coff = d->y_coff; r.mode = d->mode; r.ks = d->deconv_ks; r.cout = d->cout;
     r.m_h = deconv ? d->in_h : d->out_h; r.m_w = deconv ? d->in_w : d->out_w; r.out_h = d->out_h; r.out_w = d->out_w;
     return launch_splitk_reduce(r, st);
+}
+
+}
+
+extern "C" int sgv3d_conv2d_x3_forward(const sgv3d_conv_desc *d, const float *x, const void *u3_packed, const float *scale,
+                                       const float *bias, const float *residual, float *y, void *workspace, size_t workspace_bytes,
+                                       void *stream) {
+    return x3_forward_impl(d, x, u3_packed, scale, bias, residual, y, false, nullptr, 0, workspace, workspace_bytes, stream);
+}
+
+extern "C" int sgv3d_conv2d_x3_forward_occ(const sgv3d_conv_desc *d, const float *x, const void *u3_packed, const float *scale,
+                                           const float *bias, const float *residual, float *y, const uint32_t *occ, int occ_ld,
+                                           void *workspace, size_t workspace_bytes, void *stream) {
+    return x3_forward_impl(d, x, u3_packed, scale, bias, residual, y, true, occ, occ_ld, workspace, workspace_bytes, stream);
 }
 
 extern "C" int sgv3d_conv2d_x3_shortcut_forward(const sgv3d_conv_desc *da, const float *xa, const void *u3a, const float *scale_a,
diff --git a/sgv3d_amd/csrc/voxel_pooling.hip b/sgv3d_amd/csrc/voxel_pooling.hip
--- a/sgv3d_amd/csrc/voxel_pooling.hip
+++ b/sgv3d_amd/csrc/voxel_pooling.hip
@@ -67,8 +67,9 @@
     long long total;
     int nblk;
     int ncw;
-    size_t off_seg, off_cur, off_order, off_slotvox, off_blk, off_hdr, off_geom, off_long, off_perm, off_bins, bytes;
+    size_t off_seg, off_cur, off_order, off_slotvox, off_blk, off_hdr, off_geom, off_long, off_perm, off_bins, off_occ, bytes;
     int long_cap;
+    int occ_ld;
 };
 
 constexpr int kVoxClasses = 55;
@@ -115,7 +116,9 @@
     L.off_perm = al(L.off_long + sizeof(int) * (size_t)(L.long_cap + 1));
     L.off_bins = al(L.off_perm + sizeof(int) * 4 * (size_t)L.V);
     L.ncw = cdiv(L.V, kBlock);
-    L.bytes = al(L.off_bins + sizeof(int) * ((size_t)kVoxClasses * L.ncw + 2 * kVoxClasses + 2));
+    L.off_occ = al(L.off_bins + sizeof(int) * ((size_t)kVoxClasses * L.ncw + 2 * kVoxClasses + 2));
+    L.occ_ld = (X + 31) / 32;
+    L.bytes = al(L.off_occ + sizeof(unsigned) * (size_t)B * Y * L.occ_ld);
     return L;
 }
 
@@ -343,6 +346,25 @@
                                                               const int *__restrict__ dirty) {
     VP_SKIP_IF_CLEAN(dirty);
     vp_long_list_body(V, seg_start, long_list, cap, dirty, (int)blockIdx.x, (int)gridDim.x);
+}
+
+__global__ __launch_bounds__(kBlock) void vp_occupancy_kernel(long long n_words, int X, int occ_ld, const int *__restrict__ seg_start,
+                                                              unsigned *__restrict__ occ, const int *__restrict__ dirty) {
+    VP_SKIP_IF_CLEAN(dirty);
+    const long long i = (long long)blockIdx.x * kBlock + threadIdx.x;
+    if (i >= n_words) return;
+    const long long row = i / occ_ld;
+    const int x0 = (int)(i - row * occ_ld) * 32;
+    const int n = X - x0 < 32 ? X - x0 : 32;
+    const int *s = seg_start + row * X + x0;
+    unsigned bits = 0;
+    int prev = s[0];
+    for (int j = 0; j < n; ++j) {
+        const int next = s[j + 1];
+        bits |= next > prev ? 1u << j : 0u;
+        prev = next;
+    }
+    occ[i] = bits;
 }
 
 __device__ __forceinline__ void vp_fill_body(long long total_pts, int N, int X, int Y, int Z,
@@ -1585,6 +1607,11 @@
         hipLaunchKernelGGL((vp_sort_segments_kernel<256, 8192>), dim3(g_large), dim3(256), 0, st, L.V, seg, order,
                            2048, 0x7fffffff, dirty);
     }
+    {
+        const long long n_words = (long long)batch_size * num_voxel_y * L.occ_ld;
+        hipLaunchKernelGGL(vp_occupancy_kernel, dim3(cdiv(n_words, kBlock)), dim3(kBlock), 0, st, n_words, num_voxel_x, L.occ_ld, seg,
+                           reinterpret_cast<unsigned *>(base + L.off_occ), dirty);
+    }
     if (cached)
         hipLaunchKernelGGL(vp_plan_commit_kernel, dim3(1), dim3(64), 0, st, hdr, p[0], p[1], p[2], p[3], p[4], p[5], p[6]);
     return check_launch(what);
@@ -1949,6 +1976,11 @@
     return plan_layout(batch_size, num_points, num_voxel_x, num_voxel_y).off_hdr;
 }
 
+extern "C" size_t sgv3d_voxel_plan_occupancy_offset(int batch_size, int num_points, int num_voxel_x, int num_voxel_y) {
+    if (batch_size <= 0 || num_points <= 0 || num_voxel_x <= 0 || num_voxel_y <= 0) return 0;
+    return plan_layout(batch_size, num_points, num_voxel_x, num_voxel_y).off_occ;
+}
+
 extern "C" size_t sgv3d_voxel_pooling_workspace_bytes(int batch_size, int num_points, int num_channels) {
     if (batch_size <= 0 || num_points <= 0 || num_channels <= 0) return 0;
     return 16;
diff --git a/sgv3d_amd/hip_ops.py b/sgv3d_amd/hip_ops.py
--- a/sgv3d_amd/hip_ops.py
+++ b/sgv3d_amd/hip_ops.py
@@ -157,6 +157,37 @@
 WINO4_X3 = _os.environ.get("SGV3D_WINO4_X3", "1") != "0"
 PW_X3 = _os.environ.get("SGV3D_PW_X3", "1") != "0"
 PW_X3_TILES = conv_tiles.family("pw_x3")
+BEV_OCC = _os.environ.get("SGV3D_BEV_OCC", "1") != "0"
+
+
+def bev_occ_empty_tiles(occ, in_w, kh, kw, stride, pad, bm, dil=1):
+    import numpy as np
+    occ = np.asarray(occ).astype(np.int64) & 0xffffffff
+    B, in_h, ld = occ.shape
+    bits = ((occ[:, :, :, None] >> np.arange(32)) & 1).reshape(B, in_h, ld * 32)[:, :, :in_w].astype(bool)
+    oh = (in_h + 2 * pad - dil * (kh - 1) - 1) // stride + 1
+    ow = (in_w + 2 * pad - dil * (kw - 1) - 1) // stride + 1
+    padded = np.zeros((B, in_h + 2 * pad, in_w + 2 * pad), dtype=bool)
+    padded[:, pad:pad + in_h, pad:pad + in_w] = bits
+    active = np.zeros((B, oh, ow), dtype=bool)
+    for th in range(kh):
+        for tw in range(kw):
+            active |= padded[:, th * dil:th * dil + (oh - 1) * stride + 1:stride, tw * dil:tw * dil + (ow - 1) * stride + 1:stride]
+    flat = active.reshape(-1)
+    tiles = -(-flat.size // bm)
+    flat = np.concatenate([flat, np.zeros(tiles * bm - flat.size, dtype=bool)])
+    return ~flat.reshape(tiles, bm).any(axis=1)
+
+
+def bev_occ_applies(conv, x_dtype, x_shape, occ_dtype, occ_shape, tile, residual=False, gate=False, io=0, training=False):
+    if not (BEV_OCC and PW_X3 and not MFMA_BF16 and not MFMA_F32X3 and not training and io == 0 and not gate):
+        return False
+    if x_dtype != torch.float32 or occ_dtype != torch.int32 or len(x_shape) != 4 or len(occ_shape) != 3:
+        return False
+    if conv.transposed or conv.k_order != 0 or (conv.kw - 1) * conv.dil >= 32 or int(tile) not in PW_X3_TILES:
+        return False
+    B, H, W, _ = (int(v) for v in x_shape)
+    return tuple(int(v) for v in occ_shape[:2]) == (B, H) and int(occ_shape[2]) * 32 >= W
 PW_X3_DIMS = {t: (TILES[t].bm, TILES[t].bn) for t in PW_X3_TILES}
 
 
@@ -522,7 +553,7 @@
             self.shift = saved
 
     def _call(self, x, out=None, *, x_coff=0, y_coff=0, residual=None, gate=None, nchw_out=False, tile=None,
-              group_planes=0, split_k=None, out_dtype=None):
+              group_planes=0, split_k=None, out_dtype=None, occ=None, occ_choice=None):
         B, H, W, x_ld = (int(s) for s in x.shape)
         assert x.is_contiguous() and x.dtype in (torch.float32, torch.bfloat16)
         if out is not None:
@@ -595,11 +626,56 @@
                     choice = self._rule(t, sk, d, gemm_m, gemm_n, gate)
             t, sk = choice
         d.tile, d.split_k = t, sk
+        if occ is not None and not (occ.is_contiguous() and occ.device == x.device and d.mode == CONV_NORMAL and bev_occ_applies(
+                self, x.dtype, x.shape, occ.dtype, occ.shape, t, residual is not None, gate is not None, io)):
+            occ = None
+        if occ is not None:
+            if occ_choice is None and tile is not None and split_k:
+                occ_choice = (t, sk)
+            choice = occ_choice or self._occ_choice(lib, d, x, residual, out, occ, gemm_m, gemm_n, nkt)
+            if choice is None:
+                occ = None
+            else:
+                t, sk = choice
+                d.tile, d.split_k = t, sk
         name, flops, nbytes, extra = self._profile_record(TILES[t], sk, x, out, residual, gemm_m, io)
+        if occ is not None and extra is not None:
+            extra["symbol"] = extra["symbol"].replace(", 2>", ", 5>")
         with torch.cuda.device(x.device), prof(name, flops, nbytes, extra):
-            rc = self._launch(lib, d, x, residual, gate, out, io)
+            rc = self._launch(lib, d, x, residual, gate, out, io, occ)
         _lib.check(rc, "sgv3d_conv2d_forward")
         return out
+
+    def occ_signature(self, x):
+        B, H, W, _ = (int(v) for v in x.shape)
+        return f"pair|bevocc|{self.cout}x{self.cin}k{self.kh}s{self.stride}|{B}x{H}x{W}|r{int(self.relu)}|ts{TUNE_STREAMS}"
+
+    def _occ_candidates(self, d, gemm_m, gemm_n, nkt):
+        return [(t, sk) for t, splits in self._candidates(d, None, gemm_m, gemm_n, nkt, 0, 0, 0) if t in PW_X3_TILES for sk in splits]
+
+    def _occ_choice(self, lib, d, x, residual, out, occ, gemm_m, gemm_n, nkt):
+        rule = (int(d.tile), int(d.split_k))
+        sig = self.occ_signature(x)
+        hit = tune_lookup(sig, x.device)
+        if hit is not None:
+            on, code = (int(v) for v in hit)
+            if not on:
+                return None
+            choice = (code % 100, max(1, code // 100))
+            return choice if choice in self._occ_candidates(d, gemm_m, gemm_n, nkt) else rule
+        if not tune_may_measure():
+            return rule
+        TUNE_STATS["measured"] += 1
+        cands = self._occ_candidates(d, gemm_m, gemm_n, nkt)
+        if rule not in cands:
+            cands = [rule] + cands
+        plain, times = {}, {}
+        self._time_candidates(lib, d, x, residual, None, out, [rule], 0, None, times=plain)
+        best = self._time_candidates(lib, d, x, residual, None, out, cands, 0, occ, times=times)
+        d.tile, d.split_k = rule
+        on = times[best] < plain[rule]
+        tune_record(sig, [1, 100 * best[1] + best[0]] if on else [0, 0])
+        return best if on else None
 
     def _profile_record(self, T, sk, x, out, residual, gemm_m, io):
         B, H, W, _ = (int(s) for s in x.shape)
@@ -668,13 +744,17 @@
                 and d.x_ld % 8 == 0 and d.x_coff % 8 == 0 and d.y_ld % 8 == 0 and d.y_coff % 8 == 0
                 and (d.res_ld % 8 == 0))
 
-    def _launch(self, lib, d, x, residual, gate, out, io=0):
+    def _launch(self, lib, d, x, residual, gate, out, io=0, occ=None):
         T = TILES[d.tile]
         ws, nws = None, 0
         if d.split_k > 1 and T.family != "dw_bf16":
             nws = lib.sgv3d_conv2d_workspace_bytes(ctypes.byref(d))
             ws = torch.empty(nws, dtype=torch.uint8, device=x.device)
         tail = (_lib.ptr(self.scale), _lib.ptr(self.shift), _lib.ptr(residual))
+        if occ is not None:
+            if T.family != "pw_x3" or self.k_order != 0:
+                raise _lib.SGV3DError("the masked launch is the tap-major f32x3 kernel's (a pw_x3 tile, cin % 32 != 0)")
+            return self._launch_x3(lib, T, d, x, tail, gate, out, io, ws, nws, occ)
         return getattr(self, "_launch_" + T.entry)(lib, T, d, x, tail, gate, out, io, ws, nws)
 
     @staticmethod
@@ -719,11 +799,14 @@
                                   "(cout % 64 == 0) or 64 output channels (cin % 64 == 0), NHWC output, no gate, no split-K")
         return lib.sgv3d_conv3x3_f4res_forward(self._abi(d, T), x.data_ptr(), self._form(T.form).data_ptr(), *tail, out.data_ptr(), _st(x))
 
-    def _launch_x3(self, lib, T, d, x, tail, gate, out, io, ws, nws):
+    def _launch_x3(self, lib, T, d, x, tail, gate, out, io, ws, nws, occ=None):
         if not self.pw_x3_ok(d, gate, io) or x.dtype != torch.float32:
             raise _lib.SGV3DError("the implicit-GEMM f32x3 kernel covers f32 layers with at most 32 taps, cin % 32 == 0 (>= 64), cout % 4 == 0, "
                                   "NHWC output, no gate")
         u = self._form(T.form)
+        if occ is not None:
+            return lib.sgv3d_conv2d_x3_forward_occ(self._abi(d, T, d.k_pad, self.pw_x3_cout_pad), x.data_ptr(), u.data_ptr(), *tail,
+                                                   out.data_ptr(), occ.data_ptr(), int(occ.shape[-1]), _lib.ptr(ws), nws, _st(x))
         return lib.sgv3d_conv2d_x3_forward(self._abi(d, T, d.k_pad, self.pw_x3_cout_pad), x.data_ptr(), u.data_ptr(), *tail, out.data_ptr(),
                                            _lib.ptr(ws), nws, _st(x))
 
@@ -745,7 +828,7 @@
                                                          out.data_ptr(), ws.data_ptr(), nws, _st(x))
         return lib.sgv3d_conv_dw_bf16_forward(self._abi(d, T), x.data_ptr(), self._dw_weights().data_ptr(), *tail, out.data_ptr(), _st(x))
 
-    def _time_under_load(self, lib, d, x, residual, gate, out, rounds=None, io=0):
+    def _time_under_load(self, lib, d, x, residual, gate, out, rounds=None, io=0, occ=None):
         global _TUNE_SIDE_STREAMS
         cur = torch.cuda.current_stream(x.device)
         if len(_TUNE_SIDE_STREAMS) < TUNE_STREAMS:
@@ -760,7 +843,7 @@
                 s.wait_event(e0)
                 with torch.cuda.stream(s):
                     for _r in range(rounds):
-                        self._launch(lib, d, x, residual, gate, out, io)
+                        self._launch(lib, d, x, residual, gate, out, io, occ)
                 cur.wait_stream(s)
             e1.record(cur)
             e1.synchronize()
@@ -851,27 +934,33 @@
 
     def _autotune(self, lib, d, x, residual, gate, out, gemm_m, gemm_n, nkt, fixed_tile, fixed_split, io=0):
         cands = self._candidates(d, gate, gemm_m, gemm_n, nkt, fixed_tile, fixed_split, io)
-        best, best_t = (cands[0][0], fixed_split or 1), None
+        return self._time_candidates(lib, d, x, residual, gate, out, [(t, sk) for t, splits in cands for sk in splits], io,
+                                     first=(cands[0][0], fixed_split or 1))
+
+    def _time_candidates(self, lib, d, x, residual, gate, out, pairs, io=0, occ=None, first=None, times=None):
+        best, best_t = first, None
         with torch.cuda.device(x.device):
-            for t, splits in cands:
-                for sk in splits:
-                    d.tile, d.split_k = t, sk
-                    _lib.check(self._launch(lib, d, x, residual, gate, out, io), "sgv3d_conv2d_forward")
-                    if TUNE_STREAMS > 1:
-                        dt = self._time_under_load(lib, d, x, residual, gate, out, io=io)
-                    else:
-                        nrep = max(4, TUNE_ROUNDS * TUNE_REPEATS // 2)
-                        evs = [torch.cuda.Event(enable_timing=True) for _ in range(nrep + 1)]
-                        evs[0].record()
-                        for r in range(nrep):
-                            self._launch(lib, d, x, residual, gate, out, io)
-                            evs[r + 1].record()
-                        evs[-1].synchronize()
-                        dt = min(evs[r].elapsed_time(evs[r + 1]) for r in range(nrep))
-                    if TUNE_VERBOSE:
-                        print(f"[tune] {self.cout}x{self.cin}k{self.kh} {d.batch}x{d.in_h}x{d.in_w}: tile {t} split {sk}: {dt * 1e3:.1f} us", flush=True)
-                    if best_t is None or dt < best_t:
-                        best, best_t = (t, sk), dt
+            for t, sk in pairs:
+                d.tile, d.split_k = t, sk
+                _lib.check(self._launch(lib, d, x, residual, gate, out, io, occ), "sgv3d_conv2d_forward")
+                if TUNE_STREAMS > 1:
+                    dt = self._time_under_load(lib, d, x, residual, gate, out, io=io, occ=occ)
+                else:
+                    nrep = max(4, TUNE_ROUNDS * TUNE_REPEATS // 2)
+                    evs = [torch.cuda.Event(enable_timing=True) for _ in range(nrep + 1)]
+                    evs[0].record()
+                    for r in range(nrep):
+                        self._launch(lib, d, x, residual, gate, out, io, occ)
+                        evs[r + 1].record()
+                    evs[-1].synchronize()
+                    dt = min(evs[r].elapsed_time(evs[r + 1]) for r in range(nrep))
+                if TUNE_VERBOSE:
+                    print(f"[tune] {self.cout}x{self.cin}k{self.kh} {d.batch}x{d.in_h}x{d.in_w}{' occ' if occ is not None else ''}: "
+                          f"tile {t} split {sk}: {dt * 1e3:.1f} us", flush=True)
+                if times is not None:
+                    times[(t, sk)] = dt
+                if best_t is None or dt < best_t:
+                    best, best_t = (t, sk), dt
         return best
 
 
@@ -948,7 +1037,8 @@
     return tuple(g.get(k) for k in ("AUTOTUNE", "SPLIT_K", "WINOGRAD", "FUSED_HEAD", "HEAD_PATH", "MFMA_BF16", "BF16_ACTIVATIONS",
                                     "MFMA_F32X3", "MFIRST", "WINO4", "WINO_HALF", "PATCH_BF16", "DW_BF16", "DW_DEEP", "DW_NARROW",
                                     "DW_SPLIT_K", "DW_DEEP_MAX_WGS", "PAIR_BF16", "TUNE_STREAMS", "PARALLEL_BRANCHES", "F4RES", "OCC5", "WINO4_G48", "DCN_FUSED", "WINO4_X3", "WINO4_MULTI", "PW_X3",
-                                    "DCN_FUSED_BF16", "DCN_FUSED_TRAIN", "TRAIN_BF16_STORAGE", "SHORTCUT_X3", "DECONV_X3", "VIT_BF16", "STEM_FUSED"))
+                                    "DCN_FUSED_BF16", "DCN_FUSED_TRAIN", "TRAIN_BF16_STORAGE", "SHORTCUT_X3", "DECONV_X3", "VIT_BF16", "STEM_FUSED",
+                                    "BEV_OCC"))
 
 
 def conv_pair_eligible(a, b, x, residual=None):
diff --git a/sgv3d_amd/layers/backbones/bsm_lss_fpn.py b/sgv3d_amd/layers/backbones/bsm_lss_fpn.py
--- a/sgv3d_amd/layers/backbones/bsm_lss_fpn.py
+++ b/sgv3d_amd/layers/backbones/bsm_lss_fpn.py
@@ -199,6 +199,8 @@
 
 
 class BSMLSSFPN(LSSFPN):
+    hands_out_occupancy = False
+
     def __init__(self, x_bound, y_bound, z_bound, d_bound, final_dim, output_channels, downsample_factor,
                  img_backbone_conf, img_neck_conf, height_net_conf, is_train_height, is_bsm):
         HipModule.__init__(self)
diff --git a/sgv3d_amd/layers/backbones/lss_fpn.py b/sgv3d_amd/layers/backbones/lss_fpn.py
--- a/sgv3d_amd/layers/backbones/lss_fpn.py
+++ b/sgv3d_amd/layers/backbones/lss_fpn.py
@@ -295,6 +295,8 @@
 
 
 class LSSFPN(HipModule):
+    hands_out_occupancy = True
+
     def __init__(self, x_bound, y_bound, z_bound, d_bound, final_dim, output_channels, downsample_factor,
                  img_backbone_conf, img_neck_conf, height_net_conf, is_train_height, is_bsm=False):
         super().__init__()
@@ -465,23 +467,29 @@
             _, lifted = hip_ops.lift(height_feature, D, C, lifted_dtype=hip_ops.activation_dtype(C))
             ldo = hip_ops.pad_channels(C) if (nhwc_out and lifted.dtype == torch.bfloat16 and getattr(self, '_single_sweep', True)) else 0
             bev = plan.pool(lifted.view(batch_size, num_cams * D * fH * fW, C), out_bf16_ld=ldo)
+        self._sweep_occ = plan.occupancy if bev.dtype == torch.float32 else None
         feature_map = bev.permute(0, 3, 1, 2)
         if nhwc_out:
             return feature_map.permute(0, 2, 3, 1)
         return hip_ops.nhwc_to_nchw(feature_map.permute(0, 2, 3, 1))
 
-    def forward(self, sweep_imgs, mats_dict, timestamps=None, nhwc_out=False):
+    def forward(self, sweep_imgs, mats_dict, timestamps=None, nhwc_out=False, return_occ=False):
         _require_hip_inference(self, sweep_imgs)
         batch_size, num_sweeps, num_cams, num_channels, img_height, img_width = sweep_imgs.shape
         self._single_sweep = num_sweeps == 1
         key_frame_res = self._forward_single_sweep(0, sweep_imgs[:, 0:1, ...], mats_dict, nhwc_out=nhwc_out)
+        if return_occ:
+            occ, self._sweep_occ = (self._sweep_occ if (num_sweeps == 1 and nhwc_out) else None), None
+            if num_sweeps == 1:
+                return key_frame_res, occ
         if num_sweeps == 1:
             return key_frame_res
         ret_feature_list = [key_frame_res]
         for sweep_index in range(1, num_sweeps):
             ret_feature_list.append(self._forward_single_sweep(
                 sweep_index, sweep_imgs[:, sweep_index:sweep_index + 1, ...], mats_dict, nhwc_out=nhwc_out))
-        return torch.cat(ret_feature_list, 3 if nhwc_out else 1)
+        out = torch.cat(ret_feature_list, 3 if nhwc_out else 1)
+        return (out, None) if return_occ else out
 
     def hip_compile(self, device):
         return {}
diff --git a/sgv3d_amd/layers/heads/bev_height_head.py b/sgv3d_amd/layers/heads/bev_height_head.py
--- a/sgv3d_amd/layers/heads/bev_height_head.py
+++ b/sgv3d_amd/layers/heads/bev_height_head.py
@@ -142,11 +142,11 @@
                     out_begin=ob_dev,
                     slices=slices, nb=len(br), hc=hc, total=off)
 
-    def hip_forward(self, x):
+    def hip_forward(self, x, occ=None):
         s = self.hip_state(x.device)
         trunk_outs = [x]
         dt = self.trunk.act_dtype()
-        h = self.trunk.hip_state(x.device)['stem'](x, out_dtype=dt)
+        h = self.trunk.hip_state(x.device)['stem'](x, out_dtype=dt, occ=None if self.training else occ)
         for i, layer_name in enumerate(self.trunk.res_layers):
             for blk in getattr(self.trunk, layer_name):
                 h = blk.hip_forward(h, dt)
@@ -208,7 +208,7 @@
         hip_ops.tune_record(sig, (100 + choice, 1))
         return choice
 
-    def forward(self, x, nhwc=False):
+    def forward(self, x, nhwc=False, occ=None):
         if not x.is_cuda:
             raise RuntimeError("sgv3d_amd runs on the MI355X only (no CPU fallback)")
         if self.training:
@@ -220,7 +220,7 @@
             x = x.contiguous()
         if int(x.shape[-1]) < cin_pad:
             x = torch.nn.functional.pad(x, (0, cin_pad - int(x.shape[-1])))
-        return self.hip_forward(x)
+        return self.hip_forward(x, occ=occ)
 
     def get_targets(self, gt_bboxes_3d, gt_labels_3d):
         import ctypes
diff --git a/sgv3d_amd/models/bev_height.py b/sgv3d_amd/models/bev_height.py
--- a/sgv3d_amd/models/bev_height.py
+++ b/sgv3d_amd/models/bev_height.py
@@ -139,8 +139,13 @@
                              self._graph_digest)
             return preds
         self._decoded = None
-        bev = self.backbone(x, mats_dict, timestamps, nhwc_out=True)
-        return self.head(bev, nhwc=True)
+        bev, occ = self._backbone_nhwc(x, mats_dict, timestamps)
+        return self.head(bev, nhwc=True, occ=occ)
+
+    def _backbone_nhwc(self, x, mats_dict, timestamps):
+        if getattr(self.backbone, 'hands_out_occupancy', False):
+            return self.backbone(x, mats_dict, timestamps, nhwc_out=True, return_occ=True)
+        return self.backbone(x, mats_dict, timestamps, nhwc_out=True), None
 
     def _graphed_forward(self, x, mats_dict):
         if (not self.graph_forward or self._graph_suspended or torch.is_grad_enabled() or not x.is_cuda
@@ -193,8 +198,8 @@
 
         def eager():
             with eager_forward(self):
-                bev = self.backbone(x, mats_dict, None, nhwc_out=True)
-                self.head.decode_device(self.head(bev, nhwc=True))
+                bev, occ = self._backbone_nhwc(x, mats_dict, None)
+                self.head.decode_device(self.head(bev, nhwc=True, occ=occ))
         t_graph = timed(lambda: graphed(self, x, mats_dict))
         t_eager = timed(eager)
         return {"replay_ms": t_graph * 1e3, "eager_ms": t_eager * 1e3, "replay_chosen": bool(t_graph < 0.98 * t_eager)}
diff --git a/sgv3d_amd/ops/voxel_pooling/voxel_pooling.py b/sgv3d_amd/ops/voxel_pooling/voxel_pooling.py
--- a/sgv3d_amd/ops/voxel_pooling/voxel_pooling.py
+++ b/sgv3d_amd/ops/voxel_pooling/voxel_pooling.py
@@ -67,6 +67,9 @@
             raise RuntimeError("voxel plan: bad sizes")
         self.buf = torch.empty(nbytes, dtype=torch.uint8, device=geom_xyz.device)
         self.nbytes = nbytes
+        ld = (self.X + 31) // 32
+        off = lib.sgv3d_voxel_plan_occupancy_offset(self.B, self.N, self.X, self.Y)
+        self.occupancy = self.buf[off:off + 4 * self.B * self.Y * ld].view(torch.int32).view(self.B, self.Y, ld)
         if cached:
             with torch.cuda.device(geom_xyz.device):
                 _lib.check(lib.sgv3d_voxel_plan_init(self.B, self.N, self.X, self.Y, self.buf.data_ptr(), nbytes,
```

Result: no change. 296.8 (-0.0%).
